# Gepetto/mpc-interface

Hardware: AMD Instinct MI355X
Metric: QP assemblies/sec (P,q,G,h), biped N=16 batched (higher is better)
Workload: dtype f64; 1 GPU; C2 biped LIPM N=16 no=36 nc=76, per-instance (A,B)/given/aim, K1 on chip; batch_per_gpu=4096, global_batch=4096, streams=2

## Files before the change

include/mpcasm.h:

```cpp
#ifndef MPCASM_H
#define MPCASM_H

#include <stddef.h>
#include <stdint.h>

#ifdef __cplusplus
extern "C" {
#endif

typedef enum mpcasm_status {
  MPCASM_OK = 0,
  MPCASM_ERR_ARG = -1,
  MPCASM_ERR_PLAN = -2,
  MPCASM_ERR_HIP = -3,
  MPCASM_ERR_NODEVICE = -4,
  MPCASM_ERR_LIMIT = -5
} mpcasm_status;

typedef struct mpcasm_plan mpcasm_plan;


int mpcasm_abi_version(void);
int mpcasm_device_count(void);
int mpcasm_last_hip(void);
const char* mpcasm_status_string(int status);
enum { MPCASM_OPT_PATH = 1, MPCASM_OPT_PHASE_MASK = 2, MPCASM_OPT_RESIDENT_PER_CU = 3, MPCASM_OPT_JIT = 4,
       MPCASM_OPT_P_DIRECT = 5, MPCASM_OPT_RESIDENT_GRID = 6, MPCASM_OPT_JIT_FETCH_RUNS = 7 };
int mpcasm_set_option(int option, int value);
int mpcasm_plan_set_option(mpcasm_plan* plan, int option, int value);
int mpcasm_resident_lds_bytes(const int32_t* h_itab, size_t n_itab, const double* h_dtab, size_t n_dtab,
                              int64_t out[2]);
int mpcasm_jit_check(const int32_t* h_itab, size_t n_itab, const double* h_dtab, size_t n_dtab,
                     char* log, size_t log_capacity);
int mpcasm_fetch_segments(const int32_t* h_itab, size_t n_itab, const double* h_dtab, size_t n_dtab,
                          int limit, int32_t* out, size_t capacity, int64_t* n_words);

int mpcasm_plan_prepare(const mpcasm_plan* plan, int batch);
int mpcasm_jit_stats(int64_t out[3]);

int mpcasm_fill_su(const double* d_A, const double* d_B, double* d_S, double* d_U,
                   int batch, int N, int n, int m, int ltv, void* stream);

int mpcasm_plan_create(const int32_t* h_itab, size_t n_itab,
                       const double* h_dtab, size_t n_dtab,
                       mpcasm_plan** out_plan);
int mpcasm_plan_destroy(mpcasm_plan* plan);

int mpcasm_plan_sizes(const mpcasm_plan* plan, int64_t out[8]);

int mpcasm_plan_csc_sizes(const mpcasm_plan* plan, int64_t out[2]);

int mpcasm_workspace_bytes(const mpcasm_plan* plan, int batch, size_t* out_bytes);

int mpcasm_assemble(const mpcasm_plan* plan, const double* const* h_src,
                    const int64_t* h_src_stride, const double* d_params,
                    const double* d_given, double* d_P, double* d_q, double* d_G,
                    double* d_h, void* d_work, int batch, void* stream);

int mpcasm_assemble_indexed(const mpcasm_plan* plan, const double* const* h_src,
                            const int64_t* h_src_stride, const double* d_params, const double* d_given,
                            const int32_t* d_given_index, double* d_P, double* d_q, double* d_G,
                            double* d_h, void* d_work, int batch, void* stream);

enum { MPCASM_KERNEL_NONE = 0, MPCASM_KERNEL_RESIDENT = 1, MPCASM_KERNEL_RESIDENT_JIT = 2,
       MPCASM_KERNEL_FUSED = 3, MPCASM_KERNEL_STAGED = 4, MPCASM_KERNEL_TILED = 5,
       MPCASM_KERNEL_TILED_SCAN = 6 ,
       MPCASM_KERNEL_SWEEP = 7 ,
       MPCASM_KERNEL_TILED_SHARED = 8  };
int mpcasm_plan_last_kernel(const mpcasm_plan* plan);

int mpcasm_preview_matrices(const mpcasm_plan* plan, const double* const* h_src,
                            const int64_t* h_src_stride, double* d_PM, int batch,
                            void* stream);

int mpcasm_preview(const double* d_PM, const double* d_given, const double* d_optim,
                   double* d_out, int batch, int rows, int ng, int no, void* stream);

int mpcasm_preview_direct(const mpcasm_plan* plan, const double* const* h_src,
                          const int64_t* h_src_stride, const double* d_given, const double* d_optim,
                          double* d_out, void* d_work, int batch, void* stream);

int mpcasm_goal_distance(const double* d_preview, int64_t preview_stride, const double* d_params,
                         int64_t n_params, const int32_t* d_terms, int nterms, int ngoals,
                         double* d_out, int batch, void* stream);

int mpcasm_preview_goal_distance(const mpcasm_plan* plan, const double* const* h_src,
                                 const int64_t* h_src_stride, const double* d_given,
                                 const double* d_optim, const double* d_params, const int32_t* d_terms,
                                 int nterms, int ngoals, double* d_out, void* d_work, int batch,
                                 void* stream);

enum { MPCASM_PREVIEW_NONE = 0 , MPCASM_PREVIEW_DIRECT = 1,
       MPCASM_PREVIEW_STAGED = 2 ,
       MPCASM_PREVIEW_BLOCKED = 3  };
int mpcasm_preview_route(const int32_t* h_itab, size_t n_itab, const double* h_dtab, size_t n_dtab,
                         const int64_t* h_src_stride, int nterms, int ngoals, int32_t out[8]);

int mpcasm_sweep_route(const int32_t* h_itab, size_t n_itab, const double* h_dtab, size_t n_dtab, int32_t out[8]);

enum { MPCASM_TILED_SCAN = 1, MPCASM_TILED_TOEPLITZ = 2, MPCASM_TILED_SHARED = 3, MPCASM_TILED_GENERAL = 4 };
enum { MPCASM_TILED_TABLES_NONE = 0, MPCASM_TILED_TABLES_SMALL = 1 ,
       MPCASM_TILED_TABLES_SYSTEM = 2  };
enum { MPCASM_WANT_COST = 1, MPCASM_WANT_CONSTRAINTS = 2 };
int mpcasm_tiled_route(const int32_t* h_itab, size_t n_itab, const double* h_dtab, size_t n_dtab,
                       const int64_t* h_src_stride, int batch, int want, int path, int32_t out[16]);

int mpcasm_gather(const double* d_src, int64_t src_stride, const int32_t* d_index, int nnz,
                  double* d_dst, int batch, void* stream);

enum { MPCASM_BOX_RECENTER = 0, MPCASM_BOX_TRANSLATE, MPCASM_BOX_ROTATE, MPCASM_BOX_SCALE,
       MPCASM_BOX_MARGIN };
int mpcasm_box_transform(double* d_params, int64_t n_params, int batch, const int32_t* d_facets,
                         int nfacets, int op, const double* d_arg, int64_t arg_stride,
                         void* stream);

int mpcasm_box_transform_ss(double* d_params, int64_t n_params, int batch,
                            const int32_t* d_facets, int nfacets, int op, const double* d_L,
                            int lrows, int ss_dim, const double* d_arg, int64_t arg_stride,
                            void* stream);

int mpcasm_admm(int no, int nc, const double* d_P, const double* d_q, const double* d_G,
                const double* d_h, double* d_x, double* d_y, double* d_z, double* d_res, double rho,
                double sigma, double alpha, int iters, int warm, int batch, double* d_kinv, int kinv_valid,
                void* stream);

enum {
  MPCASM_QP_SOLVED = 1,
  MPCASM_QP_MAX_ITER = -2,
  MPCASM_QP_PRIMAL_INFEASIBLE = -3,
  MPCASM_QP_DUAL_INFEASIBLE = -4,
  MPCASM_QP_NON_CVX = -7
};

int mpcasm_qp_solve(int no, int nc, const double* d_P, const double* d_q, const double* d_G,
                    const double* d_h, double* d_x, double* d_y, double* d_z, int warm, double* d_rho,
                    double sigma, double alpha, double eps_abs, double eps_rel, double eps_prim_inf,
                    double eps_dual_inf, int max_iter, int check_every, int adaptive_rho_interval,
                    int32_t* d_status, int32_t* d_iters, double* d_res, int batch, double* d_kinv,
                    int kinv_valid, void* stream);
int mpcasm_qp_solve_lds_bytes(int no, int nc, int64_t* out);

int mpcasm_qp_solve_wide(int no, int nc, const double* d_P, const double* d_q, const double* d_G,
                         const double* d_h, double* d_x, double* d_y, double* d_z, int warm, double* d_rho,
                         double sigma, double alpha, double eps_abs, double eps_rel, double eps_prim_inf,
                         double eps_dual_inf, int max_iter, int check_every, int adaptive_rho_interval,
                         int32_t* d_status, int32_t* d_iters, double* d_res, int batch, double* d_kinv,
                         int kinv_valid, void* stream);
int mpcasm_qp_solve_wide_info(int no, int nc, int64_t* lds_bytes, int32_t* kinv_on_chip);

enum { MPCASM_GIVEN_KEEP = -1, MPCASM_GIVEN_CONST = -2 };
int mpcasm_given_map_compile(const mpcasm_plan* plan, const int32_t* h_rows, const double* h_values, int ng,
                             int32_t* h_map, int64_t capacity, int64_t* words);

#define MPCASM_QP_BIT(status) (1u << ((status) < 0 ? -(status) : (status)))
int mpcasm_next_given(const mpcasm_plan* plan, const double* const* h_src, const int64_t* h_src_stride,
                      double* d_given, int64_t rows, const double* d_optim, const int32_t* d_index,
                      const int32_t* d_status, uint32_t apply_mask, const int32_t* d_map, int64_t map_words,
                      void* d_work, int count, void* stream);

enum { MPCASM_ROLL_GIVEN = 0, MPCASM_ROLL_OPTIM = 1, MPCASM_ROLL_STATE = 2 };
#define MPCASM_ROLL_REC_WORDS 8
int mpcasm_ltv_rollout_compile(const int32_t* h_itab, size_t n_itab, const double* h_dtab, size_t n_dtab,
                               const int32_t h_sizes[7], const int32_t* h_recs, int nrec, const double* h_cvec,
                               int ncvec, int32_t* h_table, int64_t capacity, int64_t* words);

int mpcasm_ltv_rollout(const mpcasm_plan* plan, const double* const* h_src, const int64_t* h_src_stride,
                       const double* d_given, int64_t rows, const double* d_optim, const int32_t* d_index,
                       const int32_t* d_table, int64_t table_words, double* d_out, int count, void* stream);

int mpcasm_ltv_advance(const mpcasm_plan* plan, const double* const* h_src, const int64_t* h_src_stride,
                       double* d_given, int64_t rows, const double* d_optim, const int32_t* d_index,
                       const int32_t* d_status, uint32_t apply_mask, const int32_t* d_table, int64_t table_words,
                       int count, void* stream);

#ifdef __cplusplus
}
#endif
#endif
```

mpc-interface_amd/csrc/capi.hip:

```cpp
#include <hip/hip_runtime.h>
#include <stdint.h>
#include <stdlib.h>
#include <string.h>

#include <algorithm>
#include <cmath>
#include <mutex>
#include <new>
#include <string>
#include <vector>

#include "jit.h"
#include "kernels.h"

using namespace mpcasm;

namespace mpcasm {
int g_p_direct = 0;
extern int g_path;
extern int g_phase_mask;
extern int g_resident_per_cu, g_resident_grid;
}

struct mpcasm_plan {
// ... 777 lines not shown
    }
    if (it[H_CSC_PNNZ] != 0 || it[H_CSC_GNNZ] != 0) {
      const int64_t pn = it[H_CSC_PNNZ], gn = it[H_CSC_GNNZ], ldp = no + (no & 1);
      if (gn * nc > (1ll << 27)) return MPCASM_ERR_PLAN;
      if (pn < 0 || gn < 0 || pn > no * no || gn > nc * no || (it[H_CSC_GSINGLE] & ~1) ||
          !in_range(it[H_OFF_CSC_P], pn, n, H_WORDS) || !in_range(it[H_OFF_CSC_G], gn * 2, n, H_WORDS) ||
          it[H_OFF_CSC_G] % 2)
        return MPCASM_ERR_PLAN;
      const int32_t* cp = it + it[H_OFF_CSC_P];
      for (int64_t k = 0; k < pn; ++k)
        if (cp[k] < 0 || cp[k] / ldp >= no || cp[k] % ldp >= no) return MPCASM_ERR_PLAN;
      const int32_t* cg = it + it[H_OFF_CSC_G];
      for (int64_t k = 0; k < gn; ++k) {
        const uint32_t w0 = (uint32_t)cg[2 * k], w1 = (uint32_t)cg[2 * k + 1];
        bool found = false;
        for (int64_t R = 0; R < nc && !found; ++R) {
          const int32_t* x = rrw + R * RS_RR_WORDS;
          if (x[RR_NAXES] > 2) return MPCASM_ERR_PLAN;
          for (int sw = 0; sw < 2 && !found; ++sw) {
            const uint32_t v0 = (uint32_t)x[RR_VOFF + sw], v1 = (uint32_t)x[RR_VOFF + 1 - sw];
            const uint32_t a0 = (uint32_t)x[RR_ARROW + sw], a1 = (uint32_t)x[RR_ARROW + 1 - sw];
            if (w1 != (a0 | (a1 << 16))) continue;
            const uint32_t c = (w0 & 0xFFFF) - v0;
            found = (w0 & 0xFFFF) >= v0 && c < (uint32_t)no && (w0 >> 16) == v1 + c && v1 + c < 65536;
          }
        }
        if (!found) return MPCASM_ERR_PLAN;
      }
    }
    for (int64_t g = 0; g < nlti; ++g) {
      const int32_t* x = it + it[H_OFF_RS_LTI] + g * RS_LTI_WORDS;
      const int64_t gn = x[LT_N], gm = x[LT_M], gN = x[LT_HORIZON];
      if (gn < 1 || gm < 1 || gN < 1 || gn > 64 || gm > 64 || gN > 4096) return MPCASM_ERR_PLAN;
      int stages = 0;
      while ((1ll << stages) < gN) ++stages;
      if (!in_range(x[LT_A], gn * gn, nab, 0) || !in_range(x[LT_B], gn * gm, nab, 0) ||
          !in_range(x[LT_TA], gN * gn * gn, img, dma) || !in_range(x[LT_TB], gN * gn * gm, img, dma) ||
          !in_range(x[LT_TP], (stages + 1) * gn * gn, img, dma))
        return MPCASM_ERR_PLAN;
    }
    auto loads_ok = [&](const int32_t* im, int64_t lanes, int64_t bytes) {
      for (int64_t i = 0; i < lanes; ++i) {
        const int st = im[2 * i];
        const int64_t off = im[2 * i + 1];
        if (st < 0 || st > it[H_NSRC] + 2 || off < 0 || off % bytes) return false;
        const int64_t lim = st < it[H_NSRC]        ? (it + it[H_OFF_ARENA])[2 * st + 1]
                            : st == it[H_NSRC]     ? ng
                            : st == it[H_NSRC] + 1 ? (int64_t)it[H_NPARAMS]
                                                   : 4;
        if (off + bytes > lim * 8) return false;
      }
      return true;
    };
    if (!loads_ok(it + it[H_OFF_RS_INMETA], nchunk * 64, unit) ||
        !loads_ok(it + it[H_OFF_RS_ABMETA], nab * 2, 4))
      return MPCASM_ERR_PLAN;
    for (int c = 0; c < no; ++c) {
      int on = 0;
      for (int g = 0; g < it[H_NGTERM]; ++g) {
        const int32_t* r = it + it[H_OFF_GTERM] + g * GT_WORDS;
        if ((r[GT_FLAGS] & GT_FLAG_DIAG) && c >= r[GT_AOFF] && c < r[GT_AOFF] + r[GT_NROWS]) ++on;
      }
      if (on > RS_DIAG_MAX) return MPCASM_ERR_PLAN;
    }
  }

  {
    const int vrc = validate_tiled(it, h_dtab, n, nd);
    if (vrc != MPCASM_OK) return vrc;
    const int src = validate_sweep(it, n, nd);
    if (src != MPCASM_OK) return src;
  }
  const int32_t* seg = it + it[H_OFF_SEG];
  for (int s = 0; s < it[H_NSEG]; ++s) {
    const int32_t* r = seg + s * SEG_WORDS;
    if (r[SEG_KIND] != SEG_KIND_GATHER && r[SEG_KIND] != SEG_KIND_IDENTITY) return MPCASM_ERR_PLAN;
    if (r[SEG_KIND] == SEG_KIND_GATHER && (r[SEG_SRC] < 0 || r[SEG_SRC] >= it[H_NSRC]))
      return MPCASM_ERR_PLAN;
    if (r[SEG_DST0] < 0 || r[SEG_LEN] < 0 || r[SEG_DST0] + r[SEG_LEN] > W) return MPCASM_ERR_PLAN;
  }
  const int32_t* colseg = it + it[H_OFF_COLSEG];
  for (int64_t i = 0; i < (int64_t)it[H_NBASE] * W; ++i)
    if (colseg[i] < -1 || colseg[i] >= it[H_NSEG]) return MPCASM_ERR_PLAN;
  auto check_csr = [&](int off_ptr, int rows, int off_base, int nent) {
    const int32_t* rp = it + off_ptr;
    if (rp[0] != 0 || rp[rows] != nent) return false;
    for (int r = 0; r < rows; ++r)
      if (rp[r + 1] < rp[r]) return false;
    const int32_t* eb = it + off_base;
    for (int e = 0; e < nent; ++e)
      if (eb[e] < 0 || eb[e] >= it[H_NBASE]) return false;
    return true;
  };
  if (!check_csr(it[H_OFF_ROWPTR], it[H_RTOT], it[H_OFF_ENTBASE], it[H_NENT])) return MPCASM_ERR_PLAN;
  if (!check_csr(it[H_OFF_PM_ROWPTR], it[H_PMROWS], it[H_OFF_PM_ENTBASE], it[H_PM_NENT]))
    return MPCASM_ERR_PLAN;
  const int32_t* gt = it + it[H_OFF_GTERM];
  for (int g = 0; g < it[H_NGTERM]; ++g) {
    const int32_t* r = gt + g * GT_WORDS;
    const int nr = r[GT_NROWS];
    if (r[GT_WPARAM] < 0 || r[GT_WPARAM] >= it[H_NPARAMS]) return MPCASM_ERR_PLAN;
    if (r[GT_AIMPARAM] < 0 || r[GT_AIMPARAM] >= it[H_NPARAMS]) return MPCASM_ERR_PLAN;
    if (r[GT_FLAGS] & GT_FLAG_DIAG) {
      if ((r[GT_FLAGS] & GT_FLAG_P) || nr < 0 || r[GT_AOFF] < 0 || r[GT_AOFF] + nr > no ||
          r[GT_BOFF] < 0 || r[GT_BOFF] + nr > it[H_NDIAGCOEF])
        return MPCASM_ERR_PLAN;
      continue;
    }
    if (nr < 0 || r[GT_AOFF] < 0 || r[GT_AOFF] + nr > it[H_RTOT]) return MPCASM_ERR_PLAN;
    if (r[GT_DOFF] < 0 || r[GT_DOFF] + nr > it[H_RTOT]) return MPCASM_ERR_PLAN;
    if ((r[GT_FLAGS] & GT_FLAG_P) && (r[GT_BOFF] < 0 || r[GT_BOFF] + nr > it[H_RTOT]))
      return MPCASM_ERR_PLAN;
    if (r[GT_WPARAM] < 0 || r[GT_WPARAM] >= it[H_NPARAMS]) return MPCASM_ERR_PLAN;
    if (r[GT_AIMPARAM] < 0 || r[GT_AIMPARAM] >= it[H_NPARAMS]) return MPCASM_ERR_PLAN;
  }
  const int32_t* lim = it + it[H_OFF_LIMIT];
  const int32_t* lax = it + it[H_OFF_LAX];
  const int32_t* rowlimit = it + it[H_OFF_ROWLIMIT];
  for (int l = 0; l < it[H_NLIMIT]; ++l) {
    const int32_t* r = lim + l * LM_WORDS;
    const int nr = r[LM_NROWS], na = r[LM_NAXES];
    if (nr < 0 || na < 0 || r[LM_OUT0] < 0 || r[LM_OUT0] + nr > nc) return MPCASM_ERR_PLAN;
    if (r[LM_LAX0] < 0 || r[LM_LAX0] + na > it[H_NLAX]) return MPCASM_ERR_PLAN;
    const int ar = r[LM_ARROW_ROWS], cr = r[LM_CENTER_ROWS], er = r[LM_EXTREME_ROWS];
    if ((ar != 1 && ar != nr) || (cr != 1 && cr != nr) || (er != 1 && er != nr))
      return MPCASM_ERR_PLAN;
    if (r[LM_ARROW_P] < 0 || r[LM_ARROW_P] + ar * na > it[H_NPARAMS]) return MPCASM_ERR_PLAN;
    if (r[LM_CENTER_P] < 0 || r[LM_CENTER_P] + cr * na > it[H_NPARAMS]) return MPCASM_ERR_PLAN;
    if (r[LM_EXTREME_P] < 0 || r[LM_EXTREME_P] + er > it[H_NPARAMS]) return MPCASM_ERR_PLAN;
    for (int a = 0; a < na; ++a) {
      const int32_t* x = lax + (r[LM_LAX0] + a) * LX_WORDS;
      if ((x[LX_ROWS] != 1 && x[LX_ROWS] != nr) || x[LX_ROWOFF] < 0 ||
          x[LX_ROWOFF] + x[LX_ROWS] > it[H_RTOT])
        return MPCASM_ERR_PLAN;
    }
    for (int k = 0; k < nr; ++k)
      if (rowlimit[r[LM_OUT0] + k] != l) return MPCASM_ERR_PLAN;
  }
  return MPCASM_OK;
}

int make_src_table(const mpcasm_plan* plan, const double* const* h_src,
                   const int64_t* h_src_stride, SrcTable* out) {
  memset(out, 0, sizeof(*out));
  for (int s = 0; s < plan->dev.nsrc; ++s) {
    if (!h_src[s] || h_src_stride[s] < 0) return MPCASM_ERR_ARG;
    out->ptr[s] = h_src[s];
    out->stride[s] = h_src_stride[s];
  }
  return MPCASM_OK;
}

}

namespace {
void plan_dev_from_tables(const int32_t* it, PlanDev* out) {
  PlanDev& d = *out;
  d.ng = it[H_NG]; d.no = it[H_NO]; d.nc = it[H_NC]; d.nparams = it[H_NPARAMS];
  d.nsrc = it[H_NSRC]; d.nbase = it[H_NBASE]; d.nseg = it[H_NSEG]; d.rtot = it[H_RTOT];
  d.nent = it[H_NENT]; d.ngterm = it[H_NGTERM]; d.nlimit = it[H_NLIMIT]; d.nlax = it[H_NLAX];
  d.pmrows = it[H_PMROWS]; d.pm_nent = it[H_PM_NENT]; d.ldv = it[H_LDV];
  d.off_seg = it[H_OFF_SEG]; d.off_colseg = it[H_OFF_COLSEG]; d.off_rowptr = it[H_OFF_ROWPTR];
  d.off_entbase = it[H_OFF_ENTBASE]; d.off_entk = it[H_OFF_ENTK]; d.off_gterm = it[H_OFF_GTERM];
  d.off_limit = it[H_OFF_LIMIT]; d.off_lax = it[H_OFF_LAX]; d.off_rowlimit = it[H_OFF_ROWLIMIT];
  d.off_pm_rowptr = it[H_OFF_PM_ROWPTR]; d.off_pm_entbase = it[H_OFF_PM_ENTBASE];
  d.off_pm_entk = it[H_OFF_PM_ENTK];
  d.doff_entcoef = it[H_DOFF_ENTCOEF]; d.doff_pm_entcoef = it[H_DOFF_PM_ENTCOEF];
  d.fused_ok = it[H_FUSED_OK]; d.arena_total = it[H_ARENA_TOTAL]; d.off_arena = it[H_OFF_ARENA];
  d.nfd = it[H_NFD]; d.off_fd_idx = it[H_OFF_FD_IDX]; d.off_fd_ptr = it[H_OFF_FD_PTR];
  d.nops = it[H_NOPS]; d.off_op = it[H_OFF_OP]; d.ncoef = it[H_NCOEF];
  d.doff_coefpool = it[H_DOFF_COEFPOOL];
  d.rs_ok = it[H_RS_OK]; d.rs_jc = it[H_RS_JC]; d.rs_sym = it[H_RS_SYM];
  d.rs_ntrip = it[H_RS_NTRIP]; d.off_rs_src = it[H_OFF_RS_SRC]; d.off_rs_gidx = it[H_OFF_RS_GIDX];
  d.off_rs_dst = it[H_OFF_RS_DST]; d.doff_rs_coef = it[H_DOFF_RS_COEF];
  d.off_rs_trip = it[H_OFF_RS_TRIP]; d.off_rs_wtrip = it[H_OFF_RS_WTRIP];
  d.rs_nsplit = it[H_RS_NSPLIT]; d.off_rs_split = it[H_OFF_RS_SPLIT];
  d.off_rs_rr = it[H_OFF_RS_RR]; d.rs_unit = it[H_RS_UNIT]; d.rs_nchunk = it[H_RS_NCHUNK];
  d.off_rs_inmeta = it[H_OFF_RS_INMETA]; d.rs_img = it[H_RS_IMG];
  d.rs_img_given = it[H_RS_IMG_GIVEN]; d.rs_img_params = it[H_RS_IMG_PARAMS];
  d.doff_rs_const = it[H_DOFF_RS_CONST];
  d.rs_nlti = it[H_RS_NLTI]; d.off_rs_lti = it[H_OFF_RS_LTI]; d.rs_img_dma = it[H_RS_IMG_DMA];
  d.rs_ab = it[H_RS_AB]; d.off_rs_abmeta = it[H_OFF_RS_ABMETA];
  d.rr_packed = it[H_RR_PACKED];
  d.off_rs_dpar = it[H_OFF_RS_DPAR]; d.doff_rs_dcoef = it[H_DOFF_RS_DCOEF];
  d.rs_ngdesc = it[H_RS_NGDESC]; d.off_rs_gdesc = it[H_OFF_RS_GDESC];
  d.rs_nzblk = it[H_RS_NZBLK]; d.off_rs_zblk = it[H_OFF_RS_ZBLK];
  d.rs_gsingle = it[H_RS_GSINGLE];
  d.csc_pnnz = it[H_CSC_PNNZ]; d.off_csc_p = it[H_OFF_CSC_P];
  d.csc_gnnz = it[H_CSC_GNNZ]; d.off_csc_g = it[H_OFF_CSC_G];
  d.csc_gsingle = it[H_CSC_GSINGLE];
  d.t_ci_ok = it[H_T_CI_OK]; d.t_nop = it[H_T_NOP]; d.off_t_cig = it[H_OFF_T_CIG];
  d.off_t_cio = it[H_OFF_T_CIO]; d.t_doff_delta = it[H_T_DOFF_DELTA]; d.t_ok = it[H_T_OK];
  d.t_nstage = it[H_T_NSTAGE]; d.off_t_stage = it[H_OFF_T_STAGE]; d.t_nlti = it[H_T_NLTI];
  d.off_t_lti = it[H_OFF_T_LTI]; d.off_t_lti_ids = it[H_OFF_T_LTI_IDS]; d.t_work = it[H_T_WORK];
  d.off_t_grow = it[H_OFF_T_GROW];
  d.off_t_srow = it[H_OFF_T_SROW]; d.t_doff_scoef = it[H_T_DOFF_SCOEF]; d.off_t_pig = it[H_OFF_T_PIG];
  d.t_ngrest = it[H_T_NGREST]; d.off_t_grest = it[H_OFF_T_GREST]; d.off_t_brow0 = it[H_OFF_T_BROW0]; d.t_toeplitz = it[H_T_TOEPLITZ];
  d.off_t_bcolptr = it[H_OFF_T_BCOLPTR]; d.off_t_bcols = it[H_OFF_T_BCOLS];
  d.rs_ngfix = it[H_RS_NGFIX]; d.off_rs_gfix = it[H_OFF_RS_GFIX];
  d.rs_compact = it[H_RS_COMPACT]; d.rs_ldv = it[H_RS_LDV]; d.rs_vd = it[H_RS_VD];
  d.rs_vrow0 = it[H_RS_VROW0]; d.off_rs_rrwin = it[H_OFF_RS_RRWIN];
  d.t_np1 = it[H_T_NP1]; d.off_t_p1ptr = it[H_OFF_T_P1PTR]; d.off_t_p1ent = it[H_OFF_T_P1ENT]; d.off_t_p2y = it[H_OFF_T_P2Y];
  d.t_scan = it[H_T_SCAN]; d.t_scan_nblk = it[H_T_SCAN_NBLK]; d.off_t_scan_blk = it[H_OFF_T_SCAN_BLK];
  d.off_t_scan_gt = it[H_OFF_T_SCAN_GT]; d.t_doff_scan_gc = it[H_T_DOFF_SCAN_GC];
  d.off_t_scan_grow = it[H_OFF_T_SCAN_GROW]; d.t_doff_scan_gcoef = it[H_T_DOFF_SCAN_GCOEF];
  d.t_scan_ngrest = it[H_T_SCAN_NGREST]; d.off_t_scan_grest = it[H_OFF_T_SCAN_GREST];
  d.off_t_scan_colblk = it[H_OFF_T_SCAN_COLBLK]; d.t_scan_nother = it[H_T_SCAN_NOTHER];
  d.sw_ok = it[H_SW_OK]; d.sw_n = it[H_SW_N]; d.sw_m = it[H_SW_M]; d.sw_horizon = it[H_SW_HORIZON];
  d.sw_src_a = it[H_SW_SRC_A]; d.sw_src_b = it[H_SW_SRC_B]; d.sw_naxes = it[H_SW_NAXES];
  d.off_sw_axis = it[H_OFF_SW_AXIS]; d.sw_nterm = it[H_SW_NTERM]; d.off_sw_term = it[H_OFF_SW_TERM];
  d.sw_nlim = it[H_SW_NLIM]; d.off_sw_lim = it[H_OFF_SW_LIM]; d.off_sw_col = it[H_OFF_SW_COL];
  d.sw_doff_cvec = it[H_SW_DOFF_CVEC]; d.sw_ncvec = it[H_SW_NCVEC];
  d.off_sw_cptr = it[H_OFF_SW_CPTR]; d.off_sw_cent = it[H_OFF_SW_CENT]; d.sw_ncent = it[H_SW_NCENT];
  d.off_sw_gptr = it[H_OFF_SW_GPTR]; d.off_sw_gent = it[H_OFF_SW_GENT]; d.sw_ngent = it[H_SW_NGENT];
  d.off_rs_prog = it[H_OFF_RS_PROG];
  d.t_scan_fused = it[H_T_SCAN_FUSED];
  d.t_nbrow = d.t_ci_ok ? it[d.off_t_brow0 + d.nbase] : 0;
  d.pm_nfd = it[H_PM_NFD]; d.off_pm_map = it[H_OFF_PM_MAP]; d.off_pm_fdptr = it[H_OFF_PM_FDPTR];
  d.off_pm_op = it[H_OFF_PM_OP]; d.doff_pm_pool = it[H_DOFF_PM_POOL];
  d.rs_src16 = 0;
  if (d.rs_ok && d.rs_unit == 16)
    for (int64_t i = 0; i < (int64_t)d.rs_nchunk * 64; ++i) {
      const int st = it[d.off_rs_inmeta + 2 * i];
      if (st < d.nsrc) d.rs_src16 |= 1u << st;
    }
  d.doff_diagcoef = it[H_DOFF_DIAGCOEF];
  d.ndiag = 0;
  d.rs_sym_any = 1;
  for (int g = 0; g < it[H_NGTERM]; ++g) {
    const int32_t* r = it + it[H_OFF_GTERM] + g * GT_WORDS;
    if (r[GT_FLAGS] & GT_FLAG_DIAG) ++d.ndiag;
    if ((r[GT_FLAGS] & GT_FLAG_P) && r[GT_AOFF] != r[GT_BOFF]) d.rs_sym_any = 0;
  }
  d.rs_diag_table = 1;
  {
    std::vector<int> on(std::max(d.no, 1), 0);
    for (int g = 0; g < it[H_NGTERM]; ++g) {
      const int32_t* r = it + it[H_OFF_GTERM] + g * GT_WORDS;
      if (!(r[GT_FLAGS] & GT_FLAG_DIAG)) continue;
      for (int k = 0; k < r[GT_NROWS]; ++k)
        if (++on[r[GT_AOFF] + k] > RS_DIAG_MAX) d.rs_diag_table = 0;
    }
    if (it[H_OFF_RS_DPAR] % 4 || it[H_DOFF_RS_DCOEF] % 2) d.rs_diag_table = 0;
  }
  d.max_axes = 0;
  for (int l = 0; l < it[H_NLIMIT]; ++l) {
    const int na = it[it[H_OFF_LIMIT] + l * LM_WORDS + LM_NAXES];
    if (na > d.max_axes) d.max_axes = na;
  }
  if (d.fused_ok && (d.off_op & 1)) d.fused_ok = 0;
  d.rs_p_direct = d.rs_ok ? resident_choose_p_direct(d, g_p_direct) : 0;
  if (d.csc_pnnz != 0 && d.rs_ok) d.rs_p_direct = resident_choose_p_direct(d, 2);
}

}

extern "C" {

int mpcasm_abi_version(void) { return 1003; }

int mpcasm_device_count(void) {
  int n = 0;
  if (hipGetDeviceCount(&n) != hipSuccess) return 0;
  return n;
}

int mpcasm_last_hip(void) { return g_last_hip; }

int mpcasm_set_option(int option, int value) {
  if (option == MPCASM_OPT_PATH) {
    if (value < 0 || value > 4) return MPCASM_ERR_ARG;
    g_path = value;
    return MPCASM_OK;
  }
  if (option == MPCASM_OPT_PHASE_MASK) {
    g_phase_mask = value;
    return MPCASM_OK;
  }
  if (option == MPCASM_OPT_P_DIRECT) {
    if (value < 0 || value > 2) return MPCASM_ERR_ARG;
    g_p_direct = value;
    return MPCASM_OK;
  }
  if (option == MPCASM_OPT_JIT) {
    if (value < 0 || value > 2) return MPCASM_ERR_ARG;
    g_jit = value;
    return MPCASM_OK;
  }
  if (option == MPCASM_OPT_RESIDENT_PER_CU) {
    if (value < 0 || value > 16) return MPCASM_ERR_ARG;
    g_resident_per_cu = value;
    return MPCASM_OK;
  }
  if (option == MPCASM_OPT_JIT_FETCH_RUNS) {
    if (value < 0 || value > FS_MAX) return MPCASM_ERR_ARG;
    g_jit_fetch_runs = value;
    return MPCASM_OK;
  }
  if (option == MPCASM_OPT_RESIDENT_GRID) {
    if (value < 0 || value > (1 << 20)) return MPCASM_ERR_ARG;
    g_resident_grid = value;
    return MPCASM_OK;
  }
  return MPCASM_ERR_ARG;
}

int mpcasm_plan_set_option(mpcasm_plan* plan, int option, int value) {
  if (!plan) return MPCASM_ERR_ARG;
  if (option == MPCASM_OPT_PATH && value >= -1 && value <= 4) plan->opt_path = value;
  else if (option == MPCASM_OPT_JIT && value >= -1 && value <= 2) plan->opt_jit = value;
  else if (option == MPCASM_OPT_RESIDENT_PER_CU && value >= -1 && value <= 16) plan->opt_per_cu = value;
  else if (option == MPCASM_OPT_RESIDENT_GRID && value >= -1 && value <= (1 << 20)) plan->opt_grid = value;
  else return MPCASM_ERR_ARG;
  return MPCASM_OK;
}

const char* mpcasm_status_string(int status) {
  switch (status) {
    case MPCASM_OK: return "ok";
    case MPCASM_ERR_ARG: return "invalid argument";
    case MPCASM_ERR_PLAN: return "malformed plan tables";
    case MPCASM_ERR_HIP: return "HIP runtime error";
    case MPCASM_ERR_NODEVICE: return "no HIP device";
    case MPCASM_ERR_LIMIT: return "problem exceeds a kernel limit";
    default: return "unknown status";
  }
}

int mpcasm_fill_su(const double* d_A, const double* d_B, double* d_S, double* d_U, int batch,
                   int N, int n, int m, int ltv, void* stream) {
  if (!d_A || !d_B || !d_S || !d_U) return MPCASM_ERR_ARG;
  if (batch < 0 || N < 1 || n < 1 || m < 1 || (ltv != 0 && ltv != 1)) return MPCASM_ERR_ARG;
  if (batch == 0) return MPCASM_OK;
  if (mpcasm_device_count() == 0) return MPCASM_ERR_NODEVICE;
  hipError_t err;
  const int rc = launch_fill_su(d_A, d_B, d_S, d_U, batch, N, n, m, ltv,
                                static_cast<hipStream_t>(stream), &err);
  if (rc == MPCASM_ERR_HIP) g_last_hip = (int)err;
  return rc;
}

int mpcasm_plan_create(const int32_t* h_itab, size_t n_itab, const double* h_dtab, size_t n_dtab,
                       mpcasm_plan** out_plan) {
  if (!h_itab || !out_plan || (n_dtab && !h_dtab)) return MPCASM_ERR_ARG;
  *out_plan = nullptr;
  const int rc = validate_plan(h_itab, h_dtab, n_itab, n_dtab);
  if (rc != MPCASM_OK) return rc;
  {
    PlanDev probe;
    memset(&probe, 0, sizeof probe);
    plan_dev_from_tables(h_itab, &probe);
    if ((probe.csc_pnnz != 0 || probe.csc_gnnz != 0) &&
        (probe.rs_p_direct != 0 || resident_lds_bytes(probe) == 0 ||
         resident_lds_bytes(probe) > RESIDENT_LDS_LIMIT))
      return MPCASM_ERR_LIMIT;
  }
  if (mpcasm_device_count() == 0) return MPCASM_ERR_NODEVICE;

  mpcasm_plan* plan = new (std::nothrow) mpcasm_plan();
  if (!plan) return MPCASM_ERR_ARG;
  hipError_t e;
  if ((e = hipGetDevice(&plan->device)) != hipSuccess) {
    delete plan;
    return hip_fail(e);
  }
  plan->d_itab = nullptr;
  plan->d_dtab = nullptr;
  const size_t dbytes = (n_dtab ? n_dtab : 1) * sizeof(double);
  if ((e = hipMalloc(&plan->d_itab, n_itab * sizeof(int32_t))) != hipSuccess ||
      (e = hipMalloc(&plan->d_dtab, dbytes)) != hipSuccess ||
      (e = hipMemcpy(plan->d_itab, h_itab, n_itab * sizeof(int32_t), hipMemcpyHostToDevice)) !=
          hipSuccess ||
      (n_dtab && (e = hipMemcpy(plan->d_dtab, h_dtab, n_dtab * sizeof(double),
                                hipMemcpyHostToDevice)) != hipSuccess)) {
    if (plan->d_itab) (void)hipFree(plan->d_itab);
    if (plan->d_dtab) (void)hipFree(plan->d_dtab);
    delete plan;
    return hip_fail(e);
  }
  PlanDev& d = plan->dev;
  plan_dev_from_tables(h_itab, &d);
  d.itab = plan->d_itab;
  d.dtab = plan->d_dtab;
  plan->h_itab.assign(h_itab, h_itab + n_itab);
  {
    hipDeviceProp_t prop;
    plan->num_cus = 256;
    if (hipGetDeviceProperties(&prop, plan->device) == hipSuccess && prop.multiProcessorCount > 0)
      plan->num_cus = prop.multiProcessorCount;
  }
  *out_plan = plan;
  return MPCASM_OK;
}

int mpcasm_resident_lds_bytes(const int32_t* h_itab, size_t n_itab, const double* h_dtab, size_t n_dtab,
                              int64_t out[2]) {
  if (!h_itab || (n_dtab && !h_dtab) || !out) return MPCASM_ERR_ARG;
  const int rc = validate_plan(h_itab, h_dtab, n_itab, n_dtab);
  if (rc != MPCASM_OK) return rc;
  PlanDev d;
  memset(&d, 0, sizeof d);
  plan_dev_from_tables(h_itab, &d);
  for (int direct = 0; direct < 2; ++direct) {
    d.rs_p_direct = 1 - direct;
    out[direct] = (int64_t)resident_lds_bytes(d);
  }
  return MPCASM_OK;
}

int mpcasm_jit_check(const int32_t* h_itab, size_t n_itab, const double* h_dtab, size_t n_dtab,
                     char* log, size_t log_capacity) {
  if (!h_itab || (n_dtab && !h_dtab)) return MPCASM_ERR_ARG;
  if (log && log_capacity) log[0] = 0;
  const int rc = validate_plan(h_itab, h_dtab, n_itab, n_dtab);
  if (rc != MPCASM_OK) return rc;
  PlanDev d;
  memset(&d, 0, sizeof d);
  plan_dev_from_tables(h_itab, &d);
  if (!d.rs_ok) return MPCASM_ERR_LIMIT;
  std::vector<char> code;
  std::string text;
  const int small = resident_p_direct_for(d, 1), large = resident_p_direct_for(d, 1 << 30);
  int out = MPCASM_OK;
  if (!jit_available()) {
    text = "libhiprtc.so could not be loaded";
    out = MPCASM_ERR_LIMIT;
  } else {
    for (int form : {small, large}) {
      if (form == large && small != large && out != MPCASM_OK) break;
      d.rs_p_direct = form;
      out = jit_code_for(jit_spec_header(d, h_itab, g_jit_fetch_runs), false, 0xBF, &code, &text) ? MPCASM_OK : MPCASM_ERR_HIP;
      if (small == large) break;
    }
  }
  if (log && log_capacity) {
    strncpy(log, text.c_str(), log_capacity - 1);
    log[log_capacity - 1] = 0;
  }
  return out;
}

int mpcasm_fetch_segments(const int32_t* h_itab, size_t n_itab, const double* h_dtab, size_t n_dtab,
                          int limit, int32_t* out, size_t capacity, int64_t* n_words) {
  if (!h_itab || (n_dtab && !h_dtab) || !n_words || (capacity && !out) || limit < 0) return MPCASM_ERR_ARG;
  const int rc = validate_plan(h_itab, h_dtab, n_itab, n_dtab);
  if (rc != MPCASM_OK) return rc;
  PlanDev d;
  memset(&d, 0, sizeof d);
  plan_dev_from_tables(h_itab, &d);
  if (!d.rs_ok) return MPCASM_ERR_LIMIT;
  const std::vector<int32_t> words = jit_fetch_plan(d, h_itab, limit);
  *n_words = (int64_t)words.size();
  if (words.size() > capacity) return MPCASM_ERR_LIMIT;
  if (!words.empty()) memcpy(out, words.data(), words.size() * sizeof(int32_t));
  return MPCASM_OK;
}

int mpcasm_jit_stats(int64_t out[3]) {
  if (!out) return MPCASM_ERR_ARG;
  long v[3];
  jit_stats(v);
  out[0] = v[0];
  out[1] = v[1];
  out[2] = v[2];
  return MPCASM_OK;
}

int mpcasm_plan_prepare(const mpcasm_plan* plan, int batch) {
  if (!plan || batch < 0) return MPCASM_ERR_ARG;
  int current = -1;
  if (hipGetDevice(&current) != hipSuccess || current != plan->device) return MPCASM_ERR_ARG;
  PlanDev p = plan->dev;
  if (!p.rs_ok || p.sw_ok) return MPCASM_OK;
  p.rs_p_direct = resident_p_direct_for(plan->dev, batch);
  const size_t rs = resident_lds_bytes(p);
  if (rs == 0 || rs > RESIDENT_LDS_LIMIT) return MPCASM_OK;
  t_path = plan->opt_path >= 0 ? plan->opt_path : g_path;
  t_jit = plan->opt_jit >= 0 ? plan->opt_jit : g_jit;
  if (t_path != 0 && p.rs_nlti == 0 && p.csc_pnnz == 0 && p.csc_gnnz == 0) return MPCASM_OK;
  (void)jit_kernel_for(p, plan->h_itab.data(), plan->device, batch, rs);
  return MPCASM_OK;
}

int mpcasm_plan_destroy(mpcasm_plan* plan) {
  if (!plan) return MPCASM_OK;
  jit_forget(plan->d_itab);
  hipError_t e1 = hipFree(plan->d_itab);
  hipError_t e2 = hipFree(plan->d_dtab);
  delete plan;
  if (e1 != hipSuccess) return hip_fail(e1);
  if (e2 != hipSuccess) return hip_fail(e2);
  return MPCASM_OK;
}

int mpcasm_plan_sizes(const mpcasm_plan* plan, int64_t out[8]) {
  if (!plan || !out) return MPCASM_ERR_ARG;
  const PlanDev& d = plan->dev;
  out[0] = d.ng; out[1] = d.no; out[2] = d.nc; out[3] = d.nparams;
  out[4] = d.nsrc; out[5] = d.rtot; out[6] = d.ldv; out[7] = d.pmrows;
  return MPCASM_OK;
}

int mpcasm_plan_csc_sizes(const mpcasm_plan* plan, int64_t out[2]) {
  if (!plan || !out) return MPCASM_ERR_ARG;
  out[0] = plan->dev.csc_pnnz;
  out[1] = plan->dev.csc_gnnz;
  return MPCASM_OK;
}

int mpcasm_workspace_bytes(const mpcasm_plan* plan, int batch, size_t* out_bytes) {
  if (!plan || !out_bytes || batch < 0) return MPCASM_ERR_ARG;
  const size_t groups = (size_t)std::min<long>(batch, (long)plan->num_cus * 8);
  const size_t stamps = 2 * groups * 8 * 8 * sizeof(uint64_t);
  const int path = plan->opt_path >= 0 ? plan->opt_path : g_path;
  if (sweep_eligible(plan->dev)) {
    *out_bytes = stamps;
    return MPCASM_OK;
  }
  if (tiled_eligible(plan->dev) && path != 2) {
    *out_bytes = std::max(tiled_workspace_bytes(plan->dev, batch), stamps);
    return MPCASM_OK;
  }
  *out_bytes = std::max(std::max(assemble_workspace_bytes(plan->dev, batch),
                                 tiled_workspace_bytes(plan->dev, batch)), stamps);
  return MPCASM_OK;
}

static int assemble_impl(const mpcasm_plan* plan, const double* const* h_src,
                         const int64_t* h_src_stride, const double* d_params, const double* d_given,
                         const int32_t* d_given_index, double* d_P, double* d_q, double* d_G, double* d_h,
                         void* d_work, int batch, void* stream) {
  if (!plan || batch < 0) return MPCASM_ERR_ARG;
  if (batch == 0) return MPCASM_OK;
  const PlanDev& d = plan->dev;
  if ((d.nsrc && (!h_src || !h_src_stride)) || (d.nparams && !d_params) || (d.ng && !d_given))
    return MPCASM_ERR_ARG;
  if ((d_P == nullptr) != (d_q == nullptr) || (d_G == nullptr) != (d_h == nullptr))
    return MPCASM_ERR_ARG;
  if (d.rtot && !d_work && !d.sw_ok) return MPCASM_ERR_ARG;
  {
    int current = -1;
    if (hipGetDevice(&current) != hipSuccess || current != plan->device) return MPCASM_ERR_ARG;
  }
  if ((reinterpret_cast<uintptr_t>(d_P) | reinterpret_cast<uintptr_t>(d_q) |
       reinterpret_cast<uintptr_t>(d_G) | reinterpret_cast<uintptr_t>(d_h)) & 15)
    return MPCASM_ERR_ARG;
  SrcTable src;
  int rc = make_src_table(plan, h_src, h_src_stride, &src);
  if (rc != MPCASM_OK) return rc;
  if (d_given_index != nullptr) {
    if (d.nsrc >= MAX_SOURCES || d.ng == 0) return MPCASM_ERR_LIMIT;
    src.ptr[MAX_SOURCES - 1] = reinterpret_cast<const double*>(d_given_index);
    src.stride[MAX_SOURCES - 1] = -1;
  }
  hipError_t err;
  t_path = plan->opt_path >= 0 ? plan->opt_path : g_path;
  t_jit = plan->opt_jit >= 0 ? plan->opt_jit : g_jit;
  t_per_cu = plan->opt_per_cu >= 0 ? plan->opt_per_cu : g_resident_per_cu;
  t_grid = plan->opt_grid >= 0 ? plan->opt_grid : g_resident_grid;
  rc = launch_assemble(d, src, d_params, d_given, d_P, d_q, d_G, d_h, d_work, batch,
                       plan->num_cus, static_cast<hipStream_t>(stream), &err, plan->h_itab.data(),
                       plan->device, d_given_index != nullptr);
  if (rc == MPCASM_ERR_HIP) g_last_hip = (int)err;
  if (rc == MPCASM_OK) plan->last_kernel = t_last_kernel;
  return rc;
}

int mpcasm_assemble(const mpcasm_plan* plan, const double* const* h_src,
                    const int64_t* h_src_stride, const double* d_params, const double* d_given,
                    double* d_P, double* d_q, double* d_G, double* d_h, void* d_work, int batch,
                    void* stream) {
  return assemble_impl(plan, h_src, h_src_stride, d_params, d_given, nullptr, d_P, d_q, d_G, d_h, d_work,
                       batch, stream);
}

int mpcasm_assemble_indexed(const mpcasm_plan* plan, const double* const* h_src,
                            const int64_t* h_src_stride, const double* d_params, const double* d_given,
                            const int32_t* d_given_index, double* d_P, double* d_q, double* d_G,
                            double* d_h, void* d_work, int batch, void* stream) {
  if (!d_given_index) return MPCASM_ERR_ARG;
  return assemble_impl(plan, h_src, h_src_stride, d_params, d_given, d_given_index, d_P, d_q, d_G, d_h,
                       d_work, batch, stream);
}

int mpcasm_plan_last_kernel(const mpcasm_plan* plan) { return plan ? plan->last_kernel : MPCASM_ERR_ARG; }

int mpcasm_preview_matrices(const mpcasm_plan* plan, const double* const* h_src,
                            const int64_t* h_src_stride, double* d_PM, int batch, void* stream) {
  if (!plan || !d_PM || batch < 0) return MPCASM_ERR_ARG;
  if (plan->dev.nsrc && (!h_src || !h_src_stride)) return MPCASM_ERR_ARG;
  if (plan->dev.rs_nlti != 0 || plan->dev.sw_ok) return MPCASM_ERR_LIMIT;
  if (batch == 0) return MPCASM_OK;
  SrcTable src;
  int rc = make_src_table(plan, h_src, h_src_stride, &src);
  if (rc != MPCASM_OK) return rc;
  hipError_t err;
  rc = launch_preview_matrices(plan->dev, src, d_PM, batch, static_cast<hipStream_t>(stream), &err);
  if (rc == MPCASM_ERR_HIP) g_last_hip = (int)err;
  return rc;
}

int mpcasm_preview(const double* d_PM, const double* d_given, const double* d_optim, double* d_out,
                   int batch, int rows, int ng, int no, void* stream) {
  if (!d_PM || !d_out || batch < 0 || rows < 0 || ng < 0 || no < 0) return MPCASM_ERR_ARG;
  if ((ng && !d_given) || (no && !d_optim)) return MPCASM_ERR_ARG;
  if (batch == 0 || rows == 0) return MPCASM_OK;
  hipError_t err;
  const int rc = launch_preview(d_PM, d_given, d_optim, d_out, batch, rows, ng, no,
                                static_cast<hipStream_t>(stream), &err);
  if (rc == MPCASM_ERR_HIP) g_last_hip = (int)err;
  return rc;
}

int mpcasm_preview_direct(const mpcasm_plan* plan, const double* const* h_src,
                          const int64_t* h_src_stride, const double* d_given, const double* d_optim,
                          double* d_out, void* d_work, int batch, void* stream) {
  if (!plan || !d_out || batch < 0) return MPCASM_ERR_ARG;
  const PlanDev& d = plan->dev;
  if ((d.nsrc && (!h_src || !h_src_stride)) || (d.ng && !d_given) || (d.no && !d_optim))
    return MPCASM_ERR_ARG;
  if (batch == 0 || d.pmrows == 0) return MPCASM_OK;
  if (d.sw_ok) return MPCASM_ERR_LIMIT;
  if (d.t_nlti != 0 && !d_work) return MPCASM_ERR_ARG;
  {
    int current = -1;
    if (hipGetDevice(&current) != hipSuccess || current != plan->device) return MPCASM_ERR_ARG;
  }
  SrcTable src, eff;
  int rc = make_src_table(plan, h_src, h_src_stride, &src);
  if (rc != MPCASM_OK) return rc;
  hipError_t err;
  rc = launch_lti_tables(d, src, static_cast<double*>(d_work), batch, plan->h_itab.data(), &eff,
                         static_cast<hipStream_t>(stream));
  if (rc != MPCASM_OK) return rc;
  rc = launch_preview_direct(d, eff, d_given, d_optim, d_out, batch, plan->num_cus,
                             static_cast<hipStream_t>(stream), &err, plan->h_itab.data());
  if (rc == MPCASM_ERR_HIP) g_last_hip = (int)err;
  return rc;
}

int mpcasm_preview_route(const int32_t* h_itab, size_t n_itab, const double* h_dtab, size_t n_dtab,
                         const int64_t* h_src_stride, int nterms, int ngoals, int32_t out[8]) {
  if (!h_itab || (n_dtab && !h_dtab) || !out || nterms < 0 || ngoals < 0) return MPCASM_ERR_ARG;
  memset(out, 0, 8 * sizeof(int32_t));
  const int rc = validate_plan(h_itab, h_dtab, n_itab, n_dtab);
  if (rc != MPCASM_OK) return rc;
  PlanDev d;
  memset(&d, 0, sizeof d);
  plan_dev_from_tables(h_itab, &d);
  if (d.nsrc && !h_src_stride) return MPCASM_ERR_ARG;
  if (d.sw_ok) return MPCASM_ERR_LIMIT;
  SrcTable src, eff;
  memset(&src, 0, sizeof src);
  for (int s = 0; s < d.nsrc; ++s) {
    if (h_src_stride[s] < 0) return MPCASM_ERR_ARG;
    src.stride[s] = h_src_stride[s];
  }
  const int lti = lti_effective_sources(d, src, nullptr, h_itab, &eff);
  if (lti != MPCASM_OK) return lti;
  return preview_route(d, eff, h_itab, nterms, ngoals, out);
}

int mpcasm_sweep_route(const int32_t* h_itab, size_t n_itab, const double* h_dtab, size_t n_dtab, int32_t out[8]) {
  if (!h_itab || (n_dtab && !h_dtab) || !out) return MPCASM_ERR_ARG;
  memset(out, 0, 8 * sizeof(int32_t));
  const int rc = validate_plan(h_itab, h_dtab, n_itab, n_dtab);
  if (rc != MPCASM_OK) return rc;
  PlanDev d;
  memset(&d, 0, sizeof d);
  plan_dev_from_tables(h_itab, &d);
  if (!sweep_eligible(d)) return MPCASM_ERR_ARG;
  SweepChoice c;
  const int choice = sweep_choose(d, h_itab, &c);
  if (choice != MPCASM_OK) return choice;
  out[0] = c.cpt;
  out[1] = c.specialised;
  out[2] = c.pair;
  out[3] = c.per_line;
  out[4] = c.reg_lines;
  out[5] = sweep_lines_ahead(c.cpt);
  out[6] = (int32_t)c.lds;
  out[7] = c.lds > 64 * 1024;
  return MPCASM_OK;
}

int mpcasm_tiled_route(const int32_t* h_itab, size_t n_itab, const double* h_dtab, size_t n_dtab,
                       const int64_t* h_src_stride, int batch, int want, int path, int32_t out[16]) {
  if (!h_itab || (n_dtab && !h_dtab) || !out || batch < 1 || path < -1 || path > 4 || want < 1 || want > 3)
    return MPCASM_ERR_ARG;
  memset(out, 0, 16 * sizeof(int32_t));
  const int rc = validate_plan(h_itab, h_dtab, n_itab, n_dtab);
  if (rc != MPCASM_OK) return rc;
  PlanDev d;
  memset(&d, 0, sizeof d);
  plan_dev_from_tables(h_itab, &d);
  if (d.nsrc && !h_src_stride) return MPCASM_ERR_ARG;
  SrcTable src;
  memset(&src, 0, sizeof src);
  for (int s = 0; s < d.nsrc; ++s) {
    if (h_src_stride[s] < 0) return MPCASM_ERR_ARG;
    src.stride[s] = h_src_stride[s];
  }
  if (path < 0) path = g_path;
  if (sweep_eligible(d)) return MPCASM_ERR_ARG;
  d.rs_p_direct = d.rs_ok ? resident_p_direct_for(d, batch) : 0;
  const size_t rs = resident_lds_bytes(d);
  if (rs != 0 && rs <= RESIDENT_LDS_LIMIT && (path == 0 || d.rs_nlti != 0 || d.csc_pnnz != 0 || d.csc_gnnz != 0))
    return MPCASM_ERR_ARG;
  if (!tiled_eligible(d) || path == 2 || d.csc_pnnz != 0 || d.csc_gnnz != 0) return MPCASM_ERR_ARG;
  TiledChoice c;
  const int choice = tiled_choose(d, src, h_itab, path, batch, (want & MPCASM_WANT_COST) != 0,
                                  (want & MPCASM_WANT_CONSTRAINTS) != 0, true, true, &c);
  if (choice != MPCASM_OK) return choice;
  out[0] = c.form;
  out[1] = c.fused;
  out[2] = c.kp;
  out[3] = c.cb;
  out[4] = c.rows_in_lds;
  out[5] = c.whole_lines;
  out[6] = (int32_t)c.lds;
  out[7] = c.lds > 64 * 1024;
  out[8] = c.tables;
  out[9] = c.tg;
  out[10] = c.sym;
  return MPCASM_OK;
}

int mpcasm_given_map_compile(const mpcasm_plan* plan, const int32_t* h_rows, const double* h_values, int ng,
                             int32_t* h_map, int64_t capacity, int64_t* words) {
  if (!plan || !h_rows || !words || capacity < 0) return MPCASM_ERR_ARG;
  const PlanDev& d = plan->dev;
  if (ng != d.ng) return MPCASM_ERR_ARG;
  if (d.sw_ok || !d.t_ci_ok) return MPCASM_ERR_LIMIT;
  for (int c = 0; c < ng; ++c) {
    const int r = h_rows[c];
    if (r == MPCASM_GIVEN_CONST ? (!h_values || !std::isfinite(h_values[c]))
                                : (r != MPCASM_GIVEN_KEEP && (r < 0 || r >= d.pmrows)))
      return MPCASM_ERR_ARG;
  }
  std::vector<int32_t> map;
  const int rc = compile_given_map(d, plan->h_itab.data(), h_rows, h_values, &map);
  if (rc != MPCASM_OK) return rc;
// ... 341 lines not shown
```

mpc-interface_amd/csrc/jit.h:

```cpp
#pragma once
#include <hip/hip_runtime.h>
#include <stdint.h>

#include <string>
#include <vector>

#include "plan_dev.h"

namespace mpcasm {

extern int g_jit;
extern int g_jit_fetch_runs;
extern int g_phase_mask;

std::string jit_spec_header(const PlanDev& d, const int32_t* h_itab, int seg_limit = FS_MAX);
std::vector<int32_t> jit_fetch_plan(const PlanDev& d, const int32_t* h_itab, int seg_limit);
int jit_compile(const std::string& header, std::vector<char>* code, std::string* log,
                bool stamps = false, int phases = 0xBF);
const void* jit_kernel_for(const PlanDev& d, const int32_t* h_itab, int device, int batch,
                           size_t lds_bytes);
bool jit_code_for(const std::string& header, bool stamps, int phases, std::vector<char>* code,
                  std::string* log, bool distrust_disk = false);
bool jit_available();
void jit_stats(long out[3]);
void jit_forget(const void* itab);
int jit_launch(const void* kernel, const PlanDev& p, const SrcTable& src, const double* params,
               const double* given, double* P, double* q, double* G, double* h, int batch,
               int num_cus, int per_cu_limit, int grid_limit, void* work, hipStream_t stream, hipError_t* err);

}
```

mpc-interface_amd/csrc/jit.hip:

```cpp
#include <dlfcn.h>
#include <hip/hip_runtime.h>
#include <stdint.h>
#include <stdio.h>
#include <stdlib.h>
#include <string.h>

#include <sys/stat.h>
#include <sys/types.h>
#include <unistd.h>

#include <atomic>
#include <condition_variable>
#include <iterator>
#include <map>
#include <mutex>
#include <string>
#include <vector>

#include "jit.h"
#include "kernels.h"

namespace mpcasm {

int g_jit = 0;
int g_jit_fetch_runs = FS_MAX;

namespace {

#include "jit_embed.inc"

constexpr int JIT_MIN_BATCH = 512;

struct Rtc {
  typedef struct _hiprtcProgram* Program;
  int (*create)(Program*, const char*, const char*, int, const char* const*, const char* const*);
  int (*compile)(Program, int, const char* const*);
  int (*log_size)(Program, size_t*);
  int (*get_log)(Program, char*);
  int (*code_size)(Program, size_t*);
  int (*get_code)(Program, char*);
  int (*destroy)(Program*);
  bool ok = false;
};

const Rtc& rtc() {
  static Rtc r;
  static std::once_flag once;
  std::call_once(once, [] {
    void* lib = nullptr;
    for (const char* name : {"libhiprtc.so", "libhiprtc.so.7", "/opt/rocm/lib/libhiprtc.so"}) {
      lib = dlopen(name, RTLD_NOW | RTLD_GLOBAL);
      if (lib) break;
    }
    if (!lib) return;
    auto sym = [&](const char* name) { return dlsym(lib, name); };
    r.create = reinterpret_cast<decltype(r.create)>(sym("hiprtcCreateProgram"));
    r.compile = reinterpret_cast<decltype(r.compile)>(sym("hiprtcCompileProgram"));
    r.log_size = reinterpret_cast<decltype(r.log_size)>(sym("hiprtcGetProgramLogSize"));
    r.get_log = reinterpret_cast<decltype(r.get_log)>(sym("hiprtcGetProgramLog"));
    r.code_size = reinterpret_cast<decltype(r.code_size)>(sym("hiprtcGetCodeSize"));
    r.get_code = reinterpret_cast<decltype(r.get_code)>(sym("hiprtcGetCode"));
    r.destroy = reinterpret_cast<decltype(r.destroy)>(sym("hiprtcDestroyProgram"));
    r.ok = r.create && r.compile && r.log_size && r.get_log && r.code_size && r.get_code && r.destroy;
  });
  return r;
}

void append(std::string& s, const char* fmt, long long v) {
  char buf[96];
  snprintf(buf, sizeof buf, fmt, v);
  s += buf;
}

}

std::vector<int32_t> jit_fetch_segments(const int32_t* meta, int lanes) {
  std::vector<int32_t> out;
  for (int i = 0; i < lanes;) {
    const int stream = meta[2 * i], byte0 = meta[2 * i + 1];
    const int step = i + 1 < lanes && meta[2 * (i + 1)] == stream ? meta[2 * (i + 1) + 1] - byte0 : 0;
    int best = 0, best_period = 0;
    for (int period : {0, 4, 2, 1}) {
      int n = 0;
      while (i + n < lanes && meta[2 * (i + n)] == stream &&
             meta[2 * (i + n) + 1] == byte0 + (period ? n % period : n) * (period == 1 ? 0 : step))
        ++n;
      if (n > best) best = n, best_period = period;
    }
    const int period = best_period && best_period < best ? best_period : best;
    out.insert(out.end(), {i, best, stream, byte0, best > 1 && period > 1 ? step : 0, period});
    i += best;
  }
  return out;
}

std::vector<int32_t> jit_fetch_plan(const PlanDev& d, const int32_t* it, int limit) {
  std::vector<int32_t> out;
  if (limit > FS_MAX) limit = FS_MAX;
  for (int kind = 0; kind < 2; ++kind) {
    const int chunks = kind == 0 ? d.rs_ab / 32 : d.rs_nchunk;
    const int32_t* meta = it + (kind == 0 ? d.off_rs_abmeta : d.off_rs_inmeta);
    for (int k = 0; k < chunks; ++k) {
      std::vector<int32_t> segs = jit_fetch_segments(meta + k * 128, 64);
      if ((int)segs.size() > limit * FS_WORDS || (kind == 1 && k >= 32)) segs.clear();
      out.insert(out.end(), {kind, k, (int32_t)(segs.size() / FS_WORDS)});
      out.insert(out.end(), segs.begin(), segs.end());
    }
  }
  return out;
}

std::string jit_spec_header(const PlanDev& d, const int32_t* it, int seg_limit) {
  std::string s = "// generated by libmpcasm (jit.hip) for one plan\n#pragma once\n"
                  "namespace mpcasm {\nnamespace spec {\nstruct PlanConst {\n";
#define MPCASM_X(f) append(s, "  static constexpr int " #f " = %lld;\n", (long long)d.f);
  MPCASM_PLAN_INT_FIELDS(MPCASM_X)
#undef MPCASM_X
  append(s, "  static constexpr unsigned rs_src16 = %lldu;\n};\n", (long long)d.rs_src16);
  const int jc = d.rs_jc <= 3 ? 3 : d.rs_jc <= 4 ? 4 : d.rs_jc <= 5 ? 5 : d.rs_jc <= 8 ? 8 : RS_JC_MAX;
  append(s, "constexpr int JC = %lld;\n", jc);
  append(s, "constexpr int NTRIP = %lld;\n", d.rs_ntrip);
  s += "constexpr int TRIPS[NTRIP + 1][8] = {\n";
  const int32_t* tr = it + d.off_rs_trip;
  for (int t = 0; t <= d.rs_ntrip; ++t) {
    s += "  {";
    for (int k = 0; k < RS_TRIP_WORDS; ++k) append(s, k ? ", %lld" : "%lld", tr[t * RS_TRIP_WORDS + k]);
    s += "},\n";
  }
  s += "};\nconstexpr int WTRIP[8][2] = {";
  const int32_t* wt = it + d.off_rs_wtrip;
  for (int w = 0; w < RS_WAVES; ++w) {
    append(s, "{%lld, ", wt[2 * w]);
    append(s, "%lld}, ", wt[2 * w + 1]);
  }
  s += "};\n";
  const std::vector<int32_t> fetch = jit_fetch_plan(d, it, seg_limit);
  for (int kind = 0; kind < 2; ++kind) {
    const int chunks = kind == 0 ? d.rs_ab / 32 : d.rs_nchunk;
    const char* name = kind == 0 ? "AB" : "IMG";
    std::string counts, table;
    long long on_table = 0;
    for (size_t at = 0; at < fetch.size(); at += 3 + fetch[at + 2] * FS_WORDS) {
      if (fetch[at] != kind) continue;
      const int n = fetch[at + 2];
      if (n == 0 && fetch[at + 1] < 32) on_table |= 1ll << fetch[at + 1];
      append(counts, "%lld, ", n);
      table += "  {";
      for (int g = 0; g < FS_MAX; ++g) {
        table += "{";
        for (int w = 0; w < FS_WORDS; ++w) append(table, w ? ", %lld" : "%lld", g < n ? fetch[at + 3 + g * FS_WORDS + w] : 0);
        table += "}, ";
      }
      table += "},\n";
    }
    if (chunks == 0) counts = "0", table = "  {},\n";
    s += std::string("constexpr int FSEG_") + name + "_N[] = {" + counts + "};\n";
    s += std::string("constexpr int FSEG_") + name + "[][8][6] = {\n" + table + "};\n";
    s += std::string("constexpr unsigned FSEG_") + name + "_TABLE = ";
    append(s, "%lldu;\n", on_table);
  }
  s += "constexpr int LTI[4][8] = {\n";
  for (int g = 0; g < RS_LTI_MAX; ++g) {
    s += "  {";
    for (int w = 0; w < RS_LTI_WORDS; ++w)
      append(s, w ? ", %lld" : "%lld", g < d.rs_nlti ? it[d.off_rs_lti + g * RS_LTI_WORDS + w] : 0);
    s += "},\n";
  }
  s += "};\n}  // namespace spec\n}  // namespace mpcasm\n";
  return s;
}

int jit_compile(const std::string& header, std::vector<char>* code, std::string* log, bool stamps,
                int phases) {
  const Rtc& r = rtc();
  if (!r.ok) {
    if (log) *log = "libhiprtc.so could not be loaded";
    return MPCASM_ERR_LIMIT;
  }
  const char* headers[] = {header.c_str(), k_src_device_prims, k_src_plan_dev, k_src_plan_tables};
  const char* names[] = {"plan_spec.h", "device_prims.h", "plan_dev.h", "plan_tables.h"};
  Rtc::Program prog = nullptr;
  if (r.create(&prog, k_src_resident, "resident.hip", 4, headers, names) != 0) return MPCASM_ERR_HIP;
  const char* waves = getenv("MPCASM_JIT_WAVES_PER_EU");
  const std::string wopt = std::string("-DMPCASM_SPEC_WAVES_PER_EU=") + (waves ? waves : "4");
  const char* last = stamps ? "-DMPCASM_SPEC_STAMPS=1"
                            : (getenv("MPCASM_JIT_PLAIN_STORES") ? "-DMPCASM_PLAIN_STORES=1" : "-DMPCASM_SPEC_NT=1");
  char popt[48];
  snprintf(popt, sizeof popt, "-DMPCASM_SPEC_PHASES=%d", phases);
  const char* opts[] = {"--offload-arch=gfx950", "-O3", "-std=c++17", "-DMPCASM_SPEC=1", wopt.c_str(), last, popt};
  const int rc = r.compile(prog, phases >= 0 ? 7 : 6, opts);
  size_t n = 0;
  if (log && r.log_size(prog, &n) == 0 && n > 1) {
    log->resize(n);
    r.get_log(prog, &(*log)[0]);
  }
  int out = MPCASM_ERR_HIP;
  if (rc == 0 && r.code_size(prog, &n) == 0 && n > 0) {
    code->resize(n);
    if (r.get_code(prog, code->data()) == 0) out = MPCASM_OK;
  }
  r.destroy(&prog);
  if (const char* dump = getenv("MPCASM_JIT_DUMP")) {
    const std::string base(dump);
    if (FILE* f = fopen((base + ".h").c_str(), "w")) {
      fwrite(header.data(), 1, header.size(), f);
      fclose(f);
    }
    if (out == MPCASM_OK)
      if (FILE* f = fopen((base + ".co").c_str(), "wb")) {
        fwrite(code->data(), 1, code->size(), f);
        fclose(f);
      }
  }
  return out;
}

namespace {

std::atomic<long> g_stat_compiled{0}, g_stat_disk_hits{0}, g_stat_disk_writes{0};

uint64_t fnv1a(const std::string& text, uint64_t h) {
  for (unsigned char c : text) {
    h ^= c;
    h *= 1099511628211ull;
  }
  return h;
}

std::string cache_dir() {
  if (const char* off = getenv("MPCASM_NO_DISK_CACHE"))
    if (off[0] && off[0] != '0') return "";
  std::string dir;
  if (const char* d = getenv("MPCASM_CACHE_DIR")) {
    dir = d;
  } else if (const char* x = getenv("XDG_CACHE_HOME")) {
    dir = std::string(x) + "/mpcasm";
  } else if (const char* home = getenv("HOME")) {
    dir = std::string(home) + "/.cache/mpcasm";
  }
  if (dir.empty()) return "";
  const size_t cut = dir.find_last_of('/');
  if (cut != std::string::npos && cut > 0) (void)mkdir(dir.substr(0, cut).c_str(), 0755);
  (void)mkdir(dir.c_str(), 0755);
  struct stat st;
  if (stat(dir.c_str(), &st) != 0 || !S_ISDIR(st.st_mode) || access(dir.c_str(), W_OK) != 0) return "";
  return dir;
}

std::string cache_key(const std::string& header, const std::string& options) {
  int major = 0, minor = 0;
  if (void* lib = dlopen("libhiprtc.so", RTLD_NOW | RTLD_NOLOAD)) {
    typedef int (*version_fn)(int*, int*);
    if (auto f = reinterpret_cast<version_fn>(dlsym(lib, "hiprtcVersion"))) (void)f(&major, &minor);
  }
  std::string all = header + "\x1f" + options + "\x1f" + k_src_resident + "\x1f" + k_src_device_prims +
                    "\x1f" + k_src_plan_dev + "\x1f" + k_src_plan_tables + "\x1fhiprtc " +
                    std::to_string(major) + "." + std::to_string(minor);
  int runtime = 0;
  if (hipRuntimeGetVersion(&runtime) == hipSuccess) all += " hip " + std::to_string(runtime);
  char name[64];
  snprintf(name, sizeof name, "%016llx%016llx", (unsigned long long)fnv1a(all, 14695981039346656037ull),
           (unsigned long long)fnv1a(all, 0x9E3779B97F4A7C15ull));
  return name;
}

bool disk_read(const std::string& path, std::vector<char>* code) {
  FILE* f = fopen(path.c_str(), "rb");
  if (!f) return false;
  fseek(f, 0, SEEK_END);
  const long n = ftell(f);
  fseek(f, 0, SEEK_SET);
  bool ok = n > 0;
  if (ok) {
    code->resize((size_t)n);
    ok = fread(code->data(), 1, (size_t)n, f) == (size_t)n;
  }
  fclose(f);
  return ok;
}

void disk_write(const std::string& path, const std::vector<char>& code) {
  const std::string tmp = path + ".tmp" + std::to_string((long)getpid());
  FILE* f = fopen(tmp.c_str(), "wb");
  if (!f) return;
  const bool ok = fwrite(code.data(), 1, code.size(), f) == code.size();
  fclose(f);
  if (ok && rename(tmp.c_str(), path.c_str()) == 0)
    ++g_stat_disk_writes;
  else
    (void)unlink(tmp.c_str());
}

struct JitKernel {
  hipModule_t module = nullptr;
  hipFunction_t fn = nullptr;
  int per_cu = 0;
  size_t lds = 0;
  bool failed = false;
  bool building = true;
};

std::mutex g_mutex;
std::condition_variable g_built;
std::map<std::pair<int, std::string>, JitKernel*> g_cache;
struct FastKey {
  const void* itab;
  int device, p_direct, phases, fetch_runs;
  bool operator<(const FastKey& o) const {
    if (fetch_runs != o.fetch_runs) return fetch_runs < o.fetch_runs;
    if (itab != o.itab) return itab < o.itab;
    if (device != o.device) return device < o.device;
    if (p_direct != o.p_direct) return p_direct < o.p_direct;
    return phases < o.phases;
  }
};
std::map<FastKey, JitKernel*> g_fast;

}

bool jit_code_for(const std::string& header, bool stamps, int phases, std::vector<char>* code,
                  std::string* log_out, bool distrust_disk) {
  const char* waves = getenv("MPCASM_JIT_WAVES_PER_EU");
  const std::string options = std::string(stamps ? "stamps " : "") + "phases " + std::to_string(phases) +
                              " waves " + (waves ? waves : "4") +
                              (getenv("MPCASM_JIT_PLAIN_STORES") ? " plain-stores" : "");
  const std::string dir = cache_dir();
  const std::string path = dir.empty() ? "" : dir + "/" + cache_key(header, options) + ".co";
  if (distrust_disk && !path.empty()) (void)unlink(path.c_str());
  if (!distrust_disk && !path.empty() && disk_read(path, code)) {
    ++g_stat_disk_hits;
    if (getenv("MPCASM_JIT_VERBOSE")) fprintf(stderr, "mpcasm: jit: code object from %s\n", path.c_str());
    return true;
  }
  std::string log;
  const int rc = jit_compile(header, code, &log, stamps, phases);
  if (log_out) *log_out = log;
  if (rc != MPCASM_OK) {
    if (getenv("MPCASM_JIT_VERBOSE")) fprintf(stderr, "mpcasm: jit failed:\n%s\n", log.c_str());
    return false;
  }
  ++g_stat_compiled;
  if (getenv("MPCASM_JIT_VERBOSE")) fprintf(stderr, "mpcasm: jit: compiled (%zu bytes)\n", code->size());
  if (!path.empty()) disk_write(path, *code);
  return true;
}

namespace {
}

const void* jit_kernel_for(const PlanDev& d, const int32_t* h_itab, int device, int batch,
                           size_t lds_bytes) {
  if (t_jit == 2) return nullptr;
  const bool stamps = (g_phase_mask & 64) != 0;
  const int phases = stamps ? -1 : g_phase_mask;
  const FastKey fast{d.itab, stamps ? device + 4096 : device, d.rs_p_direct, phases, g_jit_fetch_runs};
  const bool may_build = t_jit == 1 || batch >= JIT_MIN_BATCH;
  JitKernel* slot = nullptr;
  bool mine = false;
  std::string header;
  {
    std::unique_lock<std::mutex> lock(g_mutex);
    auto found = g_fast.find(fast);
    if (found != g_fast.end()) {
      slot = found->second;
    } else if (may_build) {
      header = jit_spec_header(d, h_itab, fast.fetch_runs);
      JitKernel*& by_text = g_cache[std::make_pair(fast.device, header + "//" + std::to_string(phases))];
      if (by_text == nullptr) {
        by_text = new JitKernel();
        mine = true;
      }
      slot = by_text;
      g_fast[fast] = slot;
    } else {
      return nullptr;
    }
    if (!mine) {
      if (slot->building && !may_build) return nullptr;
      g_built.wait(lock, [&] { return !slot->building; });
    }
  }
  if (mine) {
    std::vector<char> code;
    hipModule_t module = nullptr;
    hipFunction_t fn = nullptr;
    bool ok = false;
    for (int attempt = 0; attempt < 2 && !ok; ++attempt) {
      code.clear();
      const long hits = g_stat_disk_hits;
      ok = jit_code_for(header, stamps, phases, &code, nullptr, attempt == 1);
      const bool from_disk = g_stat_disk_hits != hits;
      if (ok && (hipModuleLoadData(&module, code.data()) != hipSuccess ||
                 hipModuleGetFunction(&fn, module, "resident_spec_kernel") != hipSuccess)) {
        (void)hipGetLastError();
        if (module) (void)hipModuleUnload(module);
        module = nullptr;
        fn = nullptr;
        ok = false;
        if (!from_disk) break;
      } else if (!ok) {
        break;
      }
    }
    if (ok && hipFuncSetAttribute(reinterpret_cast<const void*>(fn), hipFuncAttributeMaxDynamicSharedMemorySize,
                                  CU_LDS_BYTES) != hipSuccess) {
      (void)hipGetLastError();
      if (hipFuncSetAttribute(reinterpret_cast<const void*>(fn), hipFuncAttributeMaxDynamicSharedMemorySize,
                              RESIDENT_LDS_LIMIT) != hipSuccess) {
        (void)hipGetLastError();
        ok = false;
      }
    }
    {
      std::lock_guard<std::mutex> lock(g_mutex);
      slot->module = module;
      slot->fn = fn;
      slot->failed = !ok;
      slot->building = false;
    }
    g_built.notify_all();
  }
  std::lock_guard<std::mutex> lock(g_mutex);
  if (slot->failed) return nullptr;
  if (slot->lds != lds_bytes) {
    int n = 0;
    if (hipModuleOccupancyMaxActiveBlocksPerMultiprocessor(&n, slot->fn, RS_NT, lds_bytes) != hipSuccess ||
        n < 1) {
      (void)hipGetLastError();
      slot->failed = true;
      return nullptr;
    }
    slot->per_cu = n;
    slot->lds = lds_bytes;
  }
  return slot;
}

bool jit_available() { return rtc().ok; }

void jit_stats(long out[3]) {
  out[0] = g_stat_compiled;
  out[1] = g_stat_disk_hits;
  out[2] = g_stat_disk_writes;
}

void jit_forget(const void* itab) {
  std::lock_guard<std::mutex> lock(g_mutex);
  for (auto it = g_fast.begin(); it != g_fast.end();)
    it = it->first.itab == itab ? g_fast.erase(it) : std::next(it);
}

int jit_launch(const void* kernel, const PlanDev& p, const SrcTable& src, const double* params,
               const double* given, double* P, double* q, double* G, double* h, int batch,
               int num_cus, int per_cu_limit, int grid_limit, void* work, hipStream_t stream,
               hipError_t* err) {
  const JitKernel* k = static_cast<const JitKernel*>(kernel);
  int per_cu = k->per_cu;
  if (per_cu_limit > 0 && per_cu_limit < per_cu) per_cu = per_cu_limit;
  long grid = (long)num_cus * per_cu;
  if (grid_limit > 0 && grid_limit < grid) grid = grid_limit;
  if (grid > batch) grid = batch;
  const int32_t* itab = p.itab;
  const double* dtab = p.dtab;
  SrcTable s = src;
  int phases = g_phase_mask;
  unsigned long long* stamps = (g_phase_mask & 64) ? static_cast<unsigned long long*>(work) : nullptr;
  void* args[] = {&itab, &dtab, &s, &params, &given, &P, &q, &G, &h, &batch, &phases, &stamps};
  *err = hipModuleLaunchKernel(k->fn, (unsigned)grid, 1, 1, RS_NT, 1, 1, (unsigned)k->lds, stream,
                               args, nullptr);
  return *err == hipSuccess ? MPCASM_OK : MPCASM_ERR_HIP;
}

}
```

mpc-interface_amd/csrc/plan_dev.h:

```cpp
#pragma once
#ifndef __HIPCC_RTC__
#include <stdint.h>
#endif

#include "plan_tables.h"

namespace mpcasm {

#define MPCASM_PLAN_INT_FIELDS(X)                                                                   \
  X(ng) X(no) X(nc) X(nparams) X(nsrc) X(nbase) X(nseg) X(rtot) X(nent) X(ngterm) X(nlimit)         \
  X(nlax) X(pmrows) X(pm_nent) X(ldv) X(off_seg) X(off_colseg) X(off_rowptr) X(off_entbase)         \
  X(off_entk) X(off_gterm) X(off_limit) X(off_lax) X(off_rowlimit) X(off_pm_rowptr)                 \
  X(off_pm_entbase) X(off_pm_entk) X(doff_entcoef) X(doff_pm_entcoef) X(fused_ok) X(arena_total)    \
  X(off_arena) X(nfd) X(off_fd_idx) X(off_fd_ptr) X(nops) X(off_op) X(ncoef) X(doff_coefpool)       \
  X(max_axes) X(rs_sym_any) X(rs_ok) X(rs_jc) X(rs_sym) X(rs_ntrip) X(off_rs_src) X(off_rs_gidx)    \
  X(off_rs_dst) X(doff_rs_coef) X(off_rs_trip) X(off_rs_wtrip) X(rs_nsplit) X(off_rs_split)         \
  X(off_rs_rr) X(rs_unit) X(rs_nchunk) X(off_rs_inmeta) X(rs_img) X(rs_img_given)                   \
  X(rs_img_params) X(doff_rs_const) X(rs_nlti) X(off_rs_lti) X(rs_img_dma) X(rs_ab)                 \
  X(off_rs_abmeta) X(rr_packed) X(off_rs_dpar) X(doff_rs_dcoef) X(rs_ngdesc) X(off_rs_gdesc)        \
  X(pm_nfd) X(off_pm_map) X(off_pm_fdptr) X(off_pm_op) X(doff_pm_pool) X(doff_diagcoef) X(ndiag)      \
  X(rs_nzblk) X(off_rs_zblk) X(rs_p_direct) X(rs_gsingle)                                           \
  X(csc_pnnz) X(off_csc_p) X(csc_gnnz) X(off_csc_g) X(csc_gsingle)                                  \
  X(t_ci_ok) X(t_nop) X(off_t_cig) X(off_t_cio) X(t_doff_delta) X(t_ok) X(t_nstage)                 \
  X(off_t_stage) X(t_nlti) X(off_t_lti) X(off_t_lti_ids) X(t_work) X(off_t_grow)                    \
  X(off_t_srow) X(t_doff_scoef) X(off_t_pig) X(t_ngrest) X(off_t_grest) X(off_t_brow0) X(t_nbrow) X(t_toeplitz) X(rs_diag_table) X(off_t_bcolptr) X(off_t_bcols) \
  X(rs_ngfix) X(off_rs_gfix) X(rs_compact) X(rs_ldv) X(rs_vd) X(rs_vrow0) X(off_rs_rrwin) X(t_np1) X(off_t_p1ptr) X(off_t_p1ent) X(off_t_p2y) \
  X(t_scan) X(t_scan_nblk) X(off_t_scan_blk) X(off_t_scan_gt) X(t_doff_scan_gc) X(off_t_scan_grow)      \
  X(t_doff_scan_gcoef) X(t_scan_ngrest) X(off_t_scan_grest) X(off_t_scan_colblk) X(t_scan_nother) \
  X(sw_ok) X(sw_n) X(sw_m) X(sw_horizon) X(sw_src_a) X(sw_src_b) X(sw_naxes) X(off_sw_axis) X(sw_nterm)  \
  X(off_sw_term) X(sw_nlim) X(off_sw_lim) X(off_sw_col) X(sw_doff_cvec) X(sw_ncvec) \
  X(off_sw_cptr) X(off_sw_cent) X(sw_ncent) X(off_sw_gptr) X(off_sw_gent) X(sw_ngent) X(off_rs_prog) X(t_scan_fused)

struct PlanDev {
  const int32_t* itab;
  const double* dtab;
#define MPCASM_X(f) int f;
  MPCASM_PLAN_INT_FIELDS(MPCASM_X)
#undef MPCASM_X
  unsigned rs_src16;
};

constexpr int RESIDENT_LDS_LIMIT = 156 * 1024;

struct SrcTable {
  const double* ptr[MAX_SOURCES];
  long long stride[MAX_SOURCES];
};

}
```

mpc-interface_amd/csrc/resident.hip:

```cpp
#ifdef __HIPCC_RTC__
using __hip_internal::int32_t;
using __hip_internal::int64_t;
using __hip_internal::uint32_t;
using __hip_internal::uint64_t;
typedef unsigned long uintptr_t;
#else
#include <hip/hip_runtime.h>
#include <stdint.h>
#endif

#include "device_prims.h"
#include "plan_dev.h"
#ifdef MPCASM_SPEC
#include "plan_spec.h"
#endif
#ifndef __HIPCC_RTC__
#include "kernels.h"
#endif

namespace mpcasm {

#ifndef __HIPCC_RTC__
extern int g_phase_mask;
extern int g_resident_per_cu;
#endif

namespace {

constexpr int NT = RS_NT;
constexpr int MW = RS_NW;
constexpr int WT = NT - MW * 64;
constexpr int AXMAX = RS_AXMAX;
constexpr int RR_WORDS = RS_RR_WORDS;
constexpr int RR_COMPACT = 4;
static_assert(RS_DIAG_MAX == 2, "the per-column diagonal table holds two terms");

__host__ __device__ inline int even_up_i(int x) { return (x + 1) & ~1; }

constexpr int GU = 6;
template <class PlanT>
__host__ __device__ inline int resident_g_mode(const PlanT& p) {
  if (p.csc_gnnz != 0 || p.csc_pnnz != 0) return 3;
  if (!p.rr_packed) return 0;
  return p.rs_ngdesc != 0 ? 2 : 1;
}
static_assert(GU == RS_GDESC_PIECES && WT == RS_GDESC_THREADS, "descriptor table of G");

template <class PlanT>
__host__ __device__ inline int resident_v_doubles(const PlanT& p) {
  return (p.rs_vrow0 + p.rtot) * p.rs_ldv + 16;
}

struct ResidentLayout {
  int v, pl, ql, dvec, dcoef, dpar, img, ab, streams, ints, total_doubles;
  int ldp;
  int p_direct;
  int i_rr, i_meta, i_wtrip, i_split, i_lti, i_abmeta, i_gdesc, i_gfix, i_rrwin, i_cscp;
};

template <class PlanT>
__host__ __device__ inline ResidentLayout resident_layout(const PlanT& p) {
  ResidentLayout L;
  L.ldp = even_up_i(p.no);
  int o = 0;
  L.v = o;      o += resident_v_doubles(p);
  L.pl = o;
  L.ql = o;     o += L.ldp;
  L.dvec = o;   o += 2 * L.ldp;
  L.dcoef = o;  o += RS_DIAG_MAX * L.ldp;
  L.dpar = o;   o += RS_DIAG_MAX * L.ldp;
  L.img = o;    o += 2 * p.rs_img;
  L.ab = o;     o += 2 * p.rs_ab;
  L.streams = o; o += 2 * (MAX_SOURCES + 3);
  L.ints = o;
  int i = 0;
  L.i_rr = i;    i += p.nc * (p.rr_packed ? RR_COMPACT : RR_WORDS);
  L.i_meta = i;  i += p.rs_nchunk * 64 * 2;
  L.i_abmeta = i; i += p.rs_ab * 2 * 2;
  L.i_gdesc = i;  i += resident_g_mode(p) == 2 ? GU * WT * 2 : (resident_g_mode(p) == 3 ? 2 * p.csc_gnnz : 0);
  L.i_gfix = i;   i += resident_g_mode(p) == 2 && p.rs_ngfix != 0 ? 2 * WT : 0;
  L.i_rrwin = i;  i += p.rs_compact ? p.nc : 0;
  L.i_cscp = i;   i += resident_g_mode(p) == 3 ? p.csc_pnnz : 0;
  L.i_wtrip = i; i += RS_WAVES * 2;
  L.i_split = i; i += p.rs_nsplit;
  L.i_lti = i;   i += p.rs_nlti * RS_LTI_WORDS;
  o += even_up_i(i) / 2;
  L.p_direct = p.rs_p_direct;
  L.pl = o;
  if (!L.p_direct) o += p.no * L.ldp;
  L.total_doubles = o;
  return L;
}

__device__ __forceinline__ void dma16(const void* gsrc, unsigned lds_base) {
  unsigned keep;
  asm volatile(
      "s_mov_b32 %0, m0\n\ts_mov_b32 m0, %2\n\ts_nop 0\n\tglobal_load_lds_dwordx4 %1, off\n\t"
      "s_mov_b32 m0, %0"
      : "=&s"(keep)
      : "v"(gsrc), "s"(lds_base)
      : "memory");
}
__device__ __forceinline__ void dma4(const void* gsrc, unsigned lds_base) {
  unsigned keep;
  asm volatile(
      "s_mov_b32 %0, m0\n\ts_mov_b32 m0, %2\n\ts_nop 0\n\tglobal_load_lds_dword %1, off\n\t"
      "s_mov_b32 m0, %0"
      : "=&s"(keep)
      : "v"(gsrc), "s"(lds_base)
      : "memory");
}
__device__ __forceinline__ void dma_wait() { asm volatile("s_waitcnt vmcnt(0)" ::: "memory"); }
__device__ __forceinline__ void dma_wait_but(int later) {
  switch (later) {
    case 1: asm volatile("s_waitcnt vmcnt(1)" ::: "memory"); break;
    case 2: asm volatile("s_waitcnt vmcnt(2)" ::: "memory"); break;
    case 3: asm volatile("s_waitcnt vmcnt(3)" ::: "memory"); break;
    case 4: asm volatile("s_waitcnt vmcnt(4)" ::: "memory"); break;
    default: asm volatile("s_waitcnt vmcnt(0)" ::: "memory"); break;
  }
}

__device__ __forceinline__ int resident_trip_row(int lk) { return ((lk & 1) << 3) | ((lk & 2) << 1); }

#ifdef MPCASM_SPEC
struct TripState {
  const char* Vlane;
  const char* prc;
  double *Pl, *ql;
  int ldpl;
  bool mirror;
  const double* dvec;
  int lx, lg, lk;
  const char *ap, *bp;
  int bi, bj;
  bool isq, live;
  double acc, sum;
};

template <int I>
__device__ __forceinline__ void spec_trip(TripState& s) {
  using PC = spec::PlanConst;
  constexpr int A = spec::TRIPS[I][RT_A], B = spec::TRIPS[I][RT_B], D = spec::TRIPS[I][RT_D];
  constexpr int W = spec::TRIPS[I][RT_W], AIM = spec::TRIPS[I][RT_AIM], WORD = spec::TRIPS[I][RT_WORD];
  constexpr int BI = spec::TRIPS[I][RT_BI], BJ = spec::TRIPS[I][RT_BJ];
  constexpr int row_bytes = PC::rs_ldv * 8, ldp = (PC::no + 1) & ~1;
  constexpr int qmask = (WORD >> RT_QMASK) & 15, livemask = (WORD >> RT_LIVE) & 15;
  constexpr bool nop = (WORD >> RT_NOP) & 1, half = (WORD >> RT_HALF) & 1;
  if constexpr ((WORD >> RT_FIRST) & 1) {
    int lg_ = s.lg;
    asm volatile("" : "+v"(lg_));
    s.bi = (BI >> (8 * lg_)) & 255;
    s.bj = (BJ >> (8 * lg_)) & 255;
    s.isq = (qmask >> lg_) & 1;
    s.live = (livemask >> lg_) & 1;
    s.ap = s.Vlane + s.bi * 32;
    s.bp = s.Vlane + (s.isq ? 0 : s.bj * 32);
    s.acc = 0.0;
  }
  if constexpr ((WORD & 31) != 0) {
    const char* bsrc = qmask == 0 ? s.bp + B : (qmask == livemask ? s.bp + D : s.bp + (s.isq ? D : B));
    if constexpr (!((WORD >> RT_SHORT) & 1)) {
      constexpr int span = 3 * row_bytes;
      constexpr int AH = A + span < 65536 ? 0 : A, DH = D + span < 65536 ? 0 : D, BH = B + span < 65536 ? 0 : B;
      const unsigned pa = (unsigned)(uintptr_t)s.ap + AH;
      if constexpr (qmask == 0) {
        s.sum = mfma_trip16<A - AH, B - BH, row_bytes>(pa, (unsigned)(uintptr_t)s.bp + BH, s.sum);
      } else if constexpr (qmask == livemask) {
        s.sum = mfma_trip16<A - AH, D - DH, row_bytes>(pa, (unsigned)(uintptr_t)s.bp + DH, s.sum);
      } else {
        s.sum = mfma_trip16<A - AH, B - BH, row_bytes>(pa, (unsigned)(uintptr_t)s.bp + BH + (s.isq ? D - B : 0), s.sum);
      }
    } else {
      const int short_shift = (s.lk - resident_trip_row(s.lk)) * row_bytes;
      const double a = *reinterpret_cast<const double*>(s.ap + (A + short_shift));
      const double b = *reinterpret_cast<const double*>(bsrc + short_shift);
      s.sum = mfma_f64_4x4x4(a, b, s.sum);
    }
    if constexpr ((WORD >> RT_TERM_END) & 1) {
      const double w = *reinterpret_cast<const double*>(s.prc + W);
      if constexpr (qmask != 0 || nop) {
        const double aim = *reinterpret_cast<const double*>(s.prc + AIM);
        const double ws = half ? 0.5 * w : w;
        const double ones = quad_broadcast<1>(s.sum);
        const double m = s.isq ? ws : (nop ? 0.0 : w);
        s.acc = fma(m, fma(-(s.isq ? aim : 0.0), ones, s.sum), s.acc);
      } else {
        s.acc = fma(w, s.sum, s.acc);
      }
      s.sum = 0.0;
    }
  }
  if constexpr ((WORD >> RT_LAST) & 1) {
    int lk_ = s.lk, lx_ = s.lx;
    asm volatile("" : "+v"(lk_), "+v"(lx_));
    const int row = 4 * s.bi + lk_, col = 4 * s.bj + lx_;
    if (s.live && row < PC::no) {
      if (s.isq) {
        if (lx_ == 0) s.ql[row] = s.acc + s.dvec[ldp + row];
      } else if (col < PC::no) {
        const double val = s.acc + (row == col ? s.dvec[col] : 0.0);
        s.Pl[row * s.ldpl + col] = val;
        if (PC::rs_sym && s.bi != s.bj) s.Pl[col * s.ldpl + row] = val;
      }
    }
  }
}

struct LaneSrc {
  const char* base;
  long long stride;
  bool isg;
  int2 entry;
};
static_assert(FS_MAX == 8 && FS_WORDS == 6 && RS_LTI_MAX == 4 && RS_LTI_WORDS == 8, "plan_spec.h, as jit.hip writes it");
template <bool AB, int K>
constexpr int spec_fetch_runs() {
  if constexpr (AB)
    return K < spec::PlanConst::rs_ab / 32 ? spec::FSEG_AB_N[K] : 0;
  else
    return K < spec::PlanConst::rs_nchunk ? spec::FSEG_IMG_N[K] : 0;
}
template <bool AB, int K, int S>
__device__ __forceinline__ void spec_lane_run(LaneSrc& out, int lane, const SrcTable& src, const double* params,
                                              const double* given, const double* plan_dtab) {
  using PC = spec::PlanConst;
  if constexpr (S < spec_fetch_runs<AB, K>()) {
    constexpr int first = AB ? spec::FSEG_AB[K][S][FS_FIRST] : spec::FSEG_IMG[K][S][FS_FIRST];
    constexpr int lanes = AB ? spec::FSEG_AB[K][S][FS_LANES] : spec::FSEG_IMG[K][S][FS_LANES];
    constexpr int stream = AB ? spec::FSEG_AB[K][S][FS_STREAM] : spec::FSEG_IMG[K][S][FS_STREAM];
    constexpr int byte0 = AB ? spec::FSEG_AB[K][S][FS_BYTE] : spec::FSEG_IMG[K][S][FS_BYTE];
    constexpr int step = AB ? spec::FSEG_AB[K][S][FS_STEP] : spec::FSEG_IMG[K][S][FS_STEP];
    constexpr int period = AB ? spec::FSEG_AB[K][S][FS_PERIOD] : spec::FSEG_IMG[K][S][FS_PERIOD];
    static_assert(period >= lanes || (period & (period - 1)) == 0, "a periodic run repeats every 1, 2 or 4 lanes");
    const char* base;
    long long stride;
    if constexpr (stream < PC::nsrc) {
      base = reinterpret_cast<const char*>(src.ptr[stream]);
      stride = src.stride[stream] * (long long)sizeof(double);
    } else if constexpr (stream == PC::nsrc) {
      base = reinterpret_cast<const char*>(given);
      stride = (long long)PC::ng * (long long)sizeof(double);
    } else if constexpr (stream == PC::nsrc + 1) {
      base = reinterpret_cast<const char*>(params);
      stride = (long long)PC::nparams * (long long)sizeof(double);
    } else {
      base = reinterpret_cast<const char*>(plan_dtab + PC::doff_rs_const);
      stride = 0;
    }
    const int rel = lane - first;
    const int off = byte0 + (period < lanes ? rel & (period - 1) : rel) * step;
    if (S == 0 || lane >= first) {
      out.base = base + off;
      out.stride = stride;
      out.isg = stream == PC::nsrc;
      out.entry = int2{stream, off};
    }
    spec_lane_run<AB, K, S + 1>(out, lane, src, params, given, plan_dtab);
  }
}
template <bool AB, int K>
__device__ __forceinline__ LaneSrc spec_lane_src(int lane, const SrcTable& src, const double* params,
                                                 const double* given, const double* plan_dtab) {
  LaneSrc out{nullptr, 0, false, int2{0, 0}};
  spec_lane_run<AB, K, 0>(out, lane, src, params, given, plan_dtab);
  return out;
}
template <bool AB, int K>
__device__ __forceinline__ void spec_write_table(int2* table, int lane, const SrcTable& src, const double* params,
                                                 const double* given, const double* plan_dtab) {
  if constexpr (K < (AB ? spec::PlanConst::rs_ab / 32 : spec::PlanConst::rs_nchunk)) {
    table[K * 64 + lane] = spec_lane_src<AB, K>(lane, src, params, given, plan_dtab).entry;
    spec_write_table<AB, K + 1>(table, lane, src, params, given, plan_dtab);
  }
}
template <int K>
__device__ __forceinline__ void spec_first_ab(int lane, long inst0, long inst1, bool two, unsigned ab_lds,
                                              const SrcTable& src, const double* params, const double* given,
                                              const double* plan_dtab) {
  using PC = spec::PlanConst;
  if constexpr (K < PC::rs_ab / 32) {
    const LaneSrc m = spec_lane_src<true, K>(lane, src, params, given, plan_dtab);
    dma4(m.base + inst0 * m.stride, ab_lds + (unsigned)(K * 32 * 8));
    if (two) dma4(m.base + inst1 * m.stride, ab_lds + (unsigned)((PC::rs_ab + K * 32) * 8));
    spec_first_ab<K + 1>(lane, inst0, inst1, two, ab_lds, src, params, given, plan_dtab);
  }
}
template <int K>
__device__ __forceinline__ void spec_first_image(int lane, long inst, long ginst, unsigned img_lds, const SrcTable& src,
                                                 const double* params, const double* given, const double* plan_dtab) {
  using PC = spec::PlanConst;
  if constexpr (K < PC::rs_nchunk && K < 32) {
    if constexpr (spec_fetch_runs<false, K>() != 0) {
      const LaneSrc m = spec_lane_src<false, K>(lane, src, params, given, plan_dtab);
      const char* a = m.base + (m.isg ? ginst : inst) * m.stride;
      if constexpr (PC::rs_unit == 16)
        dma16(a, img_lds + (unsigned)(K * 64 * 16));
      else
        dma4(a, img_lds + (unsigned)(K * 64 * 4));
    }
    spec_first_image<K + 1>(lane, inst, ginst, img_lds, src, params, given, plan_dtab);
  }
}
constexpr bool spec_ab_by_runs() {
  for (int k = 0; k < spec::PlanConst::rs_ab / 32; ++k)
    if (spec::FSEG_AB_N[k] == 0) return false;
  return true;
}

template <int I, int N>
__device__ __forceinline__ void spec_trips(TripState& s) {
  if constexpr (I < N) {
    spec_trip<I>(s);
    __builtin_amdgcn_sched_barrier(0);
    spec_trips<I + 1, N>(s);
  }
}
template <int WAVE>
__device__ __forceinline__ void spec_wave_trips(TripState& s) {
  spec_trips<spec::WTRIP[WAVE][0], spec::WTRIP[WAVE][0] + spec::WTRIP[WAVE][1]>(s);
}
#endif

template <int JC, bool STAMPS, bool GEN, class PlanT>
__device__ __forceinline__ void resident_body(
    const PlanT& p, const int32_t* __restrict__ plan_itab, const double* __restrict__ plan_dtab,
    const SrcTable& src, const double* __restrict__ params, const double* __restrict__ given,
    double* __restrict__ P, double* __restrict__ q, double* __restrict__ G,
    double* __restrict__ h, int batch, int phases, unsigned long long* __restrict__ stamps) {
  extern __shared__ __attribute__((aligned(16))) double lds[];
  const int tid = threadIdx.x, lane = tid & 63;
  const int wave = __builtin_amdgcn_readfirstlane(tid >> 6);
  unsigned long long t_acc[8] = {0, 0, 0, 0, 0, 0, 0, 0}, t_prev = 0;
  const unsigned long long t_begin = STAMPS ? __builtin_amdgcn_s_memtime() : 0;
#define SETUP_STAMP(k)                                                                  \
  if (STAMPS && stamps != nullptr && lane == 0)                                         \
    stamps[((size_t)gridDim.x + blockIdx.x) * (NT / 64) * 8 + wave * 8 + (k)] =         \
        __builtin_amdgcn_s_memtime() - t_begin;
  const bool stamping = STAMPS && stamps != nullptr;
#define MPCASM_STAMP(slot)                                         \
  if (STAMPS && stamping) {                                        \
    const unsigned long long t_now = __builtin_amdgcn_s_memtime(); \
    t_acc[slot] += t_now - t_prev;                                 \
    t_prev = t_now;                                                \
  }
  const ResidentLayout L = resident_layout(p);
  const int no = p.no, nc = p.nc, ldv = p.rs_ldv, vd = p.rs_vd, ldp = L.ldp;

  double* V = lds + L.v;
  double* Pl = lds + L.pl;
  double* ql = lds + L.ql;
  double* dvec = lds + L.dvec;
  double2* dcoef = reinterpret_cast<double2*>(lds + L.dcoef);
  int4* dpar = reinterpret_cast<int4*>(lds + L.dpar);
  double* strm = lds + L.streams;
  int* itb = reinterpret_cast<int*>(lds + L.ints);
  int* rr = itb + L.i_rr;
  int2* meta = reinterpret_cast<int2*>(itb + L.i_meta);
  int* wtrip = itb + L.i_wtrip;
  int* split = itb + L.i_split;
  int* lti = itb + L.i_lti;
  int2* abmeta = reinterpret_cast<int2*>(itb + L.i_abmeta);
  int2* gdesc = reinterpret_cast<int2*>(itb + L.i_gdesc);
  int2* gfix = reinterpret_cast<int2*>(itb + L.i_gfix);
  int* rrwin = itb + L.i_rrwin;
  const unsigned img_lds = (unsigned)(uintptr_t)(lds + L.img);
  const int unit = p.rs_unit, nchunk = p.rs_nchunk;
  const int lx = lane & 3, lg = (lane >> 2) & 3, lk = lane >> 4;
  const unsigned ab_lds = (unsigned)(uintptr_t)(lds + L.ab);
  auto fetch_ab = [&](long inst, int slot) {
    for (int k = 0; k < p.rs_ab / 32; ++k) {
      const int2 m = abmeta[k * 64 + lane];
      const char* base = reinterpret_cast<const char* const*>(strm)[2 * m.x];
      const long long stride = reinterpret_cast<const long long*>(strm)[2 * m.x + 1];
      dma4(base + inst * stride + m.y,
           __builtin_amdgcn_readfirstlane(ab_lds + (unsigned)((slot * p.rs_ab + k * 32) * 8)));
    }
  };
  auto generate_sources = [&](int buf, int slot) {
    double* im = lds + L.img + buf * p.rs_img;
    const double* ab = lds + L.ab + slot * p.rs_ab;
    auto generate = [&](auto word) __attribute__((always_inline)) {
      const int n = word(LT_N), m = word(LT_M);
      const int N = word(LT_HORIZON), nn = n * n, nm = n * m;
      const double* Am = ab + word(LT_A);
      const double* Bm = ab + word(LT_B);
      double* TA = im + word(LT_TA);
      double* TB = im + word(LT_TB);
      double* TP = im + word(LT_TP);
      if (n <= 4 && n + m <= 4) {
        int lane_ = lane;
#ifdef MPCASM_SPEC
        asm volatile("" : "+v"(lane_));
#endif
        const int grp = lane_ >> 4, gi = lane_ & 3, gc = (lane_ >> 2) & 3;
        const bool live = gi < n && gc < n + m;
        double ar[4];
#pragma unroll
        for (int t = 0; t < 4; ++t) ar[t] = gi < n && t < n ? Am[gi * n + t] : 0.0;
        double x = !live ? 0.0 : (gc < m ? Bm[gi * m + gc] : Am[gi * n + (gc - m)]);
        double* out = gc < m ? TB + gi * m + gc : TA + gi * n + (gc - m);
        const int step = gc < m ? nm : nn;
        auto advance = [&]() {
          double y = ar[0] * quad_broadcast<0>(x);
          y = fma(ar[1], quad_broadcast<1>(x), y);
          y = fma(ar[2], quad_broadcast<2>(x), y);
          y = fma(ar[3], quad_broadcast<3>(x), y);
          x = y;
        };
        const int head = N < 4 ? N : 4;
        for (int d = 0; d < head; ++d) {
          if (live && grp == 0) out[d * step] = x;
          advance();
        }
        if (N > 4) {
          asm volatile("s_waitcnt lgkmcnt(0)" ::: "memory");
#pragma unroll
          for (int t = 0; t < 4; ++t) ar[t] = gi < n && t < n ? TA[3 * nn + gi * n + t] : 0.0;
          x = live ? out[grp * step] : 0.0;
          for (int d = grp + 4; d - grp < N; d += 4) {
            advance();
            if (live && d < N) out[d * step] = x;
          }
        }
        return;
      }
      for (int e = lane; e < nn; e += 64) {
        const double v = Am[e];
        TA[e] = v;
        TP[e] = v;
      }
      for (int e = lane; e < nm; e += 64) TB[e] = Bm[e];
      asm volatile("s_waitcnt lgkmcnt(0)" ::: "memory");
      int have = 1;
      for (int s_ = 0; have < N; ++s_) {
        const double* Pw = TP + s_ * nn;
        const int cnt = have < N - have ? have : N - have;
        const int na = cnt * nn, nb = cnt * nm, total = na + nb + nn;
        for (int e = lane; e < total; e += 64) {
          const double* X;
          double* out;
          int w, r;
          if (e < na) {
            const int d = e / nn;
            r = e - d * nn;
            X = TA + d * nn, out = TA + (have + d) * nn, w = n;
          } else if (e < na + nb) {
            const int d = (e - na) / nm;
            r = (e - na) - d * nm;
            X = TB + d * nm, out = TB + (have + d) * nm, w = m;
          } else {
            r = e - na - nb;
            X = Pw, out = TP + (s_ + 1) * nn, w = n;
          }
          const int i = r / w, j = r - i * w;
          double acc = 0.0;
          for (int t = 0; t < n; ++t) acc = fma(Pw[i * n + t], X[t * w + j], acc);
          out[r] = acc;
        }
        asm volatile("s_waitcnt lgkmcnt(0)" ::: "memory");
        have += cnt;
      }
    };
#ifdef MPCASM_SPEC
    if constexpr (PlanT::rs_nlti > 0) generate([](int k) { return spec::LTI[0][k]; });
    if constexpr (PlanT::rs_nlti > 1) generate([](int k) { return spec::LTI[1][k]; });
    if constexpr (PlanT::rs_nlti > 2) generate([](int k) { return spec::LTI[2][k]; });
    if constexpr (PlanT::rs_nlti > 3) generate([](int k) { return spec::LTI[3][k]; });
#else
    for (int g = 0; g < p.rs_nlti; ++g) {
      const int* rec = lti + g * RS_LTI_WORDS;
      generate([&](int k) { return __builtin_amdgcn_readfirstlane(rec[k]); });
    }
#endif
  };
  const int run_over = (phases >> 10) & 7;
  const int run_shift = run_over ? run_over : ((long)batch >= 16L * gridDim.x && !(phases & 256) ? 2 : 0);
  const unsigned vblock = (phases & 8192) && gridDim.x % 8 == 0
                              ? (blockIdx.x % 8) * (gridDim.x / 8) + blockIdx.x / 8 : blockIdx.x;
  auto instance_at = [&](int n) -> long {
    return ((((long)(n >> run_shift) * gridDim.x + vblock)) << run_shift) + (n & ((1 << run_shift) - 1));
  };
  const bool gen = GEN && p.rs_nlti != 0;
  const int ct = tid - 64, CT = NT - 64;
#ifdef MPCASM_SPEC
  constexpr int ZK = 2;
#else
  constexpr int ZK = 0;
#endif
  int v_zb[ZK > 0 ? ZK : 1];
  const int zt0 = tid >= MW * 64 ? tid - MW * 64 : tid + WT;
#pragma unroll
  for (int k = 0; k < ZK; ++k) {
    const int e = zt0 + k * NT;
    v_zb[k] = L.p_direct && e < p.rs_nzblk * 8 ? (plan_itab + p.off_rs_zblk)[e >> 3] : 0;
  }
  int c_sg[JC], c_dst[JC];
  double c_coef[JC];
  auto load_program = [&]() __attribute__((always_inline)) {
    const int4* prog = reinterpret_cast<const int4*>(plan_itab + p.off_rs_prog);
#pragma unroll
    for (int j = 0; j < JC; ++j) {
      const bool have = j < p.rs_jc;
      const int4 w = have ? prog[j * NT + tid] : int4{0, -1, 0, 0};
      c_sg[j] = w.x;
      c_dst[j] = w.y;
      c_coef[j] = __hiloint2double(w.w, w.z);
    }
  };
#ifdef MPCASM_SPEC
  constexpr int FK = JC <= 5 ? 3 : 0;
#else
  constexpr int FK = 0;
#endif
  const int32_t* gix = src.stride[MAX_SOURCES - 1] == -1
                           ? reinterpret_cast<const int32_t*>(src.ptr[MAX_SOURCES - 1]) : nullptr;
  const char* f_base[FK > 0 ? FK : 1];
  int f_stride[FK > 0 ? FK : 1];
  bool f_isg[FK > 0 ? FK : 1];
  bool f_shared[FK > 0 ? FK : 1];
  bool f_fast = FK > 0;
#ifdef MPCASM_SPEC
  constexpr bool prog_early = true;
#else
  constexpr bool prog_early = false;
#endif
  auto prepare_fetch = [&]() __attribute__((always_inline)) {
    if (FK > 0 && wave < MW) {
#pragma unroll
      for (int j = 0; j < FK; ++j) {
        const int k = wave + j * MW;
        const int2 m = meta[(k < nchunk ? k : 0) * 64 + lane];
        const long long stride = reinterpret_cast<const long long*>(strm)[2 * m.x + 1];
        f_base[j] = reinterpret_cast<const char* const*>(strm)[2 * m.x] + m.y;
        f_stride[j] = (int)stride;
        f_isg[j] = m.x == p.nsrc;
        f_shared[j] = __all(stride == 0);
        f_fast = f_fast && stride >= 0 && stride < (1ll << 31);
      }
    }
    f_fast = __builtin_amdgcn_readfirstlane(__all(f_fast));
  };
  auto fetch_image = [&](long inst, int buf, bool settled) {
    const unsigned dst0 = img_lds + (unsigned)buf * (unsigned)p.rs_img * 8u;
    const long ginst = gix != nullptr ? (long)gix[inst] : inst;
    int kfirst = wave;
    if (FK > 0 && f_fast) {
#pragma unroll
      for (int j = 0; j < FK; ++j) {
        const int k = wave + j * MW;
        if (k < nchunk && !(settled && f_shared[j])) {
          const char* a = f_base[j] + (unsigned long long)(f_isg[j] ? ginst : inst) * (unsigned)f_stride[j];
          const unsigned dst = __builtin_amdgcn_readfirstlane(dst0 + (unsigned)(k * 64 * unit));
          if (unit == 16)
            dma16(a, dst);
          else
            dma4(a, dst);
        }
      }
      kfirst = wave + FK * MW;
    }
    for (int k = kfirst; k < nchunk; k += MW) {
      const int2 m = meta[k * 64 + lane];
      const char* base = reinterpret_cast<const char* const*>(strm)[2 * m.x];
      const long long stride = reinterpret_cast<const long long*>(strm)[2 * m.x + 1];
      if (settled && __all(stride == 0)) continue;
      const char* a = base + (m.x == p.nsrc ? ginst : inst) * stride + m.y;
      const unsigned dst = __builtin_amdgcn_readfirstlane(dst0 + (unsigned)(k * 64 * unit));
      if (unit == 16)
        dma16(a, dst);
      else
        dma4(a, dst);
    }
  };
  if (wave == 0) {
    constexpr int MK = 2;
#ifdef MPCASM_SPEC
    constexpr int nltw = 0;
#else
    const int nltw = p.rs_nlti * RS_LTI_WORDS;
#endif
    const int nab2 = p.rs_ab * 2, nmeta = nchunk * 64;
    const int2* t_ab = reinterpret_cast<const int2*>(plan_itab + p.off_rs_abmeta);
    const int2* t_meta = reinterpret_cast<const int2*>(plan_itab + p.off_rs_inmeta);
    const int32_t* t_lti = plan_itab + p.off_rs_lti;
    int2 v_ab = int2{0, 0}, v_meta[MK];
    int v_lti = 0;
#ifdef MPCASM_SPEC
    constexpr bool ab_runs = spec_ab_by_runs();
    constexpr unsigned on_table = spec::FSEG_IMG_TABLE;
    constexpr bool img_runs = on_table == 0 && PlanT::rs_nchunk <= 32;
    constexpr int img_late = __builtin_popcount(on_table) + (PlanT::rs_nchunk > 32 ? PlanT::rs_nchunk - 32 : 0);
    const int ab_later = ab_runs ? nchunk : img_late;
    if (gen && ab_runs) {
      const long i1 = instance_at(1);
      spec_first_ab<0>(lane, instance_at(0), i1, i1 < batch, __builtin_amdgcn_readfirstlane(ab_lds), src, params,
                       given, plan_dtab);
    }
    if (ab_runs) SETUP_STAMP(2)
    {
      const long inst = instance_at(0), ginst = gix != nullptr ? (long)gix[inst] : inst;
      spec_first_image<0>(lane, inst, ginst, __builtin_amdgcn_readfirstlane(img_lds), src, params, given, plan_dtab);
    }
#else
    constexpr bool ab_runs = false, img_runs = false;
    constexpr unsigned on_table = ~0u;
    const int ab_later = nchunk;
#endif
    if (!ab_runs && lane < nab2) v_ab = t_ab[lane];
    if (lane < nltw) v_lti = t_lti[lane];
    if (!img_runs) {
#pragma unroll
      for (int k = 0; k < MK; ++k) v_meta[k] = lane + k * 64 < nmeta ? t_meta[lane + k * 64] : int2{0, 0};
    }
    if (prog_early) load_program();
    if (!ab_runs) {
      if (lane < nab2) abmeta[lane] = v_ab;
      for (int i = lane + 64; i < nab2; i += 64) abmeta[i] = t_ab[i];
    }
    if (lane < nltw) lti[lane] = v_lti;
    for (int i = lane + 64; i < nltw; i += 64) lti[i] = t_lti[i];
    if (!img_runs) {
#pragma unroll
      for (int k = 0; k < MK; ++k)
        if (lane + k * 64 < nmeta) meta[lane + k * 64] = v_meta[k];
      for (int i = lane + MK * 64; i < nmeta; i += 64) meta[i] = t_meta[i];
    }
#ifdef MPCASM_SPEC
    if constexpr (ab_runs) spec_write_table<true, 0>(abmeta, lane, src, params, given, plan_dtab);
    if constexpr (img_runs) spec_write_table<false, 0>(meta, lane, src, params, given, plan_dtab);
#endif
    for (int t = 0; t < p.nsrc + 3; ++t) {
      const int s = t - p.nsrc;
      const double* base = s < 0 ? src.ptr[t]
                                 : (s == 0 ? given : (s == 1 ? params : plan_dtab + p.doff_rs_const));
      const long long stride =
          s < 0 ? src.stride[t] : (s == 0 ? (long long)p.ng : (s == 1 ? (long long)p.nparams : 0));
      if (lane == 0) {
        reinterpret_cast<const double**>(strm)[2 * t] = base;
        reinterpret_cast<long long*>(strm)[2 * t + 1] = stride * (long long)sizeof(double);
      }
    }
    if (gen && !ab_runs) {
      fetch_ab(instance_at(0), 0);
      if (instance_at(1) < batch) fetch_ab(instance_at(1), 1);
    }
    if (!ab_runs) SETUP_STAMP(2)
    if (!img_runs) {
      const long inst = instance_at(0), ginst = gix != nullptr ? (long)gix[inst] : inst;
      for (int k = 0; k < nchunk; ++k) {
        if (k < 32 && !((on_table >> k) & 1)) continue;
        const int2 m = meta[k * 64 + lane];
        const char* base = reinterpret_cast<const char* const*>(strm)[2 * m.x];
        const long long stride = reinterpret_cast<const long long*>(strm)[2 * m.x + 1];
        const char* a = base + (m.x == p.nsrc ? ginst : inst) * stride + m.y;
        const unsigned dst = __builtin_amdgcn_readfirstlane(img_lds + (unsigned)(k * 64 * unit));
        if (unit == 16)
          dma16(a, dst);
        else
          dma4(a, dst);
      }
    }
    SETUP_STAMP(0)
    lds_barrier();
    SETUP_STAMP(1)
    prepare_fetch();
    SETUP_STAMP(3)
    if (gen) {
      dma_wait_but(ab_later);
      SETUP_STAMP(4)
      generate_sources(0, 0);
    }
    if (!prog_early) load_program();
    SETUP_STAMP(5)
  } else {
    SETUP_STAMP(0)
    lds_barrier();
    SETUP_STAMP(1)
    prepare_fetch();
    SETUP_STAMP(2)
    load_program();
    typedef int i32x4 __attribute__((ext_vector_type(4)));
    typedef int i32x2 __attribute__((ext_vector_type(2)));
    typedef double f64x2 __attribute__((ext_vector_type(2)));
    constexpr int RRK = 3;
    const int32_t* trr = plan_itab + p.off_rs_rr;
    const int nrr = p.rr_packed ? 0 : nc * RR_WORDS;
    int v_rr[RRK], v_wtrip = 0, v_split = 0, v_rrwin = 0;
    int2 v_gd[GU], v_gfix = int2{0, 0};
    i32x4 v_dpar = {0, 0, 0, 0};
    i32x2 v_rrc = {0, 0}, v_rrp = {0, 0};
    int v_rre = 0;
    f64x2 v_dcoef = {0.0, 0.0};
    const bool own_gd = resident_g_mode(p) == 2 && tid >= MW * 64;
    const bool own_diag = p.ndiag != 0 && ct >= 0 && ct < no;
    const int wt_ = tid - MW * 64;
    if (own_diag) {
      v_dpar = reinterpret_cast<const i32x4*>(plan_itab + p.off_rs_dpar)[ct];
      v_dcoef = reinterpret_cast<const f64x2*>(plan_dtab + p.doff_rs_dcoef)[ct];
    }
    if (ct >= 0) {
#pragma unroll
      for (int k = 0; k < RRK; ++k) v_rr[k] = ct + k * CT < nrr ? trr[ct + k * CT] : 0;
      if (ct < RS_WAVES * 2) v_wtrip = (plan_itab + p.off_rs_wtrip)[ct];
      if (ct < p.rs_nsplit) v_split = (plan_itab + p.off_rs_split)[ct];
      if (p.rr_packed && ct < nc) {
        v_rrc = *reinterpret_cast<const i32x2*>(trr + ct * RR_WORDS + RR_CENTER);
        v_rre = trr[ct * RR_WORDS + RR_EXTREME];
        v_rrp = *reinterpret_cast<const i32x2*>(trr + ct * RR_WORDS + RR_PACKED);
      }
      if (p.rs_compact && ct < nc) v_rrwin = (plan_itab + p.off_rs_rrwin)[ct];
    }
    if (own_gd) {
      const int2* gd = reinterpret_cast<const int2*>(plan_itab + p.off_rs_gdesc);
#pragma unroll
      for (int u = 0; u < GU; ++u) v_gd[u] = gd[u * WT + wt_];
      if (p.rs_ngfix != 0) v_gfix = reinterpret_cast<const int2*>(plan_itab + p.off_rs_gfix)[wt_];
    }
    if (ct >= 0) {
      if (!L.p_direct)
        for (int i = ct; i < no * ldp; i += CT) Pl[i] = 0.0;
      double2* V2 = reinterpret_cast<double2*>(V);
      const int n2 = resident_v_doubles(p) / 2;
      for (int i = ct; i < n2; i += CT) V2[i] = double2{0.0, 0.0};
      for (int i = ct; i < 2 * ldp; i += CT) dvec[i] = 0.0;
#pragma unroll
      for (int k = 0; k < RRK; ++k)
        if (ct + k * CT < nrr) rr[ct + k * CT] = v_rr[k];
      for (int i = ct + RRK * CT; i < nrr; i += CT) rr[i] = trr[i];
      if (p.rs_compact) {
        if (ct < nc) rrwin[ct] = v_rrwin;
        for (int R = ct + CT; R < nc; R += CT) rrwin[R] = (plan_itab + p.off_rs_rrwin)[R];
      }
      if (p.rr_packed) {
        static_assert(RR_CENTER == 8 && RR_EXTREME == 13 && RR_PACKED == 14, "the row record's second half");
        if (ct < nc)
          reinterpret_cast<int4*>(rr)[ct] = int4{v_rrp.x, v_rrp.y, v_rrc.x | (v_rrc.y << 16), v_rre};
        for (int R = ct + CT; R < nc; R += CT) {
          const int32_t* g = trr + R * RR_WORDS;
          reinterpret_cast<int4*>(rr)[R] =
              int4{g[RR_PACKED], g[RR_PACKED + 1], g[RR_CENTER] | (g[RR_CENTER + 1] << 16), g[RR_EXTREME]};
        }
      }
      if (resident_g_mode(p) == 3) {
        const int2* cg = reinterpret_cast<const int2*>(plan_itab + p.off_csc_g);
        for (int i = ct; i < p.csc_gnnz; i += CT) gdesc[i] = cg[i];
        for (int i = ct; i < p.csc_pnnz; i += CT) (itb + L.i_cscp)[i] = (plan_itab + p.off_csc_p)[i];
      }
      if (ct < RS_WAVES * 2) wtrip[ct] = v_wtrip;
      if (ct < p.rs_nsplit) split[ct] = v_split;
      for (int i = ct + CT; i < p.rs_nsplit; i += CT) split[i] = (plan_itab + p.off_rs_split)[i];
    }
    if (own_gd) {
#pragma unroll
      for (int u = 0; u < GU; ++u) gdesc[u * WT + wt_] = v_gd[u];
      if (p.rs_ngfix != 0) gfix[wt_] = v_gfix;
    }
    if (own_diag) {
      dpar[ct] = int4{v_dpar.x, v_dpar.y, v_dpar.z, v_dpar.w};
      dcoef[ct] = double2{v_dcoef.x, v_dcoef.y};
    }
    SETUP_STAMP(3)
    SETUP_STAMP(4)
    SETUP_STAMP(5)
  }
  lds_barrier();
  SETUP_STAMP(6)
  for (int r = tid; r < p.rtot; r += NT) V[(p.rs_vrow0 + r) * ldv + vd + 1] = 1.0;

  const bool lookahead = (phases & 128) != 0;
  if (wave == 0) dma_wait();
  SETUP_STAMP(7)

  const int wt = tid - MW * 64;
  const int npair = no >> 1;
  const int gtotal = nc * npair;
  const int g_mode = resident_g_mode(p);
  int zoff[ZK > 0 ? ZK : 1];
#pragma unroll
  for (int k = 0; k < ZK; ++k) {
    const int e = zt0 + k * NT;
    zoff[k] = -1;
    if (L.p_direct && e < p.rs_nzblk * 8) {
      const int z = v_zb[k], row = 4 * (z >> 8) + ((e >> 1) & 3), col = 4 * (z & 255) + 2 * (e & 1);
      if (row < no && col < no)
        zoff[k] = (row * no + col) | (col + 1 < no ? ((no & 1) == 0 ? 1 << 30 : 1 << 29) : 0);
    }
  }
  const bool skew = !(phases & 16384);
  const int g_rot = skew && gtotal % 8 == 0 && gtotal > 0 ? (int)((blockIdx.x * 53u) % (unsigned)(gtotal / 8)) * 8 : 0;
  const int g_e0 = wt >= 0 && gtotal > 0 ? (wt + g_rot) % gtotal : 0;
  const int g_first = wt >= 0 && npair > 0 ? ((g_e0 / npair) << 16) | (g_e0 % npair) : 0;
  const int g_dR = npair > 0 ? WT / npair : 0, g_dcp = npair > 0 ? WT % npair : 0;


  const auto g_packed = [&](double* Gb, const double* V, const double* prm) __attribute__((always_inline)) {
    double2* G2 = reinterpret_cast<double2*>(Gb);
    int first = g_first;
    asm volatile("" : "+v"(first));
    int R = first >> 16, cp = first & 0xFFFF;
    for (int e0 = wt; e0 < gtotal; e0 += 3 * WT) {
      int2 ds[3];
      int c2[3], wn[3], at[3];
#pragma unroll
      for (int u = 0; u < 3; ++u) {
        const int Rr = e0 + u * WT < gtotal ? R : 0;
        ds[u] = *reinterpret_cast<const int2*>(rr + Rr * RR_COMPACT);
        wn[u] = p.rs_compact ? rrwin[Rr] : 0;
        c2[u] = 2 * cp;
        at[u] = Rr * npair + cp;
        cp += g_dcp;
        R += g_dR;
        if (cp >= npair) {
          cp -= npair;
          ++R;
        }
        if (R >= nc) R -= nc;
      }
      double a0[3], a1[3];
      double2 v0[3], v1[3];
      if (p.rs_compact) {
#pragma unroll
        for (int u = 0; u < 3; ++u) {
          const unsigned win = (unsigned)wn[u], cpair = (unsigned)c2[u] >> 1;
          const unsigned d0 = cpair - (win & 255), d1 = cpair - ((win >> 16) & 255);
          const bool in0 = d0 < ((win >> 8) & 255), in1 = d1 < (win >> 24);
          a0[u] = prm[in0 ? ds[u].y & 0xFFFF : p.nparams];
          a1[u] = prm[in1 ? (unsigned)ds[u].y >> 16 : p.nparams];
          v0[u] = *reinterpret_cast<const double2*>(V + (ds[u].x & 0xFFFF) + (in0 ? 2 * d0 : 0));
          v1[u] = *reinterpret_cast<const double2*>(V + ((unsigned)ds[u].x >> 16) + (in1 ? 2 * d1 : 0));
        }
      } else {
#pragma unroll
        for (int u = 0; u < 3; ++u) {
          a0[u] = prm[ds[u].y & 0xFFFF];
          a1[u] = prm[(unsigned)ds[u].y >> 16];
          v0[u] = *reinterpret_cast<const double2*>(V + (ds[u].x & 0xFFFF) + c2[u]);
          v1[u] = *reinterpret_cast<const double2*>(V + ((unsigned)ds[u].x >> 16) + c2[u]);
        }
      }
#pragma unroll
      for (int u = 0; u < 3; ++u) {
        const int e = e0 + u * WT;
        double2 r;
        r.x = fma(a1[u], v1[u].x, a0[u] * v0[u].x);
        r.y = fma(a1[u], v1[u].y, a0[u] * v0[u].y);
        if (e < gtotal) store_result(&G2[at[u]], r);
      }
    }
  };

  if (STAMPS && stamping) t_prev = __builtin_amdgcn_s_memtime();
  int buf = 0, iter = 0;
  for (long inst = instance_at(0); inst < batch; inst = instance_at(iter + 1), buf ^= 1, ++iter) {
    const double* img = lds + L.img + buf * p.rs_img;
    const double* prm = img + p.rs_img_params;
    lds_barrier();
    MPCASM_STAMP(0)

    auto compose = [&]() {
      if (p.ndiag != 0) {
        int c = tid;
        asm volatile("" : "+v"(c));
        if (c < no) {
          const int4 par = dpar[c];
          const double2 co = dcoef[c];
          const double w0 = prm[par.x], a0 = prm[par.y], w1 = prm[par.z], a1 = prm[par.w];
          dvec[c] = (w0 * co.x) * co.x + (w1 * co.y) * co.y;
          dvec[ldp + c] = w0 * (co.x * (0.0 - a0)) + w1 * (co.y * (0.0 - a1));
        }
      }
      if (phases & 1) {
        double va[JC], vg[JC];
  #pragma unroll
        for (int j = 0; j < JC; ++j) {
          va[j] = img[c_sg[j] & 0xFFFF];
          vg[j] = img[(unsigned)c_sg[j] >> 16];
        }
        double acc = 0.0;
  #pragma unroll
        for (int j = 0; j < JC; ++j) {
          acc += c_coef[j] * va[j] * vg[j];
          if (c_dst[j] >= 0) {
            if (c_dst[j] & RS_DST_ACC)
              __hip_atomic_fetch_add(&V[c_dst[j] & ~RS_DST_ACC], acc, __ATOMIC_RELAXED,
                                     __HIP_MEMORY_SCOPE_WORKGROUP);
            else
              V[c_dst[j]] = acc;
          }
          acc = c_dst[j] >= 0 ? 0.0 : acc;
        }
      }
    };
    const long nxt = instance_at(iter + 1), nxt2 = instance_at(iter + 2);
    if (wave < MW) {
      compose();
      lds_barrier();
      MPCASM_STAMP(1)
      __builtin_amdgcn_s_setprio(2);
      if (lookahead && nxt < batch && (phases & 16)) fetch_image(nxt, buf ^ 1, iter >= 1);
      if (wave == 0 && (GEN && p.rs_nlti != 0) && nxt2 < batch) fetch_ab(nxt2, buf);
      MPCASM_STAMP(7)
      if (wave == MW - 1 && (GEN && p.rs_nlti != 0) && nxt < batch) generate_sources(buf ^ 1, buf ^ 1);
    } else {
      compose();
      lds_barrier();
      MPCASM_STAMP(1)
      if (G != nullptr && (phases & 8)) {
        double* Gb = G + (size_t)inst * nc * no;
        if (g_mode == 3) {
          double* Gd = G + (size_t)inst * p.csc_gnnz;
          int w_ = wt;
          asm volatile("" : "+v"(w_));
          for (int e0 = w_; e0 < p.csc_gnnz; e0 += 3 * WT) {
            int2 ds[3];
#pragma unroll
            for (int u = 0; u < 3; ++u) ds[u] = gdesc[min(e0 + u * WT, p.csc_gnnz - 1)];
            double a0[3], a1[3], v0[3], v1[3];
#pragma unroll
            for (int u = 0; u < 3; ++u) {
              a0[u] = prm[ds[u].y & 0xFFFF];
              v0[u] = V[ds[u].x & 0xFFFF];
              if (!p.csc_gsingle) {
                a1[u] = prm[(unsigned)ds[u].y >> 16];
                v1[u] = V[(unsigned)ds[u].x >> 16];
              }
            }
#pragma unroll
            for (int u = 0; u < 3; ++u)
              if (e0 + u * WT < p.csc_gnnz)
                Gd[e0 + u * WT] = p.csc_gsingle ? a0[u] * v0[u] : fma(a1[u], v1[u], a0[u] * v0[u]);
          }
        } else if (g_mode == 2) {
          double2* G2 = reinterpret_cast<double2*>(Gb);
          int wt_ = wt;
          asm volatile("" : "+v"(wt_));
          const bool all_single = p.rs_gsingle == (1 << (GU * (WT / 64))) - 1;
#ifdef MPCASM_SPEC
          constexpr int GB = spec::PlanConst::rs_gsingle == (1 << (GU * (WT / 64))) - 1 ? GU : 3;
#else
          constexpr int GB = 3;
#endif
          static_assert(GU % GB == 0, "batches of pieces");
          const bool h_mine = wt_ < nc;
          int fix_u = RS_GFIX_NONE;
          double fa1 = 0.0;
          double2 fv1{0.0, 0.0};
          int2 fd{0, 0};
          if (p.rs_ngfix != 0) fd = gfix[wt_];
          const int4 hc4 = reinterpret_cast<const int4*>(rr)[h_mine ? wt_ : 0];
          const int4 hr = int4{0, hc4.w, hc4.x, hc4.y};
          const int2 hc = int2{hc4.z & 0xFFFF, (int)((unsigned)hc4.z >> 16)};
          double ha0 = 0.0, ha1 = 0.0, hc0 = 0.0, hc1 = 0.0, hd0 = 0.0, hd1 = 0.0, hext = 0.0;
#pragma unroll
          for (int u0 = 0; u0 < GU; u0 += GB) {
            int2 ds[GB];
#pragma unroll
            for (int u = 0; u < GB; ++u) ds[u] = gdesc[(u0 + u) * WT + wt_];
            if (u0 == 0 && p.rs_ngfix != 0) {
              fix_u = (unsigned)fd.x >> 16;
              fa1 = prm[fd.y];
              fv1 = *reinterpret_cast<const double2*>(V + (fd.x & 0xFFFF));
            }
            if (u0 == 0) {
              ha0 = prm[hr.w & 0xFFFF];
              ha1 = prm[(unsigned)hr.w >> 16];
              hc0 = prm[hc.x];
              hc1 = prm[hc.y];
              hd0 = V[(hr.z & 0xFFFF) + vd];
              hd1 = V[((unsigned)hr.z >> 16) + vd];
              hext = prm[hr.y];
            }
            double a0[GB], a1[GB];
            double2 v0[GB], v1[GB];
            bool one[GB];
#pragma unroll
            for (int u = 0; u < GB; ++u) {
              one[u] = all_single || ((p.rs_gsingle >> ((u0 + u) * (WT / 64) + (wave - MW))) & 1);
              a0[u] = prm[ds[u].y & 0xFFFF];
              v0[u] = *reinterpret_cast<const double2*>(V + (ds[u].x & 0xFFFF));
              if (!one[u]) {
                a1[u] = prm[(unsigned)ds[u].y >> 16];
                v1[u] = *reinterpret_cast<const double2*>(V + ((unsigned)ds[u].x >> 16));
              }
            }
#pragma unroll
            for (int u = 0; u < GB; ++u) {
              const int e = wt_ + (u0 + u) * WT;
              double2 r;
              if (one[u]) {
                r.x = a0[u] * v0[u].x;
                r.y = a0[u] * v0[u].y;
                if (p.rs_ngfix != 0 && u0 + u == fix_u) {
                  r.x = fma(fa1, fv1.x, r.x);
                  r.y = fma(fa1, fv1.y, r.y);
                }
              } else {
                r.x = fma(a1[u], v1[u].x, a0[u] * v0[u].x);
                r.y = fma(a1[u], v1[u].y, a0[u] * v0[u].y);
              }
              if (e < gtotal && !((phases & 512) && r.x == r.x))
                store_result(&G2[e], r);
            }
            if (u0 == 0 && h_mine) {
              double ac = ha0 * hc0, ad = ha0 * hd0;
              ac += ha1 * hc1;
              ad = fma(ha1, hd1, ad);
              (h + (size_t)inst * nc)[wt_] = (hext + ac) - ad;
            }
          }
        } else if (g_mode == 1) {
          g_packed(Gb, V, prm);
        } else if ((no & 1) == 0) {
          int w_ = wt;
          asm volatile("" : "+v"(w_));
          const int dR = WT / npair, dcp = WT - dR * npair;
          int e = w_, R = w_ / npair, cp = w_ - (w_ / npair) * npair;
          double2* G2 = reinterpret_cast<double2*>(Gb);
          while (e < gtotal) {
            const int* rec = rr + R * RR_WORDS;
            const int naxes = rec[RR_NAXES];
            double2 accv{0.0, 0.0};
            for (int ax = 0; ax < naxes; ++ax) {
              const double a = prm[rec[RR_ARROW + ax]];
              const double2 v = *reinterpret_cast<const double2*>(V + rec[RR_VOFF + ax] + 2 * cp);
              accv.x = fma(a, v.x, accv.x);
              accv.y = fma(a, v.y, accv.y);
            }
            store_result(&G2[e], accv);
            e += WT;
            cp += dcp;
            R += dR;
            if (cp >= npair) {
              cp -= npair;
              ++R;
            }
          }
        } else {
          int w_ = wt;
          asm volatile("" : "+v"(w_));
          const int total = nc * no;
          const int dR = WT / no, dc = WT - dR * no;
          int e = w_, R = w_ / no, c = w_ - (w_ / no) * no;
          while (e < total) {
            const int* rec = rr + R * RR_WORDS;
            const int naxes = rec[RR_NAXES];
            double accv = 0.0;
            for (int ax = 0; ax < naxes; ++ax)
              accv = fma(prm[rec[RR_ARROW + ax]], V[rec[RR_VOFF + ax] + c], accv);
            store_result(&Gb[e], accv);
            e += WT;
            c += dc;
            R += dR;
            if (c >= no) {
              c -= no;
              ++R;
            }
          }
        }
        double* hb = h + (size_t)inst * nc;
        int Rh = g_mode == 2 ? wt + WT : wt;
        asm volatile("" : "+v"(Rh));
        for (int R = Rh; R < nc; R += WT) {
          if (p.rr_packed) {
            const int4 c = reinterpret_cast<const int4*>(rr)[R];
            const double a0 = prm[c.y & 0xFFFF], a1 = prm[(unsigned)c.y >> 16];
            double ac = a0 * prm[c.z & 0xFFFF], ad = a0 * V[(c.x & 0xFFFF) + vd];
            ac += a1 * prm[(unsigned)c.z >> 16];
            ad = fma(a1, V[((unsigned)c.x >> 16) + vd], ad);
            hb[R] = (prm[c.w] + ac) - ad;
            continue;
          }
          const int* rec = rr + R * RR_WORDS;
          const int naxes = rec[RR_NAXES];
          double ac = 0.0, ad = 0.0;
          for (int ax = 0; ax < naxes; ++ax) {
            const double a = prm[rec[RR_ARROW + ax]];
            ac += a * prm[rec[RR_CENTER + ax]];
            ad = fma(a, V[rec[RR_VOFF + ax] + vd], ad);
          }
          hb[R] = (prm[rec[RR_EXTREME]] + ac) - ad;
        }
      }
      MPCASM_STAMP(3)
      __builtin_amdgcn_s_setprio(2);
    }
#ifdef MPCASM_SPEC
    if (P != nullptr && (phases & 2)) {
      static_assert(RS_WAVES == 8, "one case per wavefront");
      TripState st;
      st.Vlane = reinterpret_cast<const char*>(V) + resident_trip_row(lk) * (ldv * 8) + lx * 8;
      st.prc = reinterpret_cast<const char*>(prm);
      st.Pl = L.p_direct ? P + (size_t)inst * no * no : Pl;
      st.ldpl = L.p_direct ? no : ldp;
      st.ql = ql;
      st.dvec = dvec;
      st.lx = lx, st.lg = lg, st.lk = lk;
      st.ap = st.bp = st.Vlane;
      st.bi = st.bj = 0;
      st.isq = st.live = false;
      st.acc = st.sum = 0.0;
      switch (wave) {
        case 0: spec_wave_trips<0>(st); break;
        case 1: spec_wave_trips<1>(st); break;
        case 2: spec_wave_trips<2>(st); break;
        case 3: spec_wave_trips<3>(st); break;
        case 4: spec_wave_trips<4>(st); break;
        case 5: spec_wave_trips<5>(st); break;
        case 6: spec_wave_trips<6>(st); break;
        default: spec_wave_trips<7>(st); break;
      }
    }
#else
    if (P != nullptr && (phases & 2)) {
      const int t0 = __builtin_amdgcn_readfirstlane(wtrip[2 * wave]);
      const int tn = __builtin_amdgcn_readfirstlane(wtrip[2 * wave + 1]);
      typedef int i32x8 __attribute__((ext_vector_type(8)));
      typedef const __attribute__((address_space(4))) i32x8* const_i32x8_ptr;
      const_i32x8_ptr tg = (const_i32x8_ptr)(uintptr_t)(plan_itab + p.off_rs_trip) + t0;
      if (tn > 0) {
        const char* prc = reinterpret_cast<const char*>(prm);
        const int row_bytes = ldv * (int)sizeof(double);
        const int short_shift = (lk - resident_trip_row(lk)) * row_bytes;
        const char* Vlane = reinterpret_cast<const char*>(V) + resident_trip_row(lk) * row_bytes + lx * 8;
        const char *ap = Vlane, *bp = Vlane;
        int bi = 0, bj = 0;
        bool isq = false, live = false;
        i32x8 rn = tg[0];
        double acc = 0.0, sum = 0.0;
        for (int t = 0; t < tn; ++t) {
          const i32x8 r = rn;
          rn = tg[t + 1];
          const int word = r[RT_WORD];
          if ((word >> RT_FIRST) & 1) {
            bi = (r[RT_BI] >> (8 * lg)) & 255;
            bj = (r[RT_BJ] >> (8 * lg)) & 255;
            isq = (word >> (RT_QMASK + lg)) & 1;
            live = (word >> (RT_LIVE + lg)) & 1;
            ap = Vlane + bi * 32;
            bp = Vlane + (isq ? 0 : bj * 32);
            acc = 0.0;
          }
          if (word & 31) {
            const int boff = isq ? r[RT_D] : r[RT_B];
            if (!((word >> RT_SHORT) & 1)) {
              sum = mfma_trip16_at((unsigned)(uintptr_t)(ap + r[RT_A]), (unsigned)(uintptr_t)(bp + boff),
                                   (unsigned)row_bytes, sum);
            } else {
              const double a = *reinterpret_cast<const double*>(ap + (r[RT_A] + short_shift));
              const double b = *reinterpret_cast<const double*>(bp + (boff + short_shift));
              sum = mfma_f64_4x4x4(a, b, sum);
            }
            if ((word >> RT_TERM_END) & 1) {
              const double w = *reinterpret_cast<const double*>(prc + r[RT_W]);
              if (word & ((15 << RT_QMASK) | (1 << RT_NOP))) {
                const double aim = *reinterpret_cast<const double*>(prc + r[RT_AIM]);
                const double ws = (word >> RT_HALF) & 1 ? 0.5 * w : w;
                const double ones = quad_broadcast<1>(sum);
                const double m = isq ? ws : ((word >> RT_NOP) & 1 ? 0.0 : w);
                acc = fma(m, fma(-(isq ? aim : 0.0), ones, sum), acc);
              } else {
                acc = fma(w, sum, acc);
              }
              sum = 0.0;
            }
          }
          if ((word >> RT_LAST) & 1) {
            const int row = 4 * bi + lk, col = 4 * bj + lx;
            if (live && row < no) {
              if (isq) {
                if (lx == 0) ql[row] = acc + dvec[ldp + row];
              } else if (col < no) {
                const double val = acc + (row == col ? dvec[col] : 0.0);
                double* Pout = L.p_direct ? P + (size_t)inst * no * no : Pl;
                const int ldo = L.p_direct ? no : ldp;
                Pout[row * ldo + col] = val;
                if (p.rs_sym && bi != bj) Pout[col * ldo + row] = val;
              }
            }
          }
        }
      }
    }
#endif
    MPCASM_STAMP(2)
    __builtin_amdgcn_s_setprio(0);
    lds_barrier();
    MPCASM_STAMP(4)

    if (wave < MW) {
      if (!lookahead && nxt < batch && (phases & 16)) fetch_image(nxt, buf ^ 1, iter >= 1);
      dma_wait();
      for (int i = tid; i < p.rs_nsplit; i += MW * 64) V[split[i]] = 0.0;
    }
    MPCASM_STAMP(5)
    if (P != nullptr && (phases & 32)) {
      double* Pb = P + (size_t)inst * no * no;
      int t_ = tid >= MW * 64 ? tid - MW * 64 : tid + WT;
      asm volatile("" : "+v"(t_));
      if (L.p_direct) {
#pragma unroll
        for (int k = 0; k < ZK; ++k)
          if (zoff[k] >= 0) {
            double* z = Pb + (zoff[k] & 0xFFFFFF);
            if (zoff[k] & (1 << 30))
              *reinterpret_cast<double2*>(z) = double2{0.0, 0.0};
            else {
              z[0] = 0.0;
              if (zoff[k] & (1 << 29)) z[1] = 0.0;
            }
          }
        const int32_t* zb = plan_itab + p.off_rs_zblk;
        for (int e = t_ + ZK * NT; e < p.rs_nzblk * 8; e += NT) {
          const int z = zb[e >> 3], row = 4 * (z >> 8) + ((e >> 1) & 3), col = 4 * (z & 255) + 2 * (e & 1);
          if (row < no && col < no) {
            if (col + 1 < no && ((no & 1) == 0))
              *reinterpret_cast<double2*>(Pb + (size_t)row * no + col) = double2{0.0, 0.0};
            else {
              Pb[(size_t)row * no + col] = 0.0;
              if (col + 1 < no) Pb[(size_t)row * no + col + 1] = 0.0;
            }
          }
        }
      } else if (g_mode == 3) {
        double* Pd = P + (size_t)inst * p.csc_pnnz;
        const int* cp = itb + L.i_cscp;
        for (int e = t_; e < p.csc_pnnz; e += NT) Pd[e] = Pl[cp[e]];
      } else if ((no & 1) == 0) {
        const int total = no * npair;
        double2* P2 = reinterpret_cast<double2*>(Pb);
        const double2* Pl2 = reinterpret_cast<const double2*>(Pl);
        const int rot = skew && total % 8 == 0 ? (int)((blockIdx.x * 37u) % (unsigned)(total / 8)) * 8 : 0;
        for (int e = t_; e < total; e += NT) {
          const int at = e + rot < total ? e + rot : e + rot - total;
          store_result(&P2[at], Pl2[at]);
        }
      } else {
        for (int e = t_; e < no * no; e += NT) {
          const int row = e / no;
          store_result(&Pb[e], Pl[row * ldp + (e - row * no)]);
        }
      }
      double* qb = q + (size_t)inst * no;
      for (int c = t_; c < no; c += NT) qb[c] = ql[c];
    }
    MPCASM_STAMP(6)
  }
  if (STAMPS && stamping && lane == 0) {
#pragma unroll
    for (int i = 0; i < 8; ++i) stamps[((size_t)blockIdx.x * (NT / 64) + wave) * 8 + i] = t_acc[i];
  }
#undef MPCASM_STAMP
#undef SETUP_STAMP
}

#ifdef MPCASM_SPEC
}
#ifndef MPCASM_SPEC_WAVES_PER_EU
#define MPCASM_SPEC_WAVES_PER_EU 4
#endif
extern "C" __global__ __launch_bounds__(RS_NT, MPCASM_SPEC_WAVES_PER_EU) void resident_spec_kernel(
    const int32_t* __restrict__ plan_itab, const double* __restrict__ plan_dtab, SrcTable src,
    const double* __restrict__ params, const double* __restrict__ given, double* __restrict__ P,
    double* __restrict__ q, double* __restrict__ G, double* __restrict__ h, int batch, int phases,
    unsigned long long* __restrict__ stamps) {
  constexpr spec::PlanConst p{};
#ifdef MPCASM_SPEC_STAMPS
  constexpr bool stamped = true;
#else
  constexpr bool stamped = false;
#endif
#ifdef MPCASM_SPEC_PHASES
  const int mask = MPCASM_SPEC_PHASES;
#else
  const int mask = phases;
#endif
  resident_body<spec::JC, stamped, spec::PlanConst::rs_nlti != 0>(p, plan_itab, plan_dtab, src, params,
                                                               given, P, q, G, h, batch, mask, stamps);
}
namespace {
#else
template <int JC, bool STAMPS, bool GEN>
__global__ __launch_bounds__(NT, 4) void resident_assemble_kernel(
    PlanDev p, SrcTable src, const double* __restrict__ params, const double* __restrict__ given,
    double* __restrict__ P, double* __restrict__ q, double* __restrict__ G,
    double* __restrict__ h, int batch, int phases, unsigned long long* __restrict__ stamps) {
  resident_body<JC, STAMPS, GEN>(p, p.itab, p.dtab, src, params, given, P, q, G, h, batch, phases,
                                 stamps);
}
#endif

#ifndef __HIPCC_RTC__

template <int JC>
int launch_jc(const PlanDev& p, const SrcTable& src, const double* params, const double* given,
              double* P, double* q, double* G, double* h, void* work, int batch, size_t lds_bytes,
              int num_cus, hipStream_t stream, hipError_t* err) {
  auto kernel = (g_phase_mask & 64) ? resident_assemble_kernel<JC, true, true>
                : p.rs_nlti != 0    ? resident_assemble_kernel<JC, false, true>
                                    : resident_assemble_kernel<JC, false, false>;
  struct Residency {
    int device;
    size_t lds;
    int per_cu;
  };
  constexpr int KEPT = 8;
  static thread_local Residency kept[3][KEPT];
  static thread_local int nkept[3] = {0, 0, 0};
  const int slot = (g_phase_mask & 64) ? 2 : (p.rs_nlti != 0 ? 1 : 0);
  int device = 0;
  (void)hipGetDevice(&device);
  int found = -1;
  for (int i = 0; i < nkept[slot]; ++i)
    if (kept[slot][i].device == device && kept[slot][i].lds == lds_bytes) found = kept[slot][i].per_cu;
  if (found < 0) {
    if (lds_bytes > 64 * 1024) {
      *err = allow_whole_lds(reinterpret_cast<const void*>(kernel));
      if (*err != hipSuccess) return MPCASM_ERR_HIP;
    }
    int n = 0;
    *err = hipOccupancyMaxActiveBlocksPerMultiprocessor(&n, kernel, NT, lds_bytes);
    if (*err != hipSuccess) return MPCASM_ERR_HIP;
    found = n;
    const int at = nkept[slot] < KEPT ? nkept[slot]++ : (int)(lds_bytes % KEPT);
    kept[slot][at] = Residency{device, lds_bytes, n};
  }
  int per_cu = found;
  if (per_cu < 1) return MPCASM_ERR_LIMIT;
  if (t_per_cu > 0 && t_per_cu < per_cu) per_cu = t_per_cu;
  long grid = (long)num_cus * per_cu;
  if (t_grid > 0 && t_grid < grid) grid = t_grid;
  if (grid > batch) grid = batch;
  hipLaunchKernelGGL(kernel, dim3((unsigned)grid), dim3(NT), lds_bytes, stream, p, src, params,
                     given, P, q, G, h, batch, g_phase_mask,
                     (g_phase_mask & 64) ? static_cast<unsigned long long*>(work) : nullptr);
  *err = hipGetLastError();
  return *err == hipSuccess ? MPCASM_OK : MPCASM_ERR_HIP;
}
#endif

}

#ifndef __HIPCC_RTC__
int resident_choose_p_direct(const PlanDev& p, int option) {
  PlanDev q = p;
  q.rs_p_direct = 0;
  const bool fits = (size_t)resident_layout(q).total_doubles * sizeof(double) <= (size_t)RESIDENT_LDS_LIMIT;
  return (!fits || option == 1) ? 1 : (option == 2 ? 0 : 2);
}

int resident_p_direct_for(const PlanDev& p, int batch) {
  if (p.rs_p_direct != 2) return p.rs_p_direct;
  PlanDev q = p;
  q.rs_p_direct = 0;
  const size_t with_p = (size_t)resident_layout(q).total_doubles * sizeof(double);
  q.rs_p_direct = 1;
  const size_t without = (size_t)resident_layout(q).total_doubles * sizeof(double);
  constexpr size_t HALF_CU = 80 * 1024;
  const double per_instance = 8.0 * ((double)p.no * p.no + p.no + (double)p.nc * p.no + p.nc);
  if (with_p > HALF_CU && without <= HALF_CU && per_instance < 128.0 * 1024) return 1;
  return per_instance * batch < 560e6 ? 1 : 0;
}

size_t resident_lds_bytes(const PlanDev& p) {
  if (!p.rs_ok || p.rs_jc > RS_JC_MAX || p.no > WT || p.no < 1 || p.max_axes > AXMAX) return 0;
  if ((long)(p.rs_vrow0 + p.rtot) * p.rs_ldv > (1 << 20)) return 0;
  return (size_t)resident_layout(p).total_doubles * sizeof(double);
}

bool resident_inputs_aligned(const PlanDev& p, const SrcTable& src, const double* params,
                             const double* given) {
  if (p.rs_unit != 16) return true;
  auto ok = [](const void* base, long long stride) {
    return (reinterpret_cast<uintptr_t>(base) & 15) == 0 && (stride & 1) == 0;
  };
  for (int s = 0; s < p.nsrc; ++s)
    if (((p.rs_src16 >> s) & 1) && !ok(src.ptr[s], src.stride[s])) return false;
  return ok(given, p.ng) && ok(params, p.nparams);
}

int launch_assemble_resident(const PlanDev& p, const SrcTable& src, const double* params,
                             const double* given, double* P, double* q, double* G, double* h,
                             void* work, int batch, size_t lds_bytes, int num_cus,
                             hipStream_t stream, hipError_t* err) {
#define MPCASM_RS_ARGS p, src, params, given, P, q, G, h, work, batch, lds_bytes, num_cus, stream, err
  if (p.rs_jc <= 3) return launch_jc<3>(MPCASM_RS_ARGS);
  if (p.rs_jc <= 4) return launch_jc<4>(MPCASM_RS_ARGS);
  if (p.rs_jc <= 5) return launch_jc<5>(MPCASM_RS_ARGS);
  if (p.rs_jc <= 8) return launch_jc<8>(MPCASM_RS_ARGS);
  return launch_jc<RS_JC_MAX>(MPCASM_RS_ARGS);
#undef MPCASM_RS_ARGS
}
#endif

}
```

mpc-interface_amd/mpcasm/capi.py:

```python
import ctypes
import os

_HERE = os.path.dirname(os.path.abspath(__file__))
LIB_PATH = os.environ.get("MPCASM_LIB") or os.path.join(_HERE, "libmpcasm.so")

OK = 0
ERR_LIMIT = -5
OPT_PATH = 1
OPT_PHASE_MASK = 2
OPT_RESIDENT_PER_CU = 3
OPT_RESIDENT_GRID = 6
OPT_P_DIRECT = 5
OPT_JIT_FETCH_RUNS = 7
OPT_JIT = 4
PHASE_DEFAULT = 0xBF
PHASE_STAMPS = 0x40
STATUS = {
    0: "MPCASM_OK",
    -1: "MPCASM_ERR_ARG",
    -2: "MPCASM_ERR_PLAN",
    -3: "MPCASM_ERR_HIP",
    -4: "MPCASM_ERR_NODEVICE",
    -5: "MPCASM_ERR_LIMIT",
}
QP_SOLVED, QP_MAX_ITER, QP_PRIMAL_INFEASIBLE, QP_DUAL_INFEASIBLE, QP_NON_CVX = 1, -2, -3, -4, -7
QP_STATUS = {
    1: "MPCASM_QP_SOLVED",
    -2: "MPCASM_QP_MAX_ITER",
    -3: "MPCASM_QP_PRIMAL_INFEASIBLE",
    -4: "MPCASM_QP_DUAL_INFEASIBLE",
    -7: "MPCASM_QP_NON_CVX",
}
ROLL_GIVEN, ROLL_OPTIM, ROLL_STATE, ROLL_REC_WORDS = 0, 1, 2, 8
ERR_ARG = -1
GIVEN_KEEP, GIVEN_CONST = -1, -2


def qp_bit(status):
    return 1 << abs(int(status))

_c_double_p = ctypes.POINTER(ctypes.c_double)
_void_p = ctypes.c_void_p
SIGNATURES = {
    "mpcasm_abi_version": (ctypes.c_int, []),
    "mpcasm_device_count": (ctypes.c_int, []),
    "mpcasm_last_hip": (ctypes.c_int, []),
    "mpcasm_status_string": (ctypes.c_char_p, [ctypes.c_int]),
    "mpcasm_set_option": (ctypes.c_int, [ctypes.c_int, ctypes.c_int]),
    "mpcasm_fill_su": (ctypes.c_int, [_void_p, _void_p, _void_p, _void_p, ctypes.c_int,
                                      ctypes.c_int, ctypes.c_int, ctypes.c_int, ctypes.c_int,
                                      _void_p]),
    "mpcasm_plan_create": (ctypes.c_int, [_void_p, ctypes.c_size_t, _void_p, ctypes.c_size_t,
                                          ctypes.POINTER(_void_p)]),
    "mpcasm_plan_destroy": (ctypes.c_int, [_void_p]),
    "mpcasm_resident_lds_bytes": (ctypes.c_int, [_void_p, ctypes.c_size_t, _void_p, ctypes.c_size_t,
                                                 ctypes.POINTER(ctypes.c_int64)]),
    "mpcasm_jit_check": (ctypes.c_int, [_void_p, ctypes.c_size_t, _void_p, ctypes.c_size_t,
                                        ctypes.c_char_p, ctypes.c_size_t]),
    "mpcasm_fetch_segments": (ctypes.c_int, [_void_p, ctypes.c_size_t, _void_p, ctypes.c_size_t, ctypes.c_int,
                                             _void_p, ctypes.c_size_t, ctypes.POINTER(ctypes.c_int64)]),
    "mpcasm_preview_route": (ctypes.c_int, [_void_p, ctypes.c_size_t, _void_p, ctypes.c_size_t,
                                            ctypes.POINTER(ctypes.c_int64), ctypes.c_int, ctypes.c_int,
                                            ctypes.POINTER(ctypes.c_int32)]),
    "mpcasm_sweep_route": (ctypes.c_int, [_void_p, ctypes.c_size_t, _void_p, ctypes.c_size_t,
                                          ctypes.POINTER(ctypes.c_int32)]),
    "mpcasm_tiled_route": (ctypes.c_int, [_void_p, ctypes.c_size_t, _void_p, ctypes.c_size_t,
                                          ctypes.POINTER(ctypes.c_int64), ctypes.c_int, ctypes.c_int, ctypes.c_int,
                                          ctypes.POINTER(ctypes.c_int32)]),
    "mpcasm_plan_sizes": (ctypes.c_int, [_void_p, ctypes.POINTER(ctypes.c_int64)]),
    "mpcasm_plan_csc_sizes": (ctypes.c_int, [_void_p, ctypes.POINTER(ctypes.c_int64)]),
    "mpcasm_plan_set_option": (ctypes.c_int, [_void_p, ctypes.c_int, ctypes.c_int]),
    "mpcasm_assemble_indexed": (ctypes.c_int, [_void_p, ctypes.POINTER(_void_p),
                                               ctypes.POINTER(ctypes.c_int64), _void_p, _void_p, _void_p,
                                               _void_p, _void_p, _void_p, _void_p, _void_p, ctypes.c_int,
                                               _void_p]),
    "mpcasm_plan_last_kernel": (ctypes.c_int, [_void_p]),
    "mpcasm_plan_prepare": (ctypes.c_int, [_void_p, ctypes.c_int]),
    "mpcasm_jit_stats": (ctypes.c_int, [ctypes.POINTER(ctypes.c_int64)]),
    "mpcasm_workspace_bytes": (ctypes.c_int, [_void_p, ctypes.c_int,
                                              ctypes.POINTER(ctypes.c_size_t)]),
    "mpcasm_assemble": (ctypes.c_int, [_void_p, ctypes.POINTER(_void_p),
                                       ctypes.POINTER(ctypes.c_int64), _void_p, _void_p, _void_p,
                                       _void_p, _void_p, _void_p, _void_p, ctypes.c_int, _void_p]),
    "mpcasm_preview_matrices": (ctypes.c_int, [_void_p, ctypes.POINTER(_void_p),
                                               ctypes.POINTER(ctypes.c_int64), _void_p,
                                               ctypes.c_int, _void_p]),
    "mpcasm_preview": (ctypes.c_int, [_void_p, _void_p, _void_p, _void_p, ctypes.c_int,
                                      ctypes.c_int, ctypes.c_int, ctypes.c_int, _void_p]),
    "mpcasm_preview_direct": (ctypes.c_int, [_void_p, ctypes.POINTER(_void_p),
                                             ctypes.POINTER(ctypes.c_int64), _void_p, _void_p,
                                             _void_p, _void_p, ctypes.c_int, _void_p]),
    "mpcasm_goal_distance": (ctypes.c_int, [_void_p, ctypes.c_int64, _void_p, ctypes.c_int64,
                                            _void_p, ctypes.c_int, ctypes.c_int, _void_p,
                                            ctypes.c_int, _void_p]),
    "mpcasm_preview_goal_distance": (ctypes.c_int, [_void_p, ctypes.POINTER(_void_p),
                                                    ctypes.POINTER(ctypes.c_int64), _void_p, _void_p,
                                                    _void_p, _void_p, ctypes.c_int, ctypes.c_int,
                                                    _void_p, _void_p, ctypes.c_int, _void_p]),
    "mpcasm_admm": (ctypes.c_int, [ctypes.c_int, ctypes.c_int] + [_void_p] * 8 + [ctypes.c_double] * 3 +
                    [ctypes.c_int, ctypes.c_int, ctypes.c_int, _void_p, ctypes.c_int, _void_p]),
    "mpcasm_qp_solve": (ctypes.c_int, [ctypes.c_int, ctypes.c_int] + [_void_p] * 7 + [ctypes.c_int, _void_p] +
                        [ctypes.c_double] * 6 + [ctypes.c_int] * 3 + [_void_p] * 3 +
                        [ctypes.c_int, _void_p, ctypes.c_int, _void_p]),
    "mpcasm_qp_solve_lds_bytes": (ctypes.c_int, [ctypes.c_int, ctypes.c_int, ctypes.POINTER(ctypes.c_int64)]),
    "mpcasm_qp_solve_wide": (ctypes.c_int, [ctypes.c_int, ctypes.c_int] + [_void_p] * 7 + [ctypes.c_int, _void_p] +
                             [ctypes.c_double] * 6 + [ctypes.c_int] * 3 + [_void_p] * 3 +
                             [ctypes.c_int, _void_p, ctypes.c_int, _void_p]),
    "mpcasm_qp_solve_wide_info": (ctypes.c_int, [ctypes.c_int, ctypes.c_int, ctypes.POINTER(ctypes.c_int64),
                                                 ctypes.POINTER(ctypes.c_int32)]),
    "mpcasm_given_map_compile": (ctypes.c_int, [_void_p, _void_p, _void_p, ctypes.c_int, _void_p, ctypes.c_int64,
                                                ctypes.POINTER(ctypes.c_int64)]),
    "mpcasm_next_given": (ctypes.c_int, [_void_p, ctypes.POINTER(_void_p), ctypes.POINTER(ctypes.c_int64), _void_p,
                                         ctypes.c_int64, _void_p, _void_p, _void_p, ctypes.c_uint32, _void_p,
                                         ctypes.c_int64, _void_p, ctypes.c_int, _void_p]),
    "mpcasm_ltv_rollout_compile": (ctypes.c_int, [_void_p, ctypes.c_size_t, _void_p, ctypes.c_size_t, _void_p, _void_p,
                                                  ctypes.c_int, _void_p, ctypes.c_int, _void_p, ctypes.c_int64,
                                                  ctypes.POINTER(ctypes.c_int64)]),
    "mpcasm_ltv_rollout": (ctypes.c_int, [_void_p, ctypes.POINTER(_void_p), ctypes.POINTER(ctypes.c_int64), _void_p,
                                          ctypes.c_int64, _void_p, _void_p, _void_p, ctypes.c_int64, _void_p,
                                          ctypes.c_int, _void_p]),
    "mpcasm_ltv_advance": (ctypes.c_int, [_void_p, ctypes.POINTER(_void_p), ctypes.POINTER(ctypes.c_int64), _void_p,
                                          ctypes.c_int64, _void_p, _void_p, _void_p, ctypes.c_uint32, _void_p,
                                          ctypes.c_int64, ctypes.c_int, _void_p]),
    "mpcasm_gather": (ctypes.c_int, [_void_p, ctypes.c_int64, _void_p, ctypes.c_int, _void_p,
                                     ctypes.c_int, _void_p]),
    "mpcasm_box_transform": (ctypes.c_int, [_void_p, ctypes.c_int64, ctypes.c_int, _void_p,
                                            ctypes.c_int, ctypes.c_int, _void_p, ctypes.c_int64,
                                            _void_p]),
    "mpcasm_box_transform_ss": (ctypes.c_int, [_void_p, ctypes.c_int64, ctypes.c_int, _void_p,
                                               ctypes.c_int, ctypes.c_int, _void_p, ctypes.c_int,
                                               ctypes.c_int, _void_p, ctypes.c_int64, _void_p]),
}
KERNEL_NAMES = {0: "none", 1: "resident_assemble_kernel (persistent, ahead of time)",
                2: "resident_spec_kernel (persistent, compiled for the plan by hiprtc)",
                3: "fused_assemble_kernel", 4: "staged pipeline (compose_rowsets / hessian / constraints)",
                5: "tiled_assemble_kernel",
                6: "toeplitz_scan_kernel (tiled, scan form: P summed along diagonals)",
                7: "ltv_sweep_kernel (per-step dynamics, no horizon matrix)",
                8: "shared_p_kernel / shared_g_kernel (tiled, shared-model form: weighted sums of per-term matrices)"}
PREVIEW_NONE, PREVIEW_DIRECT, PREVIEW_STAGED, PREVIEW_BLOCKED = range(4)
PREVIEW_ROUTES = {0: "none", 1: "direct", 2: "staged", 3: "blocked"}
TILED_SCAN, TILED_TOEPLITZ, TILED_SHARED, TILED_GENERAL = range(1, 5)
TILED_FORMS = {1: "scan", 2: "toeplitz", 3: "shared", 4: "general"}
TILED_TABLES_NONE, TILED_TABLES_SMALL, TILED_TABLES_SYSTEM = range(3)
WANT_COST, WANT_CONSTRAINTS = 1, 2
BOX_RECENTER, BOX_TRANSLATE, BOX_ROTATE, BOX_SCALE, BOX_MARGIN = range(5)


class MpcasmError(RuntimeError):

    def __init__(self, status, where, hip=0):
        self.status = status
        self.hip = hip
        msg = "%s failed: %s" % (where, STATUS.get(status, str(status)))
        if hip:
            msg += " (hipError_t %d)" % hip
        super().__init__(msg)


_lib = None


def load():
    global _lib
    if _lib is None:
        if not os.path.exists(LIB_PATH):
            raise RuntimeError(
                "libmpcasm.so is missing (%s): build it with `make -C mpc-interface_amd` "
                "or __graft_entry__.build(); the assembly kernels have no fallback" % LIB_PATH
            )
        try:
            import torch
        except ImportError:
            pass
        lib = ctypes.CDLL(LIB_PATH)
        for name, (restype, argtypes) in SIGNATURES.items():
            fn = getattr(lib, name)
            fn.restype = restype
            fn.argtypes = argtypes
        _lib = lib
    return _lib


def check(status, where):
    if status != OK:
        raise MpcasmError(status, where, load().mpcasm_last_hip())
```

Before: 179.1 million assemblies/s.

## Preload front kernel arguments into SGPRs and reorder spec kernel arg layout

Reorders the JIT spec kernel's arguments so the pointers and strides needed by the first fetches (two front source streams, constants, a packed grid/flag word, first index) sit at the start of the kernarg segment. It compiles with the LLVM kernarg-preload option so those arguments arrive in SGPRs instead of needing scalar loads. The goal is to cut kernel-start latency before the first global requests are issued. In exchange the argument list grows, SrcTable reads are deferred, and there is an extra front/non-front template instantiation with a new grid size limit check.

```diff
diff --git a/include/mpcasm.h b/include/mpcasm.h
--- a/include/mpcasm.h
+++ b/include/mpcasm.h
@@ -25,7 +25,8 @@
 int mpcasm_last_hip(void);
 const char* mpcasm_status_string(int status);
 enum { MPCASM_OPT_PATH = 1, MPCASM_OPT_PHASE_MASK = 2, MPCASM_OPT_RESIDENT_PER_CU = 3, MPCASM_OPT_JIT = 4,
-       MPCASM_OPT_P_DIRECT = 5, MPCASM_OPT_RESIDENT_GRID = 6, MPCASM_OPT_JIT_FETCH_RUNS = 7 };
+       MPCASM_OPT_P_DIRECT = 5, MPCASM_OPT_RESIDENT_GRID = 6, MPCASM_OPT_JIT_FETCH_RUNS = 7,
+       MPCASM_OPT_JIT_KERNARG_PRELOAD = 8 };
 int mpcasm_set_option(int option, int value);
 int mpcasm_plan_set_option(mpcasm_plan* plan, int option, int value);
 int mpcasm_resident_lds_bytes(const int32_t* h_itab, size_t n_itab, const double* h_dtab, size_t n_dtab,
@@ -34,6 +35,7 @@
                      char* log, size_t log_capacity);
 int mpcasm_fetch_segments(const int32_t* h_itab, size_t n_itab, const double* h_dtab, size_t n_dtab,
                           int limit, int32_t* out, size_t capacity, int64_t* n_words);
+int mpcasm_spec_kernarg_layout(int32_t* out, size_t capacity, int64_t* n_words);
 
 int mpcasm_plan_prepare(const mpcasm_plan* plan, int batch);
 int mpcasm_jit_stats(int64_t out[3]);
diff --git a/mpc-interface_amd/csrc/capi.hip b/mpc-interface_amd/csrc/capi.hip
--- a/mpc-interface_amd/csrc/capi.hip
+++ b/mpc-interface_amd/csrc/capi.hip
@@ -1103,6 +1103,11 @@
     g_resident_grid = value;
     return MPCASM_OK;
   }
+  if (option == MPCASM_OPT_JIT_KERNARG_PRELOAD) {
+    if (value < 0 || value > SPEC_PRELOAD_MAX) return MPCASM_ERR_ARG;
+    g_jit_kernarg_preload = value;
+    return MPCASM_OK;
+  }
   return MPCASM_ERR_ARG;
 }
 
@@ -1230,7 +1235,7 @@
     for (int form : {small, large}) {
       if (form == large && small != large && out != MPCASM_OK) break;
       d.rs_p_direct = form;
-      out = jit_code_for(jit_spec_header(d, h_itab, g_jit_fetch_runs), false, 0xBF, &code, &text) ? MPCASM_OK : MPCASM_ERR_HIP;
+      out = jit_code_for(jit_spec_header(d, h_itab, g_jit_fetch_runs), false, 0xBF, g_jit_kernarg_preload, &code, &text) ? MPCASM_OK : MPCASM_ERR_HIP;
       if (small == large) break;
     }
   }
@@ -1239,6 +1244,15 @@
     log[log_capacity - 1] = 0;
   }
   return out;
+}
+
+int mpcasm_spec_kernarg_layout(int32_t* out, size_t capacity, int64_t* n_words) {
+  if (!n_words || (capacity && !out)) return MPCASM_ERR_ARG;
+  const std::vector<int32_t> words = jit_kernarg_layout();
+  *n_words = (int64_t)words.size();
+  if (words.size() > capacity) return MPCASM_ERR_LIMIT;
+  memcpy(out, words.data(), words.size() * sizeof(int32_t));
+  return MPCASM_OK;
 }
 
 int mpcasm_fetch_segments(const int32_t* h_itab, size_t n_itab, const double* h_dtab, size_t n_dtab,
diff --git a/mpc-interface_amd/csrc/jit.h b/mpc-interface_amd/csrc/jit.h
--- a/mpc-interface_amd/csrc/jit.h
+++ b/mpc-interface_amd/csrc/jit.h
@@ -11,15 +11,17 @@
 
 extern int g_jit;
 extern int g_jit_fetch_runs;
+extern int g_jit_kernarg_preload;
 extern int g_phase_mask;
 
 std::string jit_spec_header(const PlanDev& d, const int32_t* h_itab, int seg_limit = FS_MAX);
 std::vector<int32_t> jit_fetch_plan(const PlanDev& d, const int32_t* h_itab, int seg_limit);
 int jit_compile(const std::string& header, std::vector<char>* code, std::string* log,
-                bool stamps = false, int phases = 0xBF);
+                bool stamps = false, int phases = 0xBF, int preload = SPEC_PRELOAD_MAX);
+std::vector<int32_t> jit_kernarg_layout();
 const void* jit_kernel_for(const PlanDev& d, const int32_t* h_itab, int device, int batch,
                            size_t lds_bytes);
-bool jit_code_for(const std::string& header, bool stamps, int phases, std::vector<char>* code,
+bool jit_code_for(const std::string& header, bool stamps, int phases, int preload, std::vector<char>* code,
                   std::string* log, bool distrust_disk = false);
 bool jit_available();
 void jit_stats(long out[3]);
diff --git a/mpc-interface_amd/csrc/jit.hip b/mpc-interface_amd/csrc/jit.hip
--- a/mpc-interface_amd/csrc/jit.hip
+++ b/mpc-interface_amd/csrc/jit.hip
@@ -15,6 +15,7 @@
 #include <map>
 #include <mutex>
 #include <string>
+#include <type_traits>
 #include <vector>
 
 #include "jit.h"
@@ -24,6 +25,7 @@
 
 int g_jit = 0;
 int g_jit_fetch_runs = FS_MAX;
+int g_jit_kernarg_preload = SPEC_PRELOAD_MAX;
 
 namespace {
 
@@ -74,6 +76,12 @@
 
 }
 
+struct SpecArgs {
+#define MPCASM_X(type, qual, name) type name;
+  MPCASM_SPEC_KERNEL_ARGS(MPCASM_X, MPCASM_NOTHING)
+#undef MPCASM_X
+};
+
 std::vector<int32_t> jit_fetch_segments(const int32_t* meta, int lanes) {
   std::vector<int32_t> out;
   for (int i = 0; i < lanes;) {
@@ -108,6 +116,20 @@
     }
   }
   return out;
+}
+
+void jit_front_streams(const PlanDev& d, const int32_t* it, int limit, int out[2]) {
+  out[0] = out[1] = -1;
+  const std::vector<int32_t> fetch = jit_fetch_plan(d, it, limit);
+  for (size_t at = 0; at < fetch.size(); at += 3 + fetch[at + 2] * FS_WORDS)
+    for (int g = 0; g < fetch[at + 2]; ++g) {
+      const int stream = fetch[at + 3 + g * FS_WORDS + FS_STREAM];
+      if (stream >= d.nsrc || stream == out[0] || stream == out[1]) continue;
+      if (out[0] < 0)
+        out[0] = stream;
+      else if (out[1] < 0)
+        out[1] = stream;
+    }
 }
 
 std::string jit_spec_header(const PlanDev& d, const int32_t* it, int seg_limit) {
@@ -159,6 +181,10 @@
     s += std::string("constexpr unsigned FSEG_") + name + "_TABLE = ";
     append(s, "%lldu;\n", on_table);
   }
+  int front[2];
+  jit_front_streams(d, it, seg_limit, front);
+  append(s, "constexpr int FRONT_SRC[2] = {%lld, ", front[0]);
+  append(s, "%lld};\n", front[1]);
   s += "constexpr int LTI[4][8] = {\n";
   for (int g = 0; g < RS_LTI_MAX; ++g) {
     s += "  {";
@@ -171,7 +197,7 @@
 }
 
 int jit_compile(const std::string& header, std::vector<char>* code, std::string* log, bool stamps,
-                int phases) {
+                int phases, int preload) {
   const Rtc& r = rtc();
   if (!r.ok) {
     if (log) *log = "libhiprtc.so could not be loaded";
@@ -187,8 +213,14 @@
                             : (getenv("MPCASM_JIT_PLAIN_STORES") ? "-DMPCASM_PLAIN_STORES=1" : "-DMPCASM_SPEC_NT=1");
   char popt[48];
   snprintf(popt, sizeof popt, "-DMPCASM_SPEC_PHASES=%d", phases);
-  const char* opts[] = {"--offload-arch=gfx950", "-O3", "-std=c++17", "-DMPCASM_SPEC=1", wopt.c_str(), last, popt};
-  const int rc = r.compile(prog, phases >= 0 ? 7 : 6, opts);
+  const std::string kopt = "-amdgpu-kernarg-preload-count=" + std::to_string(preload);
+  std::vector<const char*> opts = {"--offload-arch=gfx950", "-O3", "-std=c++17", "-DMPCASM_SPEC=1", wopt.c_str(), last};
+  if (phases >= 0) opts.push_back(popt);
+  if (preload > 0) {
+    opts.push_back("-mllvm");
+    opts.push_back(kopt.c_str());
+  }
+  const int rc = r.compile(prog, (int)opts.size(), opts.data());
   size_t n = 0;
   if (log && r.log_size(prog, &n) == 0 && n > 1) {
     log->resize(n);
@@ -296,6 +328,7 @@
   hipFunction_t fn = nullptr;
   int per_cu = 0;
   size_t lds = 0;
+  int front[2] = {-1, -1};
   bool failed = false;
   bool building = true;
 };
@@ -305,9 +338,10 @@
 std::map<std::pair<int, std::string>, JitKernel*> g_cache;
 struct FastKey {
   const void* itab;
-  int device, p_direct, phases, fetch_runs;
+  int device, p_direct, phases, fetch_runs, preload;
   bool operator<(const FastKey& o) const {
     if (fetch_runs != o.fetch_runs) return fetch_runs < o.fetch_runs;
+    if (preload != o.preload) return preload < o.preload;
     if (itab != o.itab) return itab < o.itab;
     if (device != o.device) return device < o.device;
     if (p_direct != o.p_direct) return p_direct < o.p_direct;
@@ -318,11 +352,11 @@
 
 }
 
-bool jit_code_for(const std::string& header, bool stamps, int phases, std::vector<char>* code,
+bool jit_code_for(const std::string& header, bool stamps, int phases, int preload, std::vector<char>* code,
                   std::string* log_out, bool distrust_disk) {
   const char* waves = getenv("MPCASM_JIT_WAVES_PER_EU");
   const std::string options = std::string(stamps ? "stamps " : "") + "phases " + std::to_string(phases) +
-                              " waves " + (waves ? waves : "4") +
+                              " waves " + (waves ? waves : "4") + " kernarg-preload " + std::to_string(preload) +
                               (getenv("MPCASM_JIT_PLAIN_STORES") ? " plain-stores" : "");
   const std::string dir = cache_dir();
   const std::string path = dir.empty() ? "" : dir + "/" + cache_key(header, options) + ".co";
@@ -333,7 +367,7 @@
     return true;
   }
   std::string log;
-  const int rc = jit_compile(header, code, &log, stamps, phases);
+  const int rc = jit_compile(header, code, &log, stamps, phases, preload);
   if (log_out) *log_out = log;
   if (rc != MPCASM_OK) {
     if (getenv("MPCASM_JIT_VERBOSE")) fprintf(stderr, "mpcasm: jit failed:\n%s\n", log.c_str());
@@ -352,8 +386,9 @@
                            size_t lds_bytes) {
   if (t_jit == 2) return nullptr;
   const bool stamps = (g_phase_mask & 64) != 0;
-  const int phases = stamps ? -1 : g_phase_mask;
-  const FastKey fast{d.itab, stamps ? device + 4096 : device, d.rs_p_direct, phases, g_jit_fetch_runs};
+  const int phases = g_phase_mask;
+  const FastKey fast{d.itab, stamps ? device + 4096 : device, d.rs_p_direct, phases, g_jit_fetch_runs,
+                     g_jit_kernarg_preload};
   const bool may_build = t_jit == 1 || batch >= JIT_MIN_BATCH;
   JitKernel* slot = nullptr;
   bool mine = false;
@@ -365,7 +400,8 @@
       slot = found->second;
     } else if (may_build) {
       header = jit_spec_header(d, h_itab, fast.fetch_runs);
-      JitKernel*& by_text = g_cache[std::make_pair(fast.device, header + "//" + std::to_string(phases))];
+      JitKernel*& by_text = g_cache[std::make_pair(
+          fast.device, header + "//" + std::to_string(phases) + "//" + std::to_string(fast.preload))];
       if (by_text == nullptr) {
         by_text = new JitKernel();
         mine = true;
@@ -388,7 +424,7 @@
     for (int attempt = 0; attempt < 2 && !ok; ++attempt) {
       code.clear();
       const long hits = g_stat_disk_hits;
-      ok = jit_code_for(header, stamps, phases, &code, nullptr, attempt == 1);
+      ok = jit_code_for(header, stamps, phases, fast.preload, &code, nullptr, attempt == 1);
       const bool from_disk = g_stat_disk_hits != hits;
       if (ok && (hipModuleLoadData(&module, code.data()) != hipSuccess ||
                  hipModuleGetFunction(&fn, module, "resident_spec_kernel") != hipSuccess)) {
@@ -413,6 +449,7 @@
     }
     {
       std::lock_guard<std::mutex> lock(g_mutex);
+      jit_front_streams(d, h_itab, fast.fetch_runs, slot->front);
       slot->module = module;
       slot->fn = fn;
       slot->failed = !ok;
@@ -437,6 +474,16 @@
 }
 
 bool jit_available() { return rtc().ok; }
+
+std::vector<int32_t> jit_kernarg_layout() {
+  std::vector<int32_t> out;
+#define MPCASM_X(type, qual, name)                                                                     \
+  out.insert(out.end(), {(int32_t)offsetof(SpecArgs, name), (int32_t)sizeof(type),                     \
+                         std::is_pointer<type>::value ? 0 : (std::is_integral<type>::value && sizeof(type) == 4 ? 1 : 2)});
+  MPCASM_SPEC_KERNEL_ARGS(MPCASM_X, MPCASM_NOTHING)
+#undef MPCASM_X
+  return out;
+}
 
 void jit_stats(long out[3]) {
   out[0] = g_stat_compiled;
@@ -460,12 +507,45 @@
   long grid = (long)num_cus * per_cu;
   if (grid_limit > 0 && grid_limit < grid) grid = grid_limit;
   if (grid > batch) grid = batch;
-  const int32_t* itab = p.itab;
-  const double* dtab = p.dtab;
-  SrcTable s = src;
-  int phases = g_phase_mask;
-  unsigned long long* stamps = (g_phase_mask & 64) ? static_cast<unsigned long long*>(work) : nullptr;
-  void* args[] = {&itab, &dtab, &s, &params, &given, &P, &q, &G, &h, &batch, &phases, &stamps};
+  if (grid < 0 || grid >= (1l << (32 - SPEC_WORD_GRID))) {
+    *err = hipSuccess;
+    return MPCASM_ERR_LIMIT;
+  }
+  SpecArgs a;
+  a.plan_itab = p.itab;
+  a.plan_dtab = p.dtab;
+  a.src = src;
+  a.params = params;
+  a.given = given;
+  a.P = P, a.q = q, a.G = G, a.h = h;
+  a.batch = batch;
+  a.phases = g_phase_mask;
+  a.stamps = (g_phase_mask & 64) ? static_cast<unsigned long long*>(work) : nullptr;
+  a.consts = p.dtab + p.doff_rs_const;
+  a.front_word = (unsigned)grid << SPEC_WORD_GRID;
+  a.first_index = nullptr;
+  if (src.stride[MAX_SOURCES - 1] == -1) {
+    a.front_word |= SPEC_WORD_GIX;
+    a.first_index = reinterpret_cast<const int32_t*>(src.ptr[MAX_SOURCES - 1]);
+  }
+  const double* fptr[2] = {nullptr, nullptr};
+  unsigned fstride[2] = {0, 0};
+  bool fits = true;
+  for (int i = 0; i < 2; ++i) {
+    const int t = k->front[i];
+    if (t < 0) continue;
+    fptr[i] = src.ptr[t];
+    fits = fits && src.stride[t] >= 0 && src.stride[t] <= 0xFFFFFFFFll;
+    fstride[i] = (unsigned)src.stride[t];
+  }
+  if (fits) a.front_word |= SPEC_WORD_FRONT;
+  a.front_ptr0 = fptr[0], a.front_ptr1 = fptr[1];
+  a.front_stride0 = fits ? fstride[0] : 0, a.front_stride1 = fits ? fstride[1] : 0;
+  void* args[] = {
+#define MPCASM_X(type, qual, name) &a.name,
+      MPCASM_SPEC_KERNEL_ARGS(MPCASM_X, MPCASM_NOTHING)
+#undef MPCASM_X
+  };
   *err = hipModuleLaunchKernel(k->fn, (unsigned)grid, 1, 1, RS_NT, 1, 1, (unsigned)k->lds, stream,
                                args, nullptr);
   return *err == hipSuccess ? MPCASM_OK : MPCASM_ERR_HIP;
diff --git a/mpc-interface_amd/csrc/plan_dev.h b/mpc-interface_amd/csrc/plan_dev.h
--- a/mpc-interface_amd/csrc/plan_dev.h
+++ b/mpc-interface_amd/csrc/plan_dev.h
@@ -47,4 +47,28 @@
   long long stride[MAX_SOURCES];
 };
 
+#define MPCASM_SPEC_KERNEL_ARGS(X, S)                                                              \
+  X(const double*, , front_ptr0) S() X(const double*, , front_ptr1) S()                             \
+  X(const double*, __restrict__, given) S() X(const double*, __restrict__, params) S()              \
+  X(const double*, , consts) S() X(unsigned, , front_stride0) S() X(unsigned, , front_stride1) S()  \
+  X(int, , batch) S() X(unsigned, , front_word) S()                                                 \
+  X(const int32_t*, __restrict__, plan_itab) S() X(const double*, __restrict__, plan_dtab) S()      \
+  X(SrcTable, , src) S() X(double*, __restrict__, P) S() X(double*, __restrict__, q) S()            \
+  X(double*, __restrict__, G) S() X(double*, __restrict__, h) S() X(int, , phases) S()              \
+  X(unsigned long long*, __restrict__, stamps) S() X(const int32_t*, , first_index)
+#define MPCASM_COMMA() ,
+#define MPCASM_NOTHING()
+
+constexpr int SPEC_PRELOAD_MAX = 14;
+constexpr unsigned SPEC_WORD_GIX = 1u, SPEC_WORD_FRONT = 2u;
+constexpr int SPEC_WORD_GRID = 8;
+
+struct SpecFront {
+  const double* ptr[2];
+  unsigned stride[2];
+  const double* consts;
+  unsigned word;
+  const int32_t* first_index;
+};
+
 }
diff --git a/mpc-interface_amd/csrc/resident.hip b/mpc-interface_amd/csrc/resident.hip
--- a/mpc-interface_amd/csrc/resident.hip
+++ b/mpc-interface_amd/csrc/resident.hip
@@ -221,9 +221,9 @@
   else
     return K < spec::PlanConst::rs_nchunk ? spec::FSEG_IMG_N[K] : 0;
 }
-template <bool AB, int K, int S>
+template <bool FRONT, bool AB, int K, int S>
 __device__ __forceinline__ void spec_lane_run(LaneSrc& out, int lane, const SrcTable& src, const double* params,
-                                              const double* given, const double* plan_dtab) {
+                                              const double* given, const SpecFront& fr) {
   using PC = spec::PlanConst;
   if constexpr (S < spec_fetch_runs<AB, K>()) {
     constexpr int first = AB ? spec::FSEG_AB[K][S][FS_FIRST] : spec::FSEG_IMG[K][S][FS_FIRST];
@@ -235,7 +235,13 @@
     static_assert(period >= lanes || (period & (period - 1)) == 0, "a periodic run repeats every 1, 2 or 4 lanes");
     const char* base;
     long long stride;
-    if constexpr (stream < PC::nsrc) {
+    if constexpr (FRONT && stream < PC::nsrc && stream == spec::FRONT_SRC[0]) {
+      base = reinterpret_cast<const char*>(fr.ptr[0]);
+      stride = (long long)fr.stride[0] * (long long)sizeof(double);
+    } else if constexpr (FRONT && stream < PC::nsrc && stream == spec::FRONT_SRC[1]) {
+      base = reinterpret_cast<const char*>(fr.ptr[1]);
+      stride = (long long)fr.stride[1] * (long long)sizeof(double);
+    } else if constexpr (stream < PC::nsrc) {
       base = reinterpret_cast<const char*>(src.ptr[stream]);
       stride = src.stride[stream] * (long long)sizeof(double);
     } else if constexpr (stream == PC::nsrc) {
@@ -245,7 +251,7 @@
       base = reinterpret_cast<const char*>(params);
       stride = (long long)PC::nparams * (long long)sizeof(double);
     } else {
-      base = reinterpret_cast<const char*>(plan_dtab + PC::doff_rs_const);
+      base = reinterpret_cast<const char*>(fr.consts);
       stride = 0;
     }
     const int rel = lane - first;
@@ -256,52 +262,67 @@
       out.isg = stream == PC::nsrc;
       out.entry = int2{stream, off};
     }
-    spec_lane_run<AB, K, S + 1>(out, lane, src, params, given, plan_dtab);
+    spec_lane_run<FRONT, AB, K, S + 1>(out, lane, src, params, given, fr);
   }
 }
-template <bool AB, int K>
+template <bool FRONT, bool AB, int K>
 __device__ __forceinline__ LaneSrc spec_lane_src(int lane, const SrcTable& src, const double* params,
-                                                 const double* given, const double* plan_dtab) {
+                                                 const double* given, const SpecFront& fr) {
   LaneSrc out{nullptr, 0, false, int2{0, 0}};
-  spec_lane_run<AB, K, 0>(out, lane, src, params, given, plan_dtab);
+  spec_lane_run<FRONT, AB, K, 0>(out, lane, src, params, given, fr);
   return out;
 }
 template <bool AB, int K>
 __device__ __forceinline__ void spec_write_table(int2* table, int lane, const SrcTable& src, const double* params,
-                                                 const double* given, const double* plan_dtab) {
+                                                 const double* given, const SpecFront& fr) {
   if constexpr (K < (AB ? spec::PlanConst::rs_ab / 32 : spec::PlanConst::rs_nchunk)) {
-    table[K * 64 + lane] = spec_lane_src<AB, K>(lane, src, params, given, plan_dtab).entry;
-    spec_write_table<AB, K + 1>(table, lane, src, params, given, plan_dtab);
+    table[K * 64 + lane] = spec_lane_src<true, AB, K>(lane, src, params, given, fr).entry;
+    spec_write_table<AB, K + 1>(table, lane, src, params, given, fr);
   }
 }
-template <int K>
+template <bool FRONT, int K>
 __device__ __forceinline__ void spec_first_ab(int lane, long inst0, long inst1, bool two, unsigned ab_lds,
                                               const SrcTable& src, const double* params, const double* given,
-                                              const double* plan_dtab) {
+                                              const SpecFront& fr) {
   using PC = spec::PlanConst;
   if constexpr (K < PC::rs_ab / 32) {
-    const LaneSrc m = spec_lane_src<true, K>(lane, src, params, given, plan_dtab);
+    const LaneSrc m = spec_lane_src<FRONT, true, K>(lane, src, params, given, fr);
     dma4(m.base + inst0 * m.stride, ab_lds + (unsigned)(K * 32 * 8));
     if (two) dma4(m.base + inst1 * m.stride, ab_lds + (unsigned)((PC::rs_ab + K * 32) * 8));
-    spec_first_ab<K + 1>(lane, inst0, inst1, two, ab_lds, src, params, given, plan_dtab);
+    spec_first_ab<FRONT, K + 1>(lane, inst0, inst1, two, ab_lds, src, params, given, fr);
   }
 }
-template <int K>
+template <bool FRONT, int K>
 __device__ __forceinline__ void spec_first_image(int lane, long inst, long ginst, unsigned img_lds, const SrcTable& src,
-                                                 const double* params, const double* given, const double* plan_dtab) {
+                                                 const double* params, const double* given, const SpecFront& fr) {
   using PC = spec::PlanConst;
   if constexpr (K < PC::rs_nchunk && K < 32) {
     if constexpr (spec_fetch_runs<false, K>() != 0) {
-      const LaneSrc m = spec_lane_src<false, K>(lane, src, params, given, plan_dtab);
+      const LaneSrc m = spec_lane_src<FRONT, false, K>(lane, src, params, given, fr);
       const char* a = m.base + (m.isg ? ginst : inst) * m.stride;
       if constexpr (PC::rs_unit == 16)
         dma16(a, img_lds + (unsigned)(K * 64 * 16));
       else
         dma4(a, img_lds + (unsigned)(K * 64 * 4));
     }
-    spec_first_image<K + 1>(lane, inst, ginst, img_lds, src, params, given, plan_dtab);
+    spec_first_image<FRONT, K + 1>(lane, inst, ginst, img_lds, src, params, given, fr);
   }
 }
+struct SpecArgsLayout {
+#define MPCASM_X(type, qual, name) type name;
+  MPCASM_SPEC_KERNEL_ARGS(MPCASM_X, MPCASM_NOTHING)
+#undef MPCASM_X
+};
+__device__ __forceinline__ const SrcTable& spec_src_from_here() {
+  typedef const __attribute__((address_space(4))) char* InArguments;
+  InArguments a = (InArguments)__builtin_amdgcn_kernarg_segment_ptr();
+  asm volatile("" : "+s"(a) : : "memory");
+  return *(const SrcTable*)(a + __builtin_offsetof(SpecArgsLayout, src));
+}
+template <bool V>
+struct SpecBool {
+  static constexpr bool value = V;
+};
 constexpr bool spec_ab_by_runs() {
   for (int k = 0; k < spec::PlanConst::rs_ab / 32; ++k)
     if (spec::FSEG_AB_N[k] == 0) return false;
@@ -327,7 +348,8 @@
     const PlanT& p, const int32_t* __restrict__ plan_itab, const double* __restrict__ plan_dtab,
     const SrcTable& src, const double* __restrict__ params, const double* __restrict__ given,
     double* __restrict__ P, double* __restrict__ q, double* __restrict__ G,
-    double* __restrict__ h, int batch, int phases, unsigned long long* __restrict__ stamps) {
+    double* __restrict__ h, int batch, int phases, unsigned long long* __restrict__ stamps,
+    const unsigned nwg, const SpecFront& front) {
   extern __shared__ __attribute__((aligned(16))) double lds[];
   const int tid = threadIdx.x, lane = tid & 63;
   const int wave = __builtin_amdgcn_readfirstlane(tid >> 6);
@@ -335,7 +357,7 @@
   const unsigned long long t_begin = STAMPS ? __builtin_amdgcn_s_memtime() : 0;
 #define SETUP_STAMP(k)                                                                  \
   if (STAMPS && stamps != nullptr && lane == 0)                                         \
-    stamps[((size_t)gridDim.x + blockIdx.x) * (NT / 64) * 8 + wave * 8 + (k)] =         \
+    stamps[((size_t)nwg + blockIdx.x) * (NT / 64) * 8 + wave * 8 + (k)] =         \
         __builtin_amdgcn_s_memtime() - t_begin;
   const bool stamping = STAMPS && stamps != nullptr;
 #define MPCASM_STAMP(slot)                                         \
@@ -475,11 +497,11 @@
 #endif
   };
   const int run_over = (phases >> 10) & 7;
-  const int run_shift = run_over ? run_over : ((long)batch >= 16L * gridDim.x && !(phases & 256) ? 2 : 0);
-  const unsigned vblock = (phases & 8192) && gridDim.x % 8 == 0
-                              ? (blockIdx.x % 8) * (gridDim.x / 8) + blockIdx.x / 8 : blockIdx.x;
+  const int run_shift = run_over ? run_over : ((long)batch >= 16L * nwg && !(phases & 256) ? 2 : 0);
+  const unsigned vblock = (phases & 8192) && nwg % 8 == 0
+                              ? (blockIdx.x % 8) * (nwg / 8) + blockIdx.x / 8 : blockIdx.x;
   auto instance_at = [&](int n) -> long {
-    return ((((long)(n >> run_shift) * gridDim.x + vblock)) << run_shift) + (n & ((1 << run_shift) - 1));
+    return ((((long)(n >> run_shift) * nwg + vblock)) << run_shift) + (n & ((1 << run_shift) - 1));
   };
   const bool gen = GEN && p.rs_nlti != 0;
   const int ct = tid - 64, CT = NT - 64;
@@ -490,11 +512,13 @@
 #endif
   int v_zb[ZK > 0 ? ZK : 1];
   const int zt0 = tid >= MW * 64 ? tid - MW * 64 : tid + WT;
-#pragma unroll
-  for (int k = 0; k < ZK; ++k) {
-    const int e = zt0 + k * NT;
-    v_zb[k] = L.p_direct && e < p.rs_nzblk * 8 ? (plan_itab + p.off_rs_zblk)[e >> 3] : 0;
-  }
+  auto load_zero_blocks = [&]() __attribute__((always_inline)) {
+#pragma unroll
+    for (int k = 0; k < ZK; ++k) {
+      const int e = zt0 + k * NT;
+      v_zb[k] = L.p_direct && e < p.rs_nzblk * 8 ? (plan_itab + p.off_rs_zblk)[e >> 3] : 0;
+    }
+  };
   int c_sg[JC], c_dst[JC];
   double c_coef[JC];
   auto load_program = [&]() __attribute__((always_inline)) {
@@ -513,8 +537,14 @@
 #else
   constexpr int FK = 0;
 #endif
-  const int32_t* gix = src.stride[MAX_SOURCES - 1] == -1
-                           ? reinterpret_cast<const int32_t*>(src.ptr[MAX_SOURCES - 1]) : nullptr;
+#ifdef MPCASM_SPEC
+  const bool indexed = (front.word & SPEC_WORD_GIX) != 0;
+  const int32_t* gix = nullptr;
+#else
+  const bool indexed = src.stride[MAX_SOURCES - 1] == -1;
+  const int32_t* gix = reinterpret_cast<const int32_t*>(src.ptr[MAX_SOURCES - 1]);
+#endif
+  auto given_row = [&](long inst) -> long { return indexed ? (long)gix[inst] : inst; };
   const char* f_base[FK > 0 ? FK : 1];
   int f_stride[FK > 0 ? FK : 1];
   bool f_isg[FK > 0 ? FK : 1];
@@ -543,7 +573,7 @@
   };
   auto fetch_image = [&](long inst, int buf, bool settled) {
     const unsigned dst0 = img_lds + (unsigned)buf * (unsigned)p.rs_img * 8u;
-    const long ginst = gix != nullptr ? (long)gix[inst] : inst;
+    const long ginst = given_row(inst);
     int kfirst = wave;
     if (FK > 0 && f_fast) {
 #pragma unroll
@@ -592,20 +622,31 @@
     constexpr bool img_runs = on_table == 0 && PlanT::rs_nchunk <= 32;
     constexpr int img_late = __builtin_popcount(on_table) + (PlanT::rs_nchunk > 32 ? PlanT::rs_nchunk - 32 : 0);
     const int ab_later = ab_runs ? nchunk : img_late;
-    if (gen && ab_runs) {
-      const long i1 = instance_at(1);
-      spec_first_ab<0>(lane, instance_at(0), i1, i1 < batch, __builtin_amdgcn_readfirstlane(ab_lds), src, params,
-                       given, plan_dtab);
-    }
-    if (ab_runs) SETUP_STAMP(2)
-    {
-      const long inst = instance_at(0), ginst = gix != nullptr ? (long)gix[inst] : inst;
-      spec_first_image<0>(lane, inst, ginst, __builtin_amdgcn_readfirstlane(img_lds), src, params, given, plan_dtab);
-    }
+    const SrcTable& src0 = spec_src_from_here();
+    auto first_requests = [&](auto use_front) __attribute__((always_inline)) {
+      constexpr bool FR = decltype(use_front)::value;
+      if (gen && ab_runs) {
+        const long i1 = instance_at(1);
+        spec_first_ab<FR, 0>(lane, instance_at(0), i1, i1 < batch, __builtin_amdgcn_readfirstlane(ab_lds), src0,
+                             params, given, front);
+      }
+      if (ab_runs) SETUP_STAMP(2)
+      const long inst = instance_at(0);
+      const long ginst = indexed ? (long)front.first_index[inst] : inst;
+      spec_first_image<FR, 0>(lane, inst, ginst, __builtin_amdgcn_readfirstlane(img_lds), src0, params, given, front);
+    };
+    if (front.word & SPEC_WORD_FRONT)
+      first_requests(SpecBool<true>{});
+    else
+      first_requests(SpecBool<false>{});
+    const SrcTable& src_late = spec_src_from_here();
+    gix = reinterpret_cast<const int32_t*>(src_late.ptr[MAX_SOURCES - 1]);
+    load_zero_blocks();
 #else
     constexpr bool ab_runs = false, img_runs = false;
     constexpr unsigned on_table = ~0u;
     const int ab_later = nchunk;
+    const SrcTable& src_late = src;
 #endif
     if (!ab_runs && lane < nab2) v_ab = t_ab[lane];
     if (lane < nltw) v_lti = t_lti[lane];
@@ -627,15 +668,15 @@
       for (int i = lane + MK * 64; i < nmeta; i += 64) meta[i] = t_meta[i];
     }
 #ifdef MPCASM_SPEC
-    if constexpr (ab_runs) spec_write_table<true, 0>(abmeta, lane, src, params, given, plan_dtab);
-    if constexpr (img_runs) spec_write_table<false, 0>(meta, lane, src, params, given, plan_dtab);
+    if constexpr (ab_runs) spec_write_table<true, 0>(abmeta, lane, src_late, params, given, front);
+    if constexpr (img_runs) spec_write_table<false, 0>(meta, lane, src_late, params, given, front);
 #endif
     for (int t = 0; t < p.nsrc + 3; ++t) {
       const int s = t - p.nsrc;
-      const double* base = s < 0 ? src.ptr[t]
+      const double* base = s < 0 ? src_late.ptr[t]
                                  : (s == 0 ? given : (s == 1 ? params : plan_dtab + p.doff_rs_const));
       const long long stride =
-          s < 0 ? src.stride[t] : (s == 0 ? (long long)p.ng : (s == 1 ? (long long)p.nparams : 0));
+          s < 0 ? src_late.stride[t] : (s == 0 ? (long long)p.ng : (s == 1 ? (long long)p.nparams : 0));
       if (lane == 0) {
         reinterpret_cast<const double**>(strm)[2 * t] = base;
         reinterpret_cast<long long*>(strm)[2 * t + 1] = stride * (long long)sizeof(double);
@@ -647,7 +688,7 @@
     }
     if (!ab_runs) SETUP_STAMP(2)
     if (!img_runs) {
-      const long inst = instance_at(0), ginst = gix != nullptr ? (long)gix[inst] : inst;
+      const long inst = instance_at(0), ginst = given_row(inst);
       for (int k = 0; k < nchunk; ++k) {
         if (k < 32 && !((on_table >> k) & 1)) continue;
         const int2 m = meta[k * 64 + lane];
@@ -674,6 +715,10 @@
     if (!prog_early) load_program();
     SETUP_STAMP(5)
   } else {
+#ifdef MPCASM_SPEC
+    gix = reinterpret_cast<const int32_t*>(spec_src_from_here().ptr[MAX_SOURCES - 1]);
+#endif
+    load_zero_blocks();
     SETUP_STAMP(0)
     lds_barrier();
     SETUP_STAMP(1)
@@ -1259,11 +1304,10 @@
 #ifndef MPCASM_SPEC_WAVES_PER_EU
 #define MPCASM_SPEC_WAVES_PER_EU 4
 #endif
+#define MPCASM_X(type, qual, name) type qual name
 extern "C" __global__ __launch_bounds__(RS_NT, MPCASM_SPEC_WAVES_PER_EU) void resident_spec_kernel(
-    const int32_t* __restrict__ plan_itab, const double* __restrict__ plan_dtab, SrcTable src,
-    const double* __restrict__ params, const double* __restrict__ given, double* __restrict__ P,
-    double* __restrict__ q, double* __restrict__ G, double* __restrict__ h, int batch, int phases,
-    unsigned long long* __restrict__ stamps) {
+    MPCASM_SPEC_KERNEL_ARGS(MPCASM_X, MPCASM_COMMA)) {
+#undef MPCASM_X
   constexpr spec::PlanConst p{};
 #ifdef MPCASM_SPEC_STAMPS
   constexpr bool stamped = true;
@@ -1275,8 +1319,10 @@
 #else
   const int mask = phases;
 #endif
-  resident_body<spec::JC, stamped, spec::PlanConst::rs_nlti != 0>(p, plan_itab, plan_dtab, src, params,
-                                                               given, P, q, G, h, batch, mask, stamps);
+  const SpecFront front{{front_ptr0, front_ptr1}, {front_stride0, front_stride1}, consts, front_word, first_index};
+  resident_body<spec::JC, stamped, spec::PlanConst::rs_nlti != 0>(p, plan_itab, plan_dtab, src, params, given, P, q,
+                                                               G, h, batch, mask, stamps,
+                                                               front_word >> SPEC_WORD_GRID, front);
 }
 namespace {
 #else
@@ -1286,7 +1332,7 @@
     double* __restrict__ P, double* __restrict__ q, double* __restrict__ G,
     double* __restrict__ h, int batch, int phases, unsigned long long* __restrict__ stamps) {
   resident_body<JC, STAMPS, GEN>(p, p.itab, p.dtab, src, params, given, P, q, G, h, batch, phases,
-                                 stamps);
+                                 stamps, gridDim.x, SpecFront{});
 }
 #endif
 
diff --git a/mpc-interface_amd/mpcasm/capi.py b/mpc-interface_amd/mpcasm/capi.py
--- a/mpc-interface_amd/mpcasm/capi.py
+++ b/mpc-interface_amd/mpcasm/capi.py
@@ -12,6 +12,7 @@
 OPT_RESIDENT_GRID = 6
 OPT_P_DIRECT = 5
 OPT_JIT_FETCH_RUNS = 7
+OPT_JIT_KERNARG_PRELOAD = 8
 OPT_JIT = 4
 PHASE_DEFAULT = 0xBF
 PHASE_STAMPS = 0x40
@@ -59,6 +60,7 @@
                                         ctypes.c_char_p, ctypes.c_size_t]),
     "mpcasm_fetch_segments": (ctypes.c_int, [_void_p, ctypes.c_size_t, _void_p, ctypes.c_size_t, ctypes.c_int,
                                              _void_p, ctypes.c_size_t, ctypes.POINTER(ctypes.c_int64)]),
+    "mpcasm_spec_kernarg_layout": (ctypes.c_int, [_void_p, ctypes.c_size_t, ctypes.POINTER(ctypes.c_int64)]),
     "mpcasm_preview_route": (ctypes.c_int, [_void_p, ctypes.c_size_t, _void_p, ctypes.c_size_t,
                                             ctypes.POINTER(ctypes.c_int64), ctypes.c_int, ctypes.c_int,
                                             ctypes.POINTER(ctypes.c_int32)]),
```

After: 178.1 million assemblies/s. About the same (-0.6%).
